# syamajala/cholesky

Hardware: AMD Instinct MI355X
Metric: fp64 factorization GF/s (numeric level loop, F_ref flops) on 3-D Laplacian (higher is better)
Workload: dtype f64; 1 GPU; tests/lapl_3375x3375 (reference fixture: 7-point Laplacian, nested-dissection ordering from the fixture files); n=3375, levels=5, separators=31, B_alg_bytes=2932064, parallelism=single GPU, precision=fp64

## Files before the change

cholesky_amd/_lib.py:

```python
import ctypes as C
import os

_HERE = os.path.dirname(os.path.abspath(__file__))
LIB_PATH = os.environ.get("CHOLAMD_LIB") or os.path.join(_HERE, "lib", "libcholamd.so")
HEADER_PATH = os.path.join(os.path.dirname(_HERE), "include", "cholamd.h")


class Filled(C.Structure):
    _fields_ = [("filled", C.c_int), ("sep_x", C.c_int), ("sep_y", C.c_int), ("interval", C.c_int), ("cluster", C.c_int),
                ("lo_x", C.c_int), ("lo_y", C.c_int), ("hi_x", C.c_int), ("hi_y", C.c_int)]


class Op(C.Structure):
    _fields_ = [("op", C.c_int), ("level", C.c_int), ("m", C.c_int), ("n", C.c_int), ("k", C.c_int),
                ("a_sx", C.c_int), ("a_sy", C.c_int), ("a_z", C.c_int), ("b_sx", C.c_int), ("b_sy", C.c_int), ("b_z", C.c_int),
                ("c_sx", C.c_int), ("c_sy", C.c_int), ("c_z", C.c_int)]


class Region(C.Structure):
    _fields_ = [("ptr", C.c_void_p), ("ld", C.c_int), ("lo_x", C.c_int), ("lo_y", C.c_int), ("hi_x", C.c_int), ("hi_y", C.c_int),
                ("tile_row", C.POINTER(C.c_int))]


class SepInfo(C.Structure):
# ... 76 lines not shown
    L.cholamd_device_set_option.argtypes = [vp, C.c_char_p, ci]
    L.cholamd_comm_unique_id.argtypes = [vp]
    L.cholamd_comm_create.argtypes = [vp, ci, ci, vp, C.POINTER(vp)]
    L.cholamd_comm_create_local.argtypes = [vp, ci, vp]
    L.cholamd_factor_multi.argtypes = [vp, vp, vp, ci, vp]
    L.cholamd_gather_factor.argtypes = [vp, vp, ci, vp]
    L.cholamd_comm_adopt.argtypes = [vp, ci, ci, C.POINTER(vp)]
    L.cholamd_comm_destroy.argtypes = [vp]
    L.cholamd_comm_destroy.restype = None
    L.cholamd_comm_allreduce.argtypes = [vp, vp, i64, vp]
    L.cholamd_device_tail_offset.argtypes = [vp]
    L.cholamd_device_tail_offset.restype = i64
    L.cholamd_exchange_tail.argtypes = [vp, vp, vp, vp]
    L.cholamd_factor_sharded.argtypes = [vp, vp, vp, vp]
    L.cholamd_factor_sharded_f32.argtypes = [vp, vp, vp, vp]
    L.cholamd_gather_to_root.argtypes = [vp, vp, ci, vp, vp]
    L.cholamd_exchange_volume.argtypes = [vp, vp]
    L.cholamd_plan_exchange_volume.argtypes = [vp, ci, ci, ci, vp]
    L.cholamd_plan_exchange_pieces.argtypes = [vp, ci, ci, ci, vp]
    L.cholamd_plan_solve_counts.argtypes = [vp, ci, ci, ci, vp]
    L.cholamd_plan_solve_skips.argtypes = [vp, ci, vp, vp]
    L.cholamd_solve_sharded.argtypes = [vp, vp, vp, vp, vp, vp]
    L.cholamd_solve_sharded_f32.argtypes = [vp, vp, vp, vp, vp, vp]
    L.cholamd_solve_refine_sharded.argtypes = [vp, vp, vp, vp, ci, C.c_double, vp, vp, vp, vp]
    L.cholamd_solve_multi.argtypes = [vp, vp, vp, vp, vp, ci, vp]
    L.cholamd_solve_refine_multi.argtypes = [vp, vp, vp, vp, ci, C.c_double, vp, vp, vp, ci, vp]
    L.cholamd_follow_rounds.argtypes = [ci, ci, ci, vp, vp]
    L.cholamd_plan_program_followers.argtypes = [vp, i64, vp]
    L.cholamd_plan_program_followers.restype = i64
    L.cholamd_plan_program_follow_own.argtypes = [vp, ci, ci, ci, ci, ci, i64, vp]
    L.cholamd_plan_program_follow_own.restype = i64
    L.cholamd_plan_program_check_follow.argtypes = [vp, ci, ci, ci, ci, ci, ci]
    L.cholamd_plan_program_hazards.argtypes = [vp, ci, ci, ci, ci, ci, vp]
    L.cholamd_factor_multi_f32.argtypes = [vp, vp, vp, ci, vp]
    L.cholamd_gather_factor_f32.argtypes = [vp, vp, ci, vp]
    L.cholamd_device_alloc.argtypes = [vp, i64, C.POINTER(vp)]
    L.cholamd_device_free.argtypes = [vp, vp]
    L.cholamd_device_upload.argtypes = [vp, vp, vp, i64, vp]
    L.cholamd_device_download.argtypes = [vp, vp, vp, i64, vp]
    L.cholamd_device_sync.argtypes = [vp, vp]
    L.cholamd_device_fill.argtypes = [vp, vp, vp]
    L.cholamd_factor.argtypes = [vp, vp, vp]
    L.cholamd_factor_levels.argtypes = [vp, vp, ci, ci, vp]
    L.cholamd_device_program_trace.argtypes = [vp, vp, vp, i64, vp, C.POINTER(ci)]
    L.cholamd_debug_live_buffers.argtypes = []
    L.cholamd_debug_live_buffers.restype = i64
    L.cholamd_factor_info.argtypes = [vp, C.POINTER(ci)]
    L.cholamd_solve.argtypes = [vp, vp, vp, vp, vp]
    L.cholamd_device_fill_f32.argtypes = [vp, vp, vp]
    L.cholamd_factor_f32.argtypes = [vp, vp, vp]
    L.cholamd_factor_levels_f32.argtypes = [vp, vp, ci, ci, vp]
    L.cholamd_solve_f32.argtypes = [vp, vp, vp, vp, vp]
    L.cholamd_solve_refine.argtypes = [vp, vp, vp, vp, ci, cd, C.POINTER(ci), C.POINTER(cd), vp]
    L.cholamd_residual.argtypes = [vp, vp, vp, vp, C.POINTER(cd), vp]
    L.cholamd_solve_nrhs.argtypes = [vp, vp, vp, i64, vp, i64, ci, vp]
    L.cholamd_solve_nrhs_f32.argtypes = [vp, vp, vp, i64, vp, i64, ci, vp]
    L.cholamd_solve_refine_nrhs.argtypes = [vp, vp, vp, i64, vp, i64, ci, ci, cd, C.POINTER(ci), vp, vp]
    L.cholamd_apply.argtypes = [vp, vp, vp, vp]
    L.cholamd_apply_nrhs.argtypes = [vp, vp, i64, vp, i64, ci, vp]
    L.cholamd_plan_apply_host.argtypes = [vp, vp, vp, vp]
    for name in ("cholamd_solve_pcg", "cholamd_solve_pcg_f32"):
        getattr(L, name).argtypes = [vp, vp, vp, vp, ci, cd, ci, vp, vp, vp, vp]
    for name in ("cholamd_solve_pcg_nrhs", "cholamd_solve_pcg_nrhs_f32"):
        getattr(L, name).argtypes = [vp, vp, vp, i64, vp, i64, ci, ci, cd, ci, vp, vp, vp, vp]
    L.cholamd_solve_half.argtypes = [vp, vp, vp, vp, ci, vp]
    L.cholamd_solve_half_f32.argtypes = [vp, vp, vp, vp, ci, vp]
# ... 125 lines not shown
```

cholesky_amd/csrc/chol_api.cpp:

```cpp
#include "chol_device.h"

int no_device_error()
{
  chol_set_error("no usable HIP device (libcholamd has no CPU fallback)");
  return CHOLAMD_ERR_NO_DEVICE;
}
bool ranges_overlap(const void *a, size_t na, const void *b, size_t nb)
{
  const char *pa = (const char *)a, *pb = (const char *)b;
  return pa < pb + nb && pb < pa + na;
}

extern "C" int cholamd_device_count(void)
{
  int n = 0;
  if (hipGetDeviceCount(&n) != hipSuccess) return 0;
  return n;
}

#define CHOL_POISON_GUARD ((size_t)64 << 10)
static bool poison_on()
{
  const char *e = std::getenv("CHOLAMD_POISON");
  return e && *e && atoi(e) != 0;
// ... 63 lines not shown

static int build_levels(cholamd_device *d)
{
  d->lv.clear(); d->lv32.clear(); d->prog = level_dev(); d->prog_ready = false;
  d->jobs.reset(); d->pwaits.reset(); d->exts.reset(); d->pctr.reset(); d->pctr_total.reset();
  d->sched_gen++;
  const int L = d->plan->levels;
  d->lv.resize(L);
  for (int lvl = 0; lvl < L; lvl++) {
    chol_level_work w;
    int rc = chol_build_level_work(d->plan, &d->opt, lvl, d->rank, d->world, &w);
    if (rc) return rc;
    rc = upload_level(d->lv[lvl], w);
    chol_level_work_free(&w);
    if (rc) return rc;
  }
  if (d->world == 1 && d->opt.program) {
    chol_level_work w;
    chol_program g;
    const bool built = chol_build_program(d->plan, &d->opt, &w, &g) == 0;
    const bool live = built && chol_program_check_built(d->plan, &d->opt, 4, &w, &g) == 0;
    if (built && !live) { chol_level_work_free(&w); chol_program_free(&g); }
    if (live) {
      int rc = upload_level(d->prog, w);
      std::vector<int> tot(g.ctr_total, g.ctr_total + g.n_ctr);
      int ncu = 256;
      hipDeviceProp_t prop;
      if (hipGetDeviceProperties(&prop, d->dev) == hipSuccess && prop.multiProcessorCount > 0) ncu = prop.multiProcessorCount;
      d->prog_grid = g.n_job < ncu ? g.n_job : ncu;
      tot.push_back(g.n_job + d->prog_grid);
      int mx = 1;
      for (int t : tot) mx = t > mx ? t : mx;
      d->prog_epoch_limit = (1 << 30) / mx;
      d->n_job = g.n_job; d->n_pctr = (int)tot.size(); d->prog_epoch = 0;
      d->jobs_host.assign(g.job, g.job + g.n_job);
      if (!rc) rc = d->jobs.upload(g.job, (size_t)g.n_job);
      const chol_wait no_wait = { 0, 0 };
      chol_ext no_ext;
      std::memset(&no_ext, 0, sizeof no_ext);
      if (!rc) rc = g.n_wait > 0 ? d->pwaits.upload(g.wait, (size_t)g.n_wait) : d->pwaits.upload(&no_wait, (size_t)1);
      if (!rc) rc = g.n_ext > 0 ? d->exts.upload(g.ext, (size_t)g.n_ext) : d->exts.upload(&no_ext, (size_t)1);
      if (!rc) rc = d->pctr_total.upload(tot.data(), tot.size());
      if (!rc) rc = d->pctr.alloc_zero(tot.size());
      chol_level_work_free(&w);
      chol_program_free(&g);
      if (rc) return rc;
      d->prog_ready = d->n_job > 0;
    }
  }
  return 0;
}

extern "C" int cholamd_device_create(const cholamd_plan *plan, int device_id, cholamd_device **out)
{
  *out = nullptr;
  if (!plan) { chol_set_error("null plan"); return CHOLAMD_ERR_ARG; }
  int ndev = 0;
  if (hipGetDeviceCount(&ndev) != hipSuccess || ndev <= 0) return no_device_error();
  if (device_id < 0 || device_id >= ndev) { chol_set_error("device %d out of range (%d devices)", device_id, ndev); return CHOLAMD_ERR_NO_DEVICE; }
  HIPCHK(hipSetDevice(device_id));
  cholamd_device *d = new cholamd_device();
  d->plan = plan; d->dev = device_id;
  chol_sched_opts_from_env(&d->opt);
  { const char *e = getenv("CHOLAMD_SOLVE_REFERENCE_SHAPE"); d->solve_reference_shape = e && *e && atoi(e) != 0; }
  { const char *e = getenv("CHOLAMD_SOLVE_DETERMINISTIC"); d->solve_deterministic = e && *e && atoi(e) != 0; }
  { const char *e = getenv("CHOLAMD_SOLVE_DETERMINISTIC_BLOCK"); d->solve_deterministic_block = e && *e && atoi(e) != 0; }
  { const char *e = getenv("CHOLAMD_SCHUR_DETERMINISTIC"); d->schur_deterministic = e && *e && atoi(e) != 0; }
// ... 30 lines not shown
  HIPCHK(hipSetDevice(d->dev));
  if (world < 1 || (world & (world - 1)) || rank < 0 || rank >= world || chol_split_level(world) > d->plan->levels - 1) {
    chol_set_error("bad partition: rank %d of %d for a %d-level tree", rank, world, d->plan->levels);
    return CHOLAMD_ERR_ARG;
  }
  d->rank = rank; d->world = world;
  free_solve_lists(d);
  return build_levels(d);
}

extern "C" int cholamd_device_bcast_phases(const cholamd_device *d)
{
  int n = 0;
  for (const level_dev &l : d->lv) for (const chol_phase &ph : l.phase) n += ph.kind == CHOL_PH_BCAST;
  return n;
}
extern "C" int cholamd_device_set_option(cholamd_device *d, const char *name, int value)
{
  HIPCHK(hipSetDevice(d->dev));
  const std::string n(name ? name : "");
  bool rebuild = true;
  if (n == "split_min") d->opt.split_min = value;
  else if (n == "split_nb") d->opt.split_nb = value;
  else if (n == "fuse") d->opt.fuse = value != 0;
  else if (n == "fuse_update_max") d->opt.fuse_update_max = value;
  else if (n == "mt_min_tiles") d->opt.mt_min_tiles = value;
  else if (n == "cells") d->opt.cells = value != 0;
  else if (n == "program") d->opt.program = value != 0;
  else if (n == "follow") d->opt.follow = value != 0;
  else if (n == "super_blocks") d->opt.super_blocks = value;
  else if (n == "follow_tail") d->opt.follow_tail = value;
  else if (n == "follow_tail_split") d->opt.follow_tail_split = value;
  else if (n == "follow_own") d->opt.follow_own = value < 0 ? 0 : value > 2 ? 2 : value;
  else if (n == "staged") d->opt.staged = value != 0;
  else if (n == "fine_upd") d->opt.fine_upd = value != 0;
  else if (n == "skyline") d->opt.skyline = value != 0;
  else if (n == "merge_targets") d->opt.merge_targets = value != 0;
  else if (n == "leaf_envelope") d->opt.leaf_envelope = value != 0;
  else if (n == "trsm_wt_min") d->opt.trsm_wt_min = value < 0 ? 0 : value;
  else if (n == "stage_chunk") d->opt.stage_chunk = value < 0 ? 0 : value;
  else if (n == "dist_top") d->opt.dist_top = value;
  else if (n == "solve_reference_shape") { d->solve_reference_shape = value != 0; rebuild = false; }
  else if (n == "solve_deterministic") { d->solve_deterministic = value != 0; rebuild = false; }
  else if (n == "solve_deterministic_block") { d->solve_deterministic_block = value != 0; rebuild = false; }
  else if (n == "schur_deterministic") { d->schur_deterministic = value != 0; rebuild = false; }
  else if (n == "multiply_nrhs_min") { d->multiply_nrhs_min = value; rebuild = false; }
  else { chol_set_error("unknown option '%s'", n.c_str()); return CHOLAMD_ERR_ARG; }
  return rebuild ? build_levels(d) : 0;
}

extern "C" int cholamd_device_alloc(cholamd_device *d, int64_t doubles, double **dptr)
{
  HIPCHK(hipSetDevice(d->dev));
  HIPCHK(fp_malloc((void **)dptr, (size_t)doubles * sizeof(double)));
  return 0;
}
extern "C" int cholamd_device_free(cholamd_device *d, double *dptr)
{
  HIPCHK(hipSetDevice(d->dev));
  HIPCHK(hipFree(dptr));
  return 0;
}
extern "C" int cholamd_device_upload(cholamd_device *d, double *d_dst, const double *h_src, int64_t doubles, void *stream)
{
  HIPCHK(hipSetDevice(d->dev));
  HIPCHK(hipMemcpyAsync(d_dst, h_src, (size_t)doubles * sizeof(double), hipMemcpyHostToDevice, (hipStream_t)stream));
// ... 172 lines not shown
  for (int k = 0; k < 4; k++) { ms_by_kind[k] = ms[k]; launches_by_kind[k] = n[k]; }
  return 0;
}

extern "C" int cholamd_device_event_overhead(cholamd_device *d, void *stream, float *ms_out)
{
  HIPCHK(hipSetDevice(d->dev));
  hipStream_t st = (hipStream_t)stream;
  const int reps = 64;
  std::vector<hipEvent_t> ev(2 * reps);
  for (auto &e : ev) e = get_event(d);
  for (int i = 0; i < reps; i++) { HIPCHK(hipEventRecord(ev[2 * i], st)); HIPCHK(hipEventRecord(ev[2 * i + 1], st)); }
  HIPCHK(hipStreamSynchronize(st));
  double acc = 0.0;
  for (int i = 0; i < reps; i++) { float ms = 0.f; HIPCHK(hipEventElapsedTime(&ms, ev[2 * i], ev[2 * i + 1])); acc += ms; }
  for (auto e : ev) d->pool.push_back(e);
  *ms_out = (float)(acc / reps);
  return 0;
}

extern "C" int cholamd_factor(cholamd_device *d, double *d_arena, void *stream)
{
  if (!d->prog_ready) return cholamd_factor_levels(d, d_arena, d->plan->levels - 1, 0, stream);
  HIPCHK(hipSetDevice(d->dev));
  hipStream_t st = (hipStream_t)stream;
  if (d->info_foreign) { HIPCHK(hipMemsetAsync(d->info, 0, 4 * sizeof(int), st)); d->info_foreign = false; }
  int *const info_cur = d->info + 2 * d->info_parity, *const info_next = d->info + 2 * (d->info_parity ^ 1);
  d->info_parity ^= 1; d->info_last = info_cur;
  if (d->prog_epoch >= d->prog_epoch_limit) { HIPCHK(hipMemsetAsync(d->pctr, 0, (size_t)d->n_pctr * sizeof(int), st)); d->prog_epoch = 0; }
  const level_dev &l = d->prog;
  {
    scoped_timer t(d, st, 3, true);
    HIPCHK((hipError_t)chol_launch_program(d_arena, d->ws, d->jobs, d->n_job, d->pwaits, l.potrf, l.trsm, l.task, l.src, d->exts, d->pctr, d->pctr_total, d->prog_epoch,
                                           d->pctr + d->n_pctr - 1, d->prog_epoch * (d->n_job + d->prog_grid), d->prog_grid, info_cur, info_next, d->trace, st));
  }
  d->prog_epoch++;
  return 0;
}
extern "C" int cholamd_device_program_trace(cholamd_device *d, double *d_arena, void *stream, int64_t cap, int64_t *out, int *njobs_out)
{
  HIPCHK(hipSetDevice(d->dev));
  if (!d->prog_ready) { chol_set_error("no program launch for this problem / these options"); return CHOLAMD_ERR_ARG; }
  *njobs_out = d->n_job;
  if (cap < (int64_t)5 * d->n_job) return 0;
  const size_t nst = (size_t)(4 + CHOL_TRACE_X) * d->n_job;
  std::vector<unsigned long long> h(nst);
  {
    dev_buf<unsigned long long> stamps;
    struct disarm { cholamd_device *d; ~disarm() { d->trace = nullptr; } } on_exit{ d };
    int rc = stamps.alloc_zero(nst);
    if (rc) return rc;
    d->trace = stamps;
    if ((rc = cholamd_factor(d, d_arena, stream))) return rc;
    HIPCHK(hipStreamSynchronize((hipStream_t)stream));
    HIPCHK(hipMemcpy(h.data(), stamps, h.size() * sizeof(unsigned long long), hipMemcpyDeviceToHost));
  }
  unsigned long long t0 = ~0ull;
  for (int j = 0; j < d->n_job; j++) if (h[4 * j] && h[4 * j] < t0) t0 = h[4 * j];
  for (int j = 0; j < d->n_job; j++) {
    out[5 * j] = d->jobs_host[j].kind + (d->jobs_host[j].kind == 0 && d->jobs_host[j].n_ext > 0 ? 10 : 0);
    for (int q = 0; q < 3; q++) out[5 * j + 1 + q] = (int64_t)(h[4 * j + q] - t0);
    out[5 * j + 4] = (int64_t)h[4 * j + 3];
  }
  if (const char *path = getenv("CHOLAMD_TRACE_FOLLOW")) {
    if (FILE *fp = fopen(path, "w")) {
      for (int j = 0; j < d->n_job; j++) {
        const unsigned long long *x = &h[(size_t)4 * d->n_job + (size_t)CHOL_TRACE_X * j];
        const int kind = d->jobs_host[j].kind;
        bool any = false;
        for (int i = 0; i < CHOL_TRACE_X; i++) any = any || x[i] != 0;
        if (!any) continue;
        if (kind == 2) { fprintf(fp, "job %d kind 2 last-stage-held %.1f\n", j, (double)(x[0] - t0) * 0.01); continue; }
        fprintf(fp, "job %d kind %d", j, kind);
        if (kind == 0 && x[1]) {
          fprintf(fp, " items %llu own-tiles-wait-over %.1f rounds:", x[1], x[0] ? (double)(x[0] - t0) * 0.01 : -1.0);
          for (unsigned long long i = 0; i < x[1] && i < 44; i++) if (x[2 + i]) fprintf(fp, " %llu:%.1f", i, (double)(x[2 + i] - t0) * 0.01);
        }
        if (kind == 0 && x[24]) { fprintf(fp, " | prologue (entry, LDS init, tables, slot tables read, columns 0-1 requested, tiles requested, columns 0-1 parked):"); const int ord[7] = { 0, 1, 2, 5, 6, 3, 4 }; for (int k = 0; k < 7; k++) fprintf(fp, " %.1f", x[24 + ord[k]] ? (double)(x[24 + ord[k]] - t0) * 0.01 : -1.0); }
        fprintf(fp, kind == 0 ? " | column started:" : " | POTRF column seen:");
        for (int k = 0; k < 24; k++) if (x[72 + k]) fprintf(fp, " %d:%.1f", k, (double)(x[72 + k] - t0) * 0.01);
        fprintf(fp, kind == 0 ? " | column published:" : " | column tile on the channel:");
        for (int k = 0; k < 24; k++) if (x[48 + k]) fprintf(fp, " %d:%.1f", k, (double)(x[48 + k] - t0) * 0.01);
        fprintf(fp, "\n");
      }
      fclose(fp);
    }
  }
  return 0;
}
extern "C" int cholamd_factor_info(cholamd_device *d, int *sep_out)
{
  HIPCHK(hipSetDevice(d->dev));
  int h[2] = { 0, 0 };
  HIPCHK(hipMemcpy(h, d->info_last ? d->info_last : d->info, sizeof h, hipMemcpyDeviceToHost));
  if (sep_out) *sep_out = h[1];
  if (h[0] == CHOLAMD_ERR_STALL)
    chol_set_error("factorisation stalled: a workgroup of a fused launch waited ~50 ms for a progress word of the same launch and gave up; the factor is not valid");
  else if (h[0] < 0) chol_set_error("factorisation failed with internal code %d", h[0]);
  return h[0];
}

__global__ void k_zero_ranges(double *y, const int *ranges, int nr)
{
  const int off = ranges[2 * blockIdx.y], len = ranges[2 * blockIdx.y + 1];
  for (int i = blockIdx.x * blockDim.x + threadIdx.x; i < len; i += gridDim.x * blockDim.x) y[off + i] = 0.0;
}
int build_solve(cholamd_device *d, int rank, int world)
{
  const int L = d->plan->levels;
  if (d->solve_ready && d->solve_rank == rank && d->solve_world == world) return 0;
  free_solve_lists(d);
// ... 1655 lines not shown
```

cholesky_amd/csrc/chol_device.h:

```cpp
#ifndef CHOL_DEVICE_H
#define CHOL_DEVICE_H
#include <hip/hip_runtime.h>
#include <rccl/rccl.h>

#include <cstdio>
#include <algorithm>
#include <cstdlib>
#include <cfloat>
#include <cmath>
#include <cctype>
#include <cstring>
#include <string>
#include <type_traits>
#include <vector>

#include <atomic>
#include "chol_devbuf.h"
#include "chol_kernels.h"
#include "chol_plan.h"
#include "cholamd.h"

#define HIPCHK(call)                                                                                  \
  do {                                                                                                \
    hipError_t e_ = (call);                                                                           \
// ... 55 lines not shown
  std::vector<level_dev> lv;
  std::vector<solve_dev> sv;
  bool solve_ready = false;
  int solve_rank = 0, solve_world = 1;
  dev_buf<int> zr_sub; int n_zr_sub = 0;
  dev_buf<double> ws;
  dev_buf<double> ws_solve;
  dev_buf<int> step_flags;
  int step_gen = 0;
  dev_buf<double> w256;
  dev_buf<double> step_xt;
  bool keep_inverses = false;
  dev_buf<int> info;
  int *info_last = nullptr;
  int info_parity = 0; bool info_foreign = false;
  dev_buf<int> progress;
  int epoch = 0, done_total = 0;
  dev_buf<int64_t> a_dst; dev_buf<double> a_val; dev_buf<int> perm; dev_buf<double> ytmp;
  dev_buf<int64_t> top_dst[2]; dev_buf<double> top_val[2]; dev_buf<int> top_e[2]; int64_t top_n[2] = { 0, 0 }; int top_gen[2] = { -1, -1 };
  dev_buf<int> a_src, csr_src; dev_buf<unsigned char> e_cls;
  dev_buf<int> e_row, e_col;
  dev_buf<int64_t> vs_dev, vs_init; pinned_words vs_host;
  int64_t vs_last[4] = { 0, 0, 0, 0 };
  bool vs_called = false, vs_last_valid = false;
  bool vs_in_force = false;
  bool f32_pending = false;
  bool timing = false;
  std::vector<timed_launch> tl;
  std::vector<hipEvent_t> pool;
  level_dev prog;
  dev_buf<chol_job> jobs; dev_buf<chol_wait> pwaits; dev_buf<chol_ext> exts;
  dev_buf<int> pctr, pctr_total;
  int n_job = 0, n_pctr = 0, prog_grid = 0, prog_epoch = 0, prog_epoch_limit = 0;
  bool prog_ready = false;
  unsigned long long *trace = nullptr;
  std::vector<chol_job> jobs_host;
  std::vector<level_dev> lv32;
  dev_buf<float> ws32;
  int f32_range = -1; int64_t f32_bad = -1;
  dev_buf<int64_t> csr_ptr; dev_buf<int> csr_col; dev_buf<double> csr_val;
  dev_buf<double> rvec, dxvec, partial;
  dev_buf<char> xstage; size_t xstage_bytes = 0; dev_buf<sum_desc> xdesc; int xdesc_gen = -1, xdesc_elem = 0, sched_gen = 0;
  chol_sched_opts opt;
  bool solve_reference_shape = false;
  bool solve_deterministic = false;
  bool solve_deterministic_block = false;
  sdet_dev sdet;
  dev_buf<double> ynrhs, bnrhs, rnrhs, dxnrhs, pnrhs;
  dev_buf<chol_trsv_desc> dg_desc; dev_buf<int> dg_prefix; int n_dg = 0;
  dev_buf<double> ld_part; dev_buf<int64_t> ld_ipart, ld_res;
  std::vector<selinv_dev> si; dev_buf<double> si_ws; bool si_ready = false;
  std::vector<schur_dev> sc;
  bool schur_deterministic = false;
  std::vector<sdet_dev> scd;
  int64_t schur_launches[4] = { 0, 0, 0, 0 };
  dev_buf<chol_mul_item> mul_item[2]; dev_buf<chol_mul_src> mul_src[2]; int n_mul_item[2] = { 0, 0 }; bool mul_ready = false;
  dev_buf<double> mvec, mr_part; dev_buf<int64_t> mr_ipart, mr_res;
  dev_buf<double> mznrhs, mwnrhs;
  int multiply_nrhs_min = 0;
  dev_buf<double> pcg_b, pcg_p, pcg_q, pcg_r, pcg_z, pcg_part;
  dev_buf<chol_pcg_rec> pcg_rec; pinned_words pcg_host;
};

struct local_group {
  int n = 0, refs = 0;
  std::vector<int> dev;
// ... 48 lines not shown
```

cholesky_amd/csrc/chol_kernels.h:

```cpp
#ifndef CHOL_KERNELS_H
#define CHOL_KERNELS_H
#include <hip/hip_runtime_api.h>
#include <stdint.h>
#include "chol_plan.h"
int chol_launch_scatter(double *arena, const int64_t *dst, const double *val, int64_t nnz, hipStream_t st);
#define CHOL_VALUES_STATUS 1
#define CHOL_VALUES_GATHER 2
int chol_launch_set_values(const double *vals, int64_t nz, const unsigned char *cls, double *a_val, const int *a_src, int64_t nnz_a,
                           double *csr_val, const int *csr_src, int64_t ncsr, int parts, int64_t *status, hipStream_t st);
int chol_launch_gather(double *out, const double *in, const int *idx, int64_t n, hipStream_t st);
int chol_launch_potrf(double *base, double *ws, const chol_potrf_desc *descs, int n, int *info, hipStream_t st);
int chol_launch_potrf_big(double *base, double *ws, const chol_potrf_desc *descs, int n, int *info, hipStream_t st);
int chol_launch_potrf_trsm(double *base, double *ws, const chol_potrf_desc *pdescs, int n_potrf, const chol_trsm_desc *tdescs, int n_trsm,
                           const chol_upd_task *tasks, const chol_upd_src *srcs, int n_task,
                           int *info, int *progress, int progress_base, int *done, int done_target, hipStream_t st);
int chol_launch_program(double *base, double *ws, const chol_job *jobs, int njobs, const chol_wait *waits, const chol_potrf_desc *pdescs, const chol_trsm_desc *tdescs,
                        const chol_upd_task *tasks, const chol_upd_src *srcs, const chol_ext *exts, int *ctr, const int *ctr_total, int epoch, int *head, int head_base,
                        int grid, int *info, int *info_next, unsigned long long *trace, hipStream_t st);
int chol_launch_trsm_w(double *base, const double *ws, const chol_trsm_desc *descs, int n, hipStream_t st);
int chol_launch_trsm_wt(double *base, const double *ws, const chol_trsm_desc *descs, int n, hipStream_t st);
int chol_launch_trsm_big(double *base, const double *ws, const chol_trsm_desc *descs, int n, hipStream_t st);
int chol_launch_dinv(const double *L, int n, int ldl, double *W, hipStream_t st);
int chol_launch_trsm(double *base, const double *ws, const chol_trsm_desc *descs, int n, hipStream_t st);
int chol_launch_update(double *base, const chol_upd_task *tasks, const chol_upd_src *srcs, int ntask, hipStream_t st);
int chol_launch_update_mt(double *base, const chol_upd_task *tasks, const chol_upd_src *srcs, int ntask, int64_t arena_elems, hipStream_t st);
int chol_launch_permute(const double *in, const int *perm, double *out, int n, int inverse, hipStream_t st);
template <class TL> int chol_launch_solve_dinv(const TL *base, const chol_trsv_desc *descs, int n, int max_n, double *W, hipStream_t st);
template <class TL> int chol_launch_solve_trsv(const TL *base, const chol_trsv_desc *descs, int n, int max_n, int max_under, const double *W, double *y, int backward, int *flags, int *gen, const double *W256, double *xt, hipStream_t st);
#define CHOL_STEPW_MAX_SEPS 128
template <class TL> int chol_launch_solve_inv256(const TL *base, const chol_trsv_desc *descs, int n, int max_n, const double *W16, double *W256, hipStream_t st);
template <class TL> int chol_launch_solve_offdiag(const TL *base, const chol_gemv_desc *blocks, const int *items, int n_items, double *y, int backward, hipStream_t st);
int chol_launch_trsv_fwd(const double *base, const chol_trsv_desc *descs, int n, double *y, hipStream_t st);
int chol_launch_gemv_fwd(const double *base, const chol_gemv_desc *descs, const int *grp_start, const int *grp_rows, int ngroups, double *y, hipStream_t st);
int chol_launch_bwd(const double *base, const chol_trsv_desc *descs, const chol_gemv_desc *gd, const int *gstart, int n, double *y, hipStream_t st);
int chol_launch_residual(const int64_t *ptr, const int *col, const double *val, const double *b, const double *x, double *r, int n, double *partial, hipStream_t st);
int chol_launch_axpy1(double *x, const double *dx, int n, hipStream_t st);
int chol_launch_scatter(float *arena, const int64_t *dst, const double *val, int64_t nnz, hipStream_t st);
int chol_launch_potrf(float *base, float *ws, const chol_potrf_desc *descs, int n, int *info, hipStream_t st);
int chol_launch_trsm(float *base, const float *ws, const chol_trsm_desc *descs, int n, hipStream_t st);
int chol_launch_trsm_wt(float *base, const float *ws, const chol_trsm_desc *descs, int n, hipStream_t st);
int chol_launch_update(float *base, const chol_upd_task *tasks, const chol_upd_src *srcs, int ntask, hipStream_t st);
int chol_launch_update_mt(float *base, const chol_upd_task *tasks, const chol_upd_src *srcs, int ntask, int64_t arena_elems, hipStream_t st);
#define CHOL_NRHS_W 32
int chol_nrhs_launch_permute(const double *B, int64_t ldb, const int *perm, double *Y, double *X, int64_t ldx, int n, int c0, int cols, int inverse, hipStream_t st);
template <class TL> int chol_nrhs_launch_trsv(const TL *base, const chol_trsv_desc *descs, int n, int max_n, int max_under, const double *W16, const double *W256, double *Y, int backward, hipStream_t st);
template <class TL> int chol_nrhs_launch_offdiag(const TL *base, const chol_gemv_desc *blocks, const int *items, int n_items, double *Y, int backward, hipStream_t st);
int chol_nrhs_launch_residual(const int64_t *ptr, const int *col, const double *val, const double *B, int64_t ldb, const double *X, int64_t ldx, double *R, int64_t ldr,
                              int n, int cols, double *partial, hipStream_t st);
int chol_nrhs_launch_axpy(double *X, int64_t ldx, const double *D, int64_t ldd, int n, int cols, hipStream_t st);
#define CHOL_LOGDET_MAX_BLOCKS 1024
template <class TL> int chol_launch_factor_diag(const TL *base, const chol_trsv_desc *descs, const int *prefix, int nd, int n, const int *perm, double *diag, hipStream_t st);
// ... 44 lines not shown
```

cholesky_amd/csrc/chol_kernels.hip:

```cpp
#include <hip/hip_runtime.h>
#include <float.h>
#include <stdint.h>

#include "chol_plan.h"
#include "chol_kernels.h"

#include "chol_wave.h"

__device__ __forceinline__ void report_stall(int *info)
{
#ifdef STALL_PLAIN
  atomicCAS(&info[0], 0, CHOLAMD_ERR_STALL);
#else
  int e;
  asm volatile("v_mov_b32 %0, %1" : "=v"(e) : "i"(CHOLAMD_ERR_STALL));
  atomicCAS(&info[0], 0, e);
#endif
}
__device__ __forceinline__ int wait_progress(const int *progress, int target, int seen, int *info)
{
  if (seen >= target) return seen;
  int v = 0;
  for (int it = 0; it < (1 << 23); ++it) {
    v = __builtin_amdgcn_readfirstlane(__hip_atomic_load(progress, __ATOMIC_RELAXED, __HIP_MEMORY_SCOPE_AGENT));
// ... 691 lines not shown
    if (rowok && col < n) e = (ti > tj || c <= r15) ? gload<PUB>(&src[(int64_t)(4 * q) * lda]) : 0.0;
    v[q] = e;
  }
  return v;
}
#define FOLLOW_SLOTS 4
#define FOLLOW_LOADS ((CHOL_FOLLOW_MAXT * TS * TS + RR_THREADS - 1) / RR_THREADS)
template <int SLEEP = 0>
__device__ __forceinline__ void wait_list(const chol_wait *__restrict__ wl, int n, const int *ctr, const int *__restrict__ ctr_total, int epoch, int lane, int *info)
{
  for (int b0 = 0; b0 < n; b0 += 64) {
    int c = 0, need = 0;
    const bool mine = b0 + lane < n;
    if (mine) { const chol_wait wt = wl[b0 + lane]; c = wt.ctr; need = wt.value + epoch * ctr_total[wt.ctr]; }
    for (int it = 0;; ++it) {
      const bool ok = !mine || __hip_atomic_load(&ctr[c], __ATOMIC_RELAXED, __HIP_MEMORY_SCOPE_AGENT) >= need;
      if (!__ballot(!ok)) break;
      if (it >= (1 << 21)) { if (lane == 0) report_stall(info); break; }
#ifndef WAIT_SLEEP
#define WAIT_SLEEP 32
#endif
      __builtin_amdgcn_s_sleep(SLEEP ? SLEEP : WAIT_SLEEP);
    }
  }
}
__device__ __forceinline__ bool wait_list_holds(const chol_wait *__restrict__ wl, int n, const int *ctr, const int *__restrict__ ctr_total, int epoch, int lane)
{
  bool ok = true;
  for (int b0 = 0; b0 < n; b0 += 64)
    if (b0 + lane < n) { const chol_wait wt = wl[b0 + lane]; ok = ok && __hip_atomic_load(&ctr[wt.ctr], __ATOMIC_RELAXED, __HIP_MEMORY_SCOPE_AGENT) >= wt.value + epoch * ctr_total[wt.ctr]; }
  return !__ballot(!ok);
}
struct follow_args { const chol_ext *ext; int n_ext; const int *ctr; const int *ctr_total; int epoch; const chol_wait *wl; int n_wl; unsigned long long *stamp, *xstamp;
                     int own_at;  };
__device__ __forceinline__ int ext_ready(const follow_args &f, int from, int lane)
{
  bool ok = true;
  if (from + lane < f.n_ext) {
    const int c = f.ext[from + lane].ctr;
    ok = __hip_atomic_load(&f.ctr[c], __ATOMIC_RELAXED, __HIP_MEMORY_SCOPE_AGENT) - f.epoch * f.ctr_total[c] >= f.ext[from + lane].need;
  }
  const unsigned long long notok = __ballot(!ok);
  const int lead = notok ? __builtin_ctzll(notok) : 64;
  return min(from + lead, f.n_ext);
}
template <bool UPD, bool PUB, bool TR = false>
__device__ __forceinline__ void follow_external(const double *__restrict__ base, const follow_args f, int T, int n, double *sE, d4 (&tile)[11], d4 (&stage)[3],
                                                const int (&ijp)[12], int w, int lane, int tid, int *info, const double *A, int lda, int r15, int g, int *sReady)
{
  const int lp = lane;
  int buf = 0;
  int ready = 0, ng = 0;
  double va[FOLLOW_LOADS], vb[FOLLOW_LOADS];
#ifndef FOLLOW_OWN_SLEEP
#define FOLLOW_OWN_SLEEP 4
#endif
  static_assert(CHOL_FOLLOW_PAIR_MAXT == RR_MAXT, "a pair of followed column tiles shares one LDS buffer of RR_MAXT tiles");
  const int own_at = f.own_at;
  const bool own_last = f.n_wl > 0 && own_at >= f.n_ext;
  bool own_ok = false;
  int own_c = 0, own_need = 0, own_v = 0;
  const bool own_look = !UPD && own_last && f.n_wl <= 64;
  if (own_look && lane < f.n_wl) { const chol_wait wt = f.wl[lane]; own_c = wt.ctr; own_need = wt.value + f.epoch * f.ctr_total[wt.ctr]; }
#define EXT_ROUND(I_) chol_follow_round(I_, f.n_ext, T)
#define EXT_LOAD(I_, V_)                                                                                             \
  {                                                                                                                  \
    const chol_ext xl_ = f.ext[I_];                                                                                  \
    const double *src_ = base + xl_.off;                                                                             \
    _Pragma("unroll") for (int it = 0; it < FOLLOW_LOADS; ++it) {                                                    \
      const int idx = tid + it * RR_THREADS;                                                                         \
      const int row = (idx >> 8) * TS + (idx & 15), col = (idx >> 4) & 15;                                           \
      V_[it] = (idx < T * TS * TS && row < n && col < xl_.ncol) ? gload<true>(&src_[row + (int64_t)col * xl_.ld]) : 0.0; \
    }                                                                                                                \
  }
#define EXT_LOAD_ROUND(I_)                                                                                           \
  {                                                                                                                  \
    EXT_LOAD(I_, va);                                                                                                \
    ng = EXT_ROUND(I_);                                                                                              \
    if (ng == 2) { EXT_LOAD((I_) + 1, vb); }                                                                         \
  }
#define EXT_UPDATE(acc_, ti_, tj_)                                                                                   \
  {                                                                                                                  \
    _Pragma("unroll") for (int st = 0; st < 4; ++st)                                                                 \
      acc_ = __builtin_amdgcn_mfma_f64_16x16x4f64(sB[(tj_) * (TS * TS) + st * 64 + lp], -sB[(ti_) * (TS * TS) + st * 64 + lp], acc_, 0, 0, 0); \
    if (G == 2) {                                                                                                    \
      _Pragma("unroll") for (int st = 0; st < 4; ++st)                                                               \
        acc_ = __builtin_amdgcn_mfma_f64_16x16x4f64(sB2[(tj_) * (TS * TS) + st * 64 + lp], -sB2[(ti_) * (TS * TS) + st * 64 + lp], acc_, 0, 0, 0); \
    }                                                                                                                \
  }
#define OWN_TILES()                                                                                                  \
  {                                                                                                                  \
  \
      if (!UPD) wait_list<FOLLOW_OWN_SLEEP>(f.wl, f.n_wl, f.ctr, f.ctr_total, f.epoch, lane, info);  \
      if (TR && !UPD && f.xstamp && lane == 0) f.xstamp[0] = __builtin_amdgcn_s_memrealtime(); \
      lds_barrier(); \
      if (UPD) { \
        int rx = r15, gx = g;  \
        asm volatile("" : "+v"(rx), "+v"(gx)); \
    _Pragma("unroll")                                                                                            \
        for (int it = 0; it < 3; ++it) { \
          const int u = min(w + it * RR_NW, 2 * T - 2); \
          stage[it] += load_tile<PUB>(A, lda, n, u < T ? u : u - T + 1, u < T ? 0 : 1, rx, gx); \
        } \
        __builtin_amdgcn_sched_barrier(0);  \
    _Pragma("unroll")                                                                                            \
        for (int s = 0; s < FOLLOW_SLOTS; ++s) \
          if (ijp[s] != 0xffff) tile[s] += load_tile<PUB>(A, lda, n, ijp[s] & 0xff, ijp[s] >> 8, rx, gx); \
        __builtin_amdgcn_sched_barrier(0); \
      } \
 \
  }
  for (int i = 0; i < f.n_ext;) {
    if (f.n_wl > 0 && i == own_at) OWN_TILES();
    if (ng == 0) {
      const int need = i + EXT_ROUND(i);
      if (ready < need) {
        if (!UPD) {
          ready = ext_ready(f, i, lane);
          for (int it = 0; ready < need; ++it) {
            if (it >= (1 << 24)) { if (lane == 0) report_stall(info); ready = f.n_ext; break; }
#ifndef EXT_SLEEP
#define EXT_SLEEP 4
#endif
            __builtin_amdgcn_s_sleep(EXT_SLEEP);
            ready = ext_ready(f, i, lane);
          }
          if (lane == 0) __hip_atomic_store(sReady, ready, __ATOMIC_RELAXED, __HIP_MEMORY_SCOPE_WORKGROUP);
        } else {
          for (int it = 0;; ++it) {
            ready = __builtin_amdgcn_readfirstlane(__hip_atomic_load(sReady, __ATOMIC_RELAXED, __HIP_MEMORY_SCOPE_WORKGROUP));
            if (ready >= need) break;
            if (it >= (1 << 25)) { if (lane == 0) report_stall(info); ready = f.n_ext; break; }
            __builtin_amdgcn_s_sleep(2);
          }
        }
      }
      EXT_LOAD_ROUND(i);
    }
    const int G = ng;
    if (TR && !UPD && f.xstamp && lane == 0 && i < 44) { f.xstamp[1] = f.n_ext; f.xstamp[2 + i] = __builtin_amdgcn_s_memrealtime(); }
    double *sB = sE + buf * (RR_MAXT * TS * TS), *sB2 = sB + T * TS * TS;
#pragma unroll
    for (int it = 0; it < FOLLOW_LOADS; ++it) {
      const int idx = tid + it * RR_THREADS;
      if (idx < T * TS * TS) { sB[idx] = va[it]; if (G == 2) sB2[idx] = vb[it]; }
    }
    const int j = i + G;
    ng = 0;
    int pv = 0, pneed = 0;
    bool polled = false;
    if (j < f.n_ext && j + EXT_ROUND(j) <= ready) { EXT_LOAD_ROUND(j); }
    else if (j < f.n_ext && !UPD) {
      polled = true;
      if (j + lane < f.n_ext) { const int c = f.ext[j + lane].ctr; pv = __hip_atomic_load(&f.ctr[c], __ATOMIC_RELAXED, __HIP_MEMORY_SCOPE_AGENT); pneed = f.epoch * f.ctr_total[c] + f.ext[j + lane].need; }
    }
    const bool look = own_look && !own_ok;
    if (look && lane < f.n_wl) own_v = __hip_atomic_load(&f.ctr[own_c], __ATOMIC_RELAXED, __HIP_MEMORY_SCOPE_AGENT);
    lds_barrier();
    if (look) own_ok = !__ballot(lane < f.n_wl && own_v < own_need);
    if (UPD) {
#pragma unroll
      for (int it = 0; it < 3; ++it) {
        const int u = w + it * RR_NW;
        if (u < 2 * T - 1) { const int tj = u < T ? 0 : 1, ti = u < T ? u : u - T + 1; EXT_UPDATE(stage[it], ti, tj); }
      }
#pragma unroll
      for (int s = 0; s < FOLLOW_SLOTS; ++s)
        if (ijp[s] != 0xffff) { const int ti = ijp[s] & 0xff, tj = ijp[s] >> 8; EXT_UPDATE(tile[s], ti, tj); }
    }
    buf ^= 1;
    if (polled) {
      const unsigned long long notok = __ballot(j + lane < f.n_ext && pv < pneed);
      const int r2 = min(j + (notok ? __builtin_ctzll(notok) : 64), f.n_ext);
      if (r2 > ready) { ready = r2; if (lane == 0) __hip_atomic_store(sReady, ready, __ATOMIC_RELAXED, __HIP_MEMORY_SCOPE_WORKGROUP); }
    } else if (UPD && j < f.n_ext && ready < j + EXT_ROUND(j)) {
      const int r2 = __builtin_amdgcn_readfirstlane(__hip_atomic_load(sReady, __ATOMIC_RELAXED, __HIP_MEMORY_SCOPE_WORKGROUP));
      ready = r2 > ready ? r2 : ready;
    }
    i = j;
  }
  if (own_last) {
    if (!UPD && !own_ok) wait_list<FOLLOW_OWN_SLEEP>(f.wl, f.n_wl, f.ctr, f.ctr_total, f.epoch, lane, info);
    if (TR && !UPD && f.xstamp && lane == 0) f.xstamp[0] = __builtin_amdgcn_s_memrealtime();
    lds_barrier();
    if (UPD) {
      int rx = r15, gx = g;
      asm volatile("" : "+v"(rx), "+v"(gx));
#pragma unroll
      for (int it = 0; it < 3; ++it) {
        const int u = min(w + it * RR_NW, 2 * T - 2);
        tile[FOLLOW_SLOTS + it] = load_tile<PUB>(A, lda, n, u < T ? u : u - T + 1, u < T ? 0 : 1, rx, gx);
      }
#pragma unroll
      for (int s = 0; s < FOLLOW_SLOTS; ++s) {
        const d4 zero4 = { 0.0, 0.0, 0.0, 0.0 };
        tile[FOLLOW_SLOTS + 3 + s] = zero4;
        if (ijp[s] != 0xffff) tile[FOLLOW_SLOTS + 3 + s] = load_tile<PUB>(A, lda, n, ijp[s] & 0xff, ijp[s] >> 8, rx, gx);
      }
    }
  }
#undef OWN_TILES
#undef EXT_LOAD_ROUND
#undef EXT_ROUND
#undef EXT_UPDATE
#undef EXT_LOAD
}

template <bool PUB, bool FOLLOW = false, bool TR = false>
__device__ __forceinline__ void potrf_rr_body(double *__restrict__ base, double *__restrict__ ws, const chol_potrf_desc d, int *__restrict__ info,
                                              int *__restrict__ progress, int progress_base, double *smem, const unsigned char *__restrict__ sky, const follow_args fa = follow_args(), const int tid = threadIdx.x)
{
  double (*const sRaw)[TS * TS] = (double (*)[TS * TS])(smem);
  double (*const sSol)[RR_MAXT][TS * TS] = (double (*)[RR_MAXT][TS * TS])(smem + RR_OFF_SOL);
  double (*const sDg)[TS * TS] = (double (*)[TS * TS])(smem + RR_OFF_DG);
  double (*const sLW)[4 * TS][TS + 1] = (double (*)[4 * TS][TS + 1])(smem + RR_OFF_LW);
  double (*const sConv)[TS + 1] = (double (*)[TS + 1])(smem + RR_OFF_CONV);
  double (*const sOv)[TS * TS] = (double (*)[TS * TS])(smem + RR_OFF_OV);
  unsigned short *const sIJ = (unsigned short *)(smem + RR_OFF_IJ);
  int *const sFlag = (int *)(smem + RR_OFF_FLAG);
  unsigned char *const sKm = (unsigned char *)(smem + RR_OFF_KM);
  int *const sMask = (int *)(smem + RR_OFF_MASK);
  unsigned char *const sSky = (unsigned char *)(smem + RR_OFF_SKY);
  int *const fL = &sFlag[0], *const fP = &sFlag[1], *const cSol = &sFlag[2], *const cUpd = &sFlag[3];
  int *const cRaw = &sFlag[4];
  int *const fA = &sFlag[6];
  int *const fD = &sFlag[7];
  int *const f00 = &sFlag[8];

  double *A = base + d.a_off;
  double *W = ws + d.dinv_off;
  const int n = d.n, lda = d.lda;
  const int T = (n + TS - 1) / TS;
  const int ntl = T * (T + 1) / 2;
  const int lane = tid & 63;
  const int wave = __builtin_amdgcn_readfirstlane(tid >> 6);
  const int r15 = lane & 15, g = lane >> 4;
  const int lp0 = g * TS + r15;

#define PSTAMP(i_) do { if (TR && fa.xstamp && fa.n_ext == 0 && tid == 64) fa.xstamp[24 + (i_)] = __builtin_amdgcn_s_memrealtime(); } while (0)
  PSTAMP(0);
  d4 stage[3];
  const bool own_pending = FOLLOW && fa.n_ext > 0 && fa.n_wl > 0 && fa.own_at >= fa.n_ext;
  const bool stage_early = !(FOLLOW && fa.n_ext > 0) && wave != 0;
  if (stage_early) {
#pragma unroll
    for (int it = 0; it < 3; ++it) {
      const int u = min(wave - 1 + it * RR_NW, 2 * T - 2);
      stage[it] = load_tile<PUB>(A, lda, n, u < T ? u : u - T + 1, u < T ? 0 : 1, r15, g);
    }
  }
  const unsigned char *const tab = d.tab > 0 ? sky - __builtin_offsetof(chol_potrf_desc, sky) + d.tab : nullptr;
  if (tab) {
    static_assert((RR_MAXT * RR_NW) % 1 == 0 && RR_THREADS >= RR_MAXT * RR_NW + RR_SLOTS * RR_NW / 2 + RR_SLOTS * RR_NW / 4, "one pass copies the tables");
    if (tid < RR_MAXT * RR_NW) sMask[tid] = ((const int *)(tab + CHOL_RR_TAB_MASK))[tid];
    else if (tid < RR_MAXT * RR_NW + RR_SLOTS * RR_NW / 2) ((int *)sIJ)[tid - RR_MAXT * RR_NW] = ((const int *)(tab + CHOL_RR_TAB_IJ))[tid - RR_MAXT * RR_NW];
    else if (tid < RR_MAXT * RR_NW + RR_SLOTS * RR_NW / 2 + RR_SLOTS * RR_NW / 4) ((int *)sKm)[tid - RR_MAXT * RR_NW - RR_SLOTS * RR_NW / 2] = ((const int *)(tab + CHOL_RR_TAB_KM))[tid - RR_MAXT * RR_NW - RR_SLOTS * RR_NW / 2];
  } else {
    for (int t = tid; t < RR_SLOTS * RR_NW; t += RR_THREADS) { sIJ[t] = (unsigned short)0xffff; sKm[t] = 0; }
    for (int t = tid; t < RR_MAXT * RR_NW; t += RR_THREADS) sMask[t] = 0;
  }
  if (tid < 24) sSky[tid] = sky[tid];
  if (tid < 10) sFlag[tid] = 0;
  if (tid < TS * TS) sConv[TS + (tid >> 4)][tid & 15] = (tid >> 4) == (tid & 15) ? 1.0 : 0.0;
  __syncthreads();
  PSTAMP(1);
  const int ntl2 = (T - 2) * (T - 1) / 2;
  if (!tab) {
  for (int t = tid + 2 * T - 1; t < ntl; t += RR_THREADS) {
    int ti, tj, ow, os;
    tile_of_index(t, T, ti, tj);
    rr_owner(ntl - 1 - t, ntl2, ow, os);
    sIJ[os * RR_NW + ow] = (unsigned short)(ti | (tj << 8));
    const int kmin = max(sky[min(ti, 23)], sky[min(tj, 23)]);
    sKm[os * RR_NW + ow] = kmin | (tj < sky[min(ti, 23)] ? CHOL_RR_KM_ZERO : 0);
    const int last = ti == tj ? tj - 2 : tj - 1;
    for (int k = min(kmin, last); k <= last; ++k) atomicOr(&sMask[k * RR_NW + ow], 1 << os);
  }
  for (int t = tid; t < T * T; t += RR_THREADS) {
    const int k = t / T, i = t % T;
    if (i >= k + 2 && sky[min(i, 23)] <= k) {
      const int hv = i % RR_NHEAVY;
      atomicOr(&sMask[k * RR_NW + hv + hv / 3], 1 << (i < k + 2 + RR_NHEAVY ? RR_M_SOLVE0 : RR_M_SOLVE1));
    }
  }
  __syncthreads();
  }
  PSTAMP(2);

  if (wave == 0) {
    __builtin_amdgcn_s_setprio(3);
    if (FOLLOW && fa.n_ext > 0) {
      d4 tdummy[RR_RSLOTS], sdummy[3];
      int idummy[RR_SLOTS];
      follow_external<false, PUB, TR>(base, fa, T, n, smem + RR_OFF_SOL, tdummy, sdummy, idummy, 0, lane, tid, info, A, lda, r15, g, &sFlag[5]);
      lds_barrier();
      if (TR && fa.stamp && lane == 0) *fa.stamp = __builtin_amdgcn_s_memrealtime();
    }
    __builtin_amdgcn_s_setprio(3);
    lds_wait_ge(f00, 1);
    d4 dk;
#pragma unroll
    for (int q = 0; q < 4; ++q) dk[q] = sDg[0][q * 64 + lp0];
    STAMP_DECL;
    POLL_DECL;
    for (int k = 0; k < T; ++k) {
      STAMPK(0);
      double a[TS], unused;
#pragma unroll
      for (int q = 0; q < 4; ++q) sConv[r15][g + 4 * q] = dk[q];
#pragma unroll
      for (int c = 0; c < TS; ++c) a[c] = sConv[lane & 31][c];
      const int cupd_early = __hip_atomic_load(cUpd, __ATOMIC_RELAXED, __HIP_MEMORY_SCOPE_WORKGROUP);
      STAMPK(1);
      if (TR && fa.xstamp && lane == 0 && k < 24) fa.xstamp[72 + k] = __builtin_amdgcn_s_memrealtime();
      const bool more = k + 1 < T;
      const int kn = more ? k + 1 : k;
      long long fl = 0;
      d4 raw, dn;
      const int bad = chol16_rows(a, unused, r15, [&]() {
        fl = __hip_atomic_load((long long *)fA, __ATOMIC_RELAXED, __HIP_MEMORY_SCOPE_WORKGROUP);
        asm volatile("" ::: "memory");
#pragma unroll
        for (int q = 0; q < 4; ++q) { raw[q] = sRaw[kn][q * 64 + lp0]; dn[q] = sDg[kn & 1][q * 64 + lp0]; }
      });
      STAMPK(2);
      if (bad && k * TS + bad <= n && lane == 0) {
        if (atomicCAS(&info[0], 0, d.col0 + k * TS + bad) == 0) info[1] = d.sep;
// ... 29 lines not shown
    STAMP_FLUSH;
    POLL_FLUSH;
    __builtin_amdgcn_s_setprio(0);
  } else {
    d4 tile[RR_RSLOTS];
    const int w = wave - 1;
    const int hw = rr_heavy_index(w);
    int ijp[RR_SLOTS];
#pragma unroll
    for (int s = 0; s < RR_SLOTS; ++s) ijp[s] = __builtin_amdgcn_readfirstlane((int)sIJ[s * RR_NW + w]);
    int kmn[RR_SLOTS];
#pragma unroll
    for (int s = 0; s < RR_SLOTS; ++s) kmn[s] = __builtin_amdgcn_readfirstlane((int)sKm[s * RR_NW + w]);
    unsigned zmask = 0;
#pragma unroll
    for (int s = 0; s < RR_SLOTS; ++s) { zmask |= (kmn[s] & CHOL_RR_KM_ZERO) ? 1u << s : 0u; kmn[s] &= CHOL_RR_KM_ZERO - 1; }
    PSTAMP(5);

    if (FOLLOW && fa.n_ext > 0) {
      const bool early = fa.n_wl == 0;
      const d4 zero4 = { 0.0, 0.0, 0.0, 0.0 };
#pragma unroll
      for (int it = 0; it < 3; ++it) {
        const int u = min(w + it * RR_NW, 2 * T - 2);
        stage[it] = zero4;
        if (early) stage[it] = load_tile<PUB>(A, lda, n, u < T ? u : u - T + 1, u < T ? 0 : 1, r15, g);
      }
#pragma unroll
      for (int s = 0; s < FOLLOW_SLOTS; ++s) {
        d4 v = zero4;
        if (early && ijp[s] != 0xffff) v = load_tile<PUB>(A, lda, n, ijp[s] & 0xff, ijp[s] >> 8, r15, g);
        tile[s] = v;
      }
      follow_external<true, PUB, TR>(base, fa, T, n, smem + RR_OFF_SOL, tile, stage, ijp, w, lane, tid, info, A, lda, r15, g, &sFlag[5]);
      lds_barrier();
      if (own_pending) {
#pragma unroll
        for (int it = 0; it < 3; ++it) stage[it] += tile[FOLLOW_SLOTS + it];
      }
    } else {
    PSTAMP(6);
#pragma unroll
    for (int s = 0; s < RR_RSLOTS; ++s) {
      d4 v = { 0.0, 0.0, 0.0, 0.0 };
      if (ijp[s] != 0xffff && !(zmask & (1u << s))) v = load_tile<PUB>(A, lda, n, ijp[s] & 0xff, ijp[s] >> 8, r15, g);
      tile[s] = v;
    }
    }
    PSTAMP(3);
#pragma unroll
    for (int it = 0; it < 3; ++it) {
      const int u = w + it * RR_NW;
      if (u < 2 * T - 1) {
        const int tj = u < T ? 0 : 1, ti = u < T ? u : u - T + 1;
        double *park = ti == tj ? &sDg[ti][0] : tj == 0 ? &sRaw[ti][0] : &sSol[1][ti][0];
#pragma unroll
        for (int q = 0; q < 4; ++q) park[q * 64 + lp0] = stage[it][q];
        if (u == 0) lds_set(f00, 1, lane);
        if (ti == 1) lds_set(tj == 0 ? fA : fD, 1, lane);
        if (tj == 0 && ti > 0) lds_inc(cRaw, lane);
      }
    }
    if (FOLLOW && fa.n_ext > 0) {
      static_assert(FOLLOW_SLOTS + 3 + FOLLOW_SLOTS <= RR_RSLOTS, "a follower's own tiles in flight fit the register tiles it does not use");
      if (own_pending) {
        __builtin_amdgcn_sched_barrier(0);
#pragma unroll
        for (int s = 0; s < FOLLOW_SLOTS; ++s) tile[s] += tile[FOLLOW_SLOTS + 3 + s];
      }
// ... 454 lines not shown
  const int wave = __builtin_amdgcn_readfirstlane(threadIdx.x >> 6);
  const int lane = threadIdx.x & 63;
  const int grp = wave >> 2;
  const int n_tg = (n_trsm + 2) / 3;
  if ((int)blockIdx.x < n_potrf) {
    potrf_rr_body<true>(base, ws, pdescs[blockIdx.x], info, progress + blockIdx.x, progress_base, smem, pdescs[blockIdx.x].sky);
  } else if ((int)blockIdx.x < n_potrf + n_tg) {
    double (*sX)[3][TS * TS] = (double (*)[3][TS * TS])smem;
    const int id = ((int)blockIdx.x - n_potrf) * 3 + grp;
    chol_trsm_desc d = tdescs[min(id, n_trsm - 1)];
    if (id >= n_trsm) d.m = 0;
    trsm_rr_body<true, FUSED_SLOTS>(base, ws, d, sX[grp], wave & 3, lane, progress + d.flag, progress_base, info);
    if (n_task > 0) {
      asm volatile("s_waitcnt vmcnt(0)" ::: "memory");
      lds_barrier();
      if (threadIdx.x == 0) __hip_atomic_fetch_add(done, 1, __ATOMIC_RELAXED, __HIP_MEMORY_SCOPE_AGENT);
    }
  } else {
    double (*sAcc)[3][3][4][64] = (double (*)[3][3][4][64])smem;
    const int u = (int)blockIdx.x - n_potrf - n_tg;
    int round = 0;
    for (int t0 = u * 3; t0 < n_task; t0 += n_upd_wg * 3, ++round) {
      const int tid = t0 + grp;
      const bool live = tid < n_task;
      update_task_body<true>(base, tasks[live ? tid : t0], srcs, sAcc[round & 1][grp], wave & 3, lane, live, round == 0 ? done : nullptr, done_target, info);
    }
  }
}

#define PROG_XFLAGS 32
#define PROG_OFF_XFLAG (3 * RR_MAXT * TS * TS)
static_assert(PROG_XFLAGS >= 4 * ((CHOL_RR_MAXN / TS + 3) / 4) && PROG_XFLAGS >= 4 * FUSED_SLOTS && PROG_OFF_XFLAG + (3 * PROG_XFLAGS + 1) / 2 <= RR_SMEM_DOUBLES, "the strips' slots and flags fit the image");
static_assert(CHOL_RR_MAXN <= RR_MAXT * TS && CHOL_FUSE_MAXN <= CHOL_RR_MAXN, "one slot per column tile of the widest strip");
template <bool TR>
__global__ __launch_bounds__(RR_THREADS) void k_program(double *__restrict__ base, double *__restrict__ ws, const chol_job *__restrict__ jobs, int njobs,
                                                        const chol_wait *__restrict__ waits, const chol_potrf_desc *__restrict__ pdescs,
                                                        const chol_trsm_desc *__restrict__ tdescs, const chol_upd_task *__restrict__ tasks,
                                                        const chol_upd_src *__restrict__ srcs, const chol_ext *__restrict__ exts,
                                                        int *__restrict__ ctr, const int *__restrict__ ctr_total, int epoch, int *__restrict__ head, int head_base,
                                                        int *__restrict__ info, int *__restrict__ info_next, unsigned long long *__restrict__ trace)
{
  if (info_next && blockIdx.x == 0 && threadIdx.x == 0) { info_next[0] = 0; info_next[1] = 0; }
  __shared__ double smem[RR_SMEM_DOUBLES];
  __shared__ int s_job;
  const int wave_id = __builtin_amdgcn_readfirstlane(threadIdx.x >> 6);
  for (;;) {
#ifdef TID_PLAIN
    int tid = threadIdx.x;
#else
    int tid = wave_id * 64 + (int)__builtin_amdgcn_mbcnt_hi(~0u, __builtin_amdgcn_mbcnt_lo(~0u, 0u));
#endif
    asm volatile("" : "+v"(tid));
    const int wave = wave_id;
    const int lane = tid & 63;
    const int grp = wave >> 2;
    __syncthreads();
    if (tid == 0) s_job = atomicAdd(head, 1) - head_base;
    __syncthreads();
    const int j = s_job;
    if (j >= njobs) break;
    const chol_job jb = jobs[j];
    if (TR && trace && tid == 0) { trace[4 * j] = __builtin_amdgcn_s_memrealtime(); trace[4 * j + 3] = blockIdx.x; }
    int *const xflags = (int *)(smem + PROG_OFF_XFLAG);
    if (jb.kind == CHOL_JOB_TRSM && tid < 3 * PROG_XFLAGS) xflags[tid] = 0;
    bool fenced = false;
    chol_upd_task tpre;
    if (jb.kind == CHOL_JOB_UPDATE) {
      const int tk = jb.first + min(jb.mode == 0 ? wave : grp, jb.n - 1);
      tpre = tasks[tk];
      int touch = 0;
      for (int sx = tpre.src_begin; sx < tpre.src_end; ++sx) touch += srcs[sx].k;
      asm volatile("" :: "s"(touch));
    }
    if (jb.n_pre > 0 && !(jb.kind == CHOL_JOB_POTRF && jb.n_ext > 0)) {
      if (wave == 0) wait_list(waits + jb.wait_first, jb.n_pre, ctr, ctr_total, epoch, lane, info);
      lds_barrier();
      fenced = true;
    }
    if (TR && trace && tid == 0) trace[4 * j + 1] = __builtin_amdgcn_s_memrealtime();
    if (jb.kind == CHOL_JOB_POTRF) {
      const chol_potrf_desc pd = pdescs[jb.first];
      follow_args fa;
      fa.ext = exts + jb.ext_first; fa.n_ext = jb.n_ext; fa.ctr = ctr; fa.ctr_total = ctr_total; fa.epoch = epoch; fa.wl = waits + jb.wait_first; fa.n_wl = jb.n_wait; fa.own_at = jb.mode; fa.stamp = TR && trace ? &trace[4 * j + 1] : nullptr; fa.xstamp = TR && trace ? &trace[4 * njobs + CHOL_TRACE_X * j] : nullptr;
      potrf_rr_body<true, true, TR>(base, ws, pd, info, ctr + pd.ctr, epoch * ctr_total[pd.ctr], smem, pdescs[jb.first].sky, fa, tid);
    } else if (jb.kind == CHOL_JOB_TRSM) {
      double (*sX)[RR_MAXT][TS * TS] = (double (*)[RR_MAXT][TS * TS])smem;
      chol_trsm_desc d = tdescs[jb.first + min(grp, jb.n - 1)];
      if (grp >= jb.n) d.m = 0;
      if (!fenced) lds_barrier();
      if (d.band > 0)
        trsm_rr_body<true, (CHOL_RR_MAXN / TS + 3) / 4, true, TR, true>(base, ws, d, sX[grp], wave & 3, lane, ctr + d.flag, epoch * ctr_total[d.flag], info, d.chan >= 0 ? ctr + d.chan : nullptr,
                                                                         TR && trace && grp == 0 ? &trace[4 * njobs + CHOL_TRACE_X * j] : nullptr, xflags + grp * PROG_XFLAGS);
      else
        trsm_rr_body<true, FUSED_SLOTS, false, TR, true>(base, ws, d, sX[grp], wave & 3, lane, ctr + d.flag, epoch * ctr_total[d.flag], info, d.chan >= 0 ? ctr + d.chan : nullptr,
                                                         TR && trace && grp == 0 ? &trace[4 * njobs + CHOL_TRACE_X * j] : nullptr, xflags + grp * PROG_XFLAGS);
    } else {
      stage_waits sw;
      sw.w = waits + jb.wait_first + jb.n_pre; sw.n = jb.n_wait - jb.n_pre; sw.ctr = ctr; sw.ctr_total = ctr_total; sw.epoch = epoch; sw.info = info;
      unsigned long long *const xs = TR && trace && wave == 0 ? &trace[4 * njobs + CHOL_TRACE_X * j] : nullptr;
      if (jb.mode == 0) {
        for (int t0 = jb.first; t0 < jb.first + jb.n; t0 += RR_NW + 1) {
          const int tk = t0 + wave;
          if (tk < jb.first + jb.n) update_task_wave<true, TR>(base, t0 == jb.first ? tpre : tasks[tk], srcs, lane, sw, xs);
        }
      } else {
        double (*sAcc)[3][3][4][64] = (double (*)[3][3][4][64])smem;
        int round = 0;
        for (int t0 = jb.first; t0 < jb.first + jb.n; t0 += 3, ++round) {
          const int tk = t0 + grp;
          const bool live = tk < jb.first + jb.n;
          update_task_body<true, TR>(base, t0 == jb.first ? tpre : tasks[live ? tk : t0], srcs, sAcc[round & 1][grp], wave & 3, lane, live, nullptr, 0, info, sw, xs);
        }
      }
    }
    if (jb.sig[0] >= 0) {
      asm volatile("s_waitcnt vmcnt(0)" ::: "memory");
      lds_barrier();
// ... 285 lines not shown
  return (int)hipGetLastError();
}
int chol_launch_potrf_big(double *base, double *ws, const chol_potrf_desc *descs, int n, int *info, hipStream_t st)
{
  if (n <= 0) return 0;
  hipLaunchKernelGGL(k_potrf_big, dim3(n), dim3(256), 0, st, base, ws, descs, info);
  return (int)hipGetLastError();
}
int chol_launch_dinv(const double *L, int n, int ldl, double *W, hipStream_t st)
{
  if (n <= 0) return 0;
  hipLaunchKernelGGL(k_dinv, dim3((n + TS - 1) / TS), dim3(64), 0, st, L, n, ldl, W);
  return (int)hipGetLastError();
}
int chol_launch_trsm(double *base, const double *ws, const chol_trsm_desc *descs, int n, hipStream_t st)
{
  if (n <= 0) return 0;
  hipLaunchKernelGGL(k_trsm_rr, dim3(n), dim3(256), 0, st, base, ws, descs);
  return (int)hipGetLastError();
}
int chol_launch_potrf_trsm(double *base, double *ws, const chol_potrf_desc *pdescs, int n_potrf, const chol_trsm_desc *tdescs, int n_trsm,
                           const chol_upd_task *tasks, const chol_upd_src *srcs, int n_task,
                           int *info, int *progress, int progress_base, int *done, int done_target, hipStream_t st)
{
  if (n_potrf <= 0) return 0;
  int n_upd_wg = (n_task + 2) / 3;
  if (n_upd_wg > 1024) n_upd_wg = 1024;
  hipLaunchKernelGGL(k_potrf_trsm, dim3(n_potrf + (n_trsm + 2) / 3 + n_upd_wg), dim3(RR_THREADS), 0, st, base, ws, pdescs, n_potrf, tdescs, n_trsm,
                     tasks, srcs, n_task, n_upd_wg, info, progress, progress_base, done, done_target);
  return (int)hipGetLastError();
}
int chol_launch_program(double *base, double *ws, const chol_job *jobs, int njobs, const chol_wait *waits, const chol_potrf_desc *pdescs, const chol_trsm_desc *tdescs,
                        const chol_upd_task *tasks, const chol_upd_src *srcs, const chol_ext *exts, int *ctr, const int *ctr_total, int epoch, int *head, int head_base,
                        int grid, int *info, int *info_next, unsigned long long *trace, hipStream_t st)
{
  if (njobs <= 0) return 0;
  if (trace) hipLaunchKernelGGL(k_program<true>, dim3(grid), dim3(RR_THREADS), 0, st, base, ws, jobs, njobs, waits, pdescs, tdescs, tasks, srcs, exts, ctr, ctr_total, epoch, head, head_base, info, info_next, trace);
  else hipLaunchKernelGGL(k_program<false>, dim3(grid), dim3(RR_THREADS), 0, st, base, ws, jobs, njobs, waits, pdescs, tdescs, tasks, srcs, exts, ctr, ctr_total, epoch, head, head_base, info, info_next, trace);
  return (int)hipGetLastError();
}
int chol_launch_trsm_w(double *base, const double *ws, const chol_trsm_desc *descs, int n, hipStream_t st)
{
  if (n <= 0) return 0;
  hipLaunchKernelGGL(k_trsm_w, dim3((n + 3) / 4), dim3(256), 0, st, base, ws, descs, n);
  return (int)hipGetLastError();
}
int chol_launch_trsm_wt(double *base, const double *ws, const chol_trsm_desc *descs, int n, hipStream_t st)
{
  if (n <= 0) return 0;
  hipLaunchKernelGGL(k_trsm_wt, dim3((n + TT_WAVES - 1) / TT_WAVES), dim3(64 * TT_WAVES), 0, st, base, ws, descs, n);
  return (int)hipGetLastError();
}
int chol_launch_trsm_big(double *base, const double *ws, const chol_trsm_desc *descs, int n, hipStream_t st)
{
  if (n <= 0) return 0;
  hipLaunchKernelGGL(k_trsm_big, dim3((n + 3) / 4), dim3(256), 0, st, base, ws, descs, n);
  return (int)hipGetLastError();
}
int chol_launch_update(double *base, const chol_upd_task *tasks, const chol_upd_src *srcs, int ntask, hipStream_t st)
{
  if (ntask <= 0) return 0;
  const int per_xcd = (ntask + 7) / 8;
  hipLaunchKernelGGL(k_update, dim3(per_xcd * 8), dim3(256), 0, st, base, tasks, srcs, ntask, per_xcd);
  return (int)hipGetLastError();
}
int chol_launch_update_mt(double *base, const chol_upd_task *tasks, const chol_upd_src *srcs, int ntask, int64_t arena_elems, hipStream_t st)
{
  if (ntask <= 0) return 0;
  const int per_xcd = (ntask + 7) / 8;
  hipLaunchKernelGGL(k_update_mt, dim3(per_xcd * 8), dim3(256), 0, st, base, tasks, srcs, ntask, per_xcd, arena_elems);
  return (int)hipGetLastError();
// ... 2 lines not shown
```

cholesky_amd/csrc/chol_plan.h:

```cpp
#ifndef CHOL_PLAN_H
#define CHOL_PLAN_H

#include <stdint.h>
#include "cholamd.h"

#ifdef __cplusplus
extern "C" {
#endif

#define CHOL_ENTRY_OUT 0
#define CHOL_ENTRY_IN 1
#define CHOL_ENTRY_DROPPED 2
#define CHOL_NB 16
#define CHOL_RR_MAXN 272
#ifndef CHOL_FOLLOW_ALL_MAXT
#define CHOL_FOLLOW_ALL_MAXT 4
#endif
#define CHOL_FOLLOW_TAIL 3
#define CHOL_FOLLOW_MAXT 10
#define CHOL32_TRSM_GROUP 16
#define CHOL32_MAXN 128

typedef struct {
  int n_int;
// ... 93 lines not shown
  int range;
  int stage, pad;
} chol_upd_src;

typedef struct {
  int64_t c_off;
  int ldc;
  short mv, nv;
  int lower;
  int src_begin, src_end;
  int ar, br;
  int blk;
} chol_upd_task;

typedef struct { int ctr, value; } chol_wait;
enum chol_job_kind { CHOL_JOB_POTRF = 0, CHOL_JOB_TRSM = 1, CHOL_JOB_UPDATE = 2 };
typedef struct {
  int kind;
  int first, n;
  int wait_first, n_wait;
  int sig[2], sig_add;
  int ext_first, n_ext;
  int mode, n_pre;
} chol_job;
typedef struct {
  int64_t off;
  int ld, ncol;
  int ctr, need;
} chol_ext;
#define CHOL_FOLLOW_PAIR_MAXT 17
#define CHOL_FOLLOW_SINGLE_TAIL 0
#define CHOL_FOLLOW_OWN_BEFORE 2
#define CHOL_FOLLOW_OWN 1
#if defined(__HIPCC__)
#define CHOL_HD __host__ __device__ __forceinline__
#else
#define CHOL_HD static inline
#endif
CHOL_HD int chol_follow_round(int i, int n_ext, int T)
{
  const int pair_lim = 2 * T <= CHOL_FOLLOW_PAIR_MAXT ? n_ext - CHOL_FOLLOW_SINGLE_TAIL : 0;
  return i + 1 < pair_lim ? 2 : 1;
}
CHOL_HD int chol_follow_own_at(int n_ext, int T)
{
  int own_at = 0;
  for (int i = 0; i < n_ext; i += chol_follow_round(i, n_ext, T))
    if (i <= n_ext - CHOL_FOLLOW_OWN_BEFORE) own_at = i;
  return own_at;
}

typedef struct {
  int n_job; chol_job *job;
  int n_wait; chol_wait *wait;
  int n_ext; chol_ext *ext;
  int n_ctr; int *ctr_total;
  int follow;
} chol_program;

enum chol_phase_kind {
  CHOL_PH_POTRF = 0, CHOL_PH_TRSM = 1,
  CHOL_PH_UPDATE = 2,
  CHOL_PH_UPDATE_MT = 3,
  CHOL_PH_TRSM_W = 4,
  CHOL_PH_FUSED = 5,
  CHOL_PH_BCAST = 6,
  CHOL_PH_TRSM_WT = 7
};
typedef struct {
  int kind;
  int first, n, first2, n2, first3, n3;
} chol_phase;
typedef struct { int64_t off, count; int owner, heap; } chol_bcast;
static inline unsigned chol_top_contributors(int heap, int world)
{
  int d = 0, l = 0;
  while ((1 << d) < world) d++;
  while ((heap >> (l + 1)) > 0) l++;
  const int lo = (heap << (d - l)) - (1 << d), hi = ((heap + 1) << (d - l)) - (1 << d);
  unsigned m = 0u;
  for (int g = lo; g < hi; g++) m |= 1u << g;
  return m;
}

#define CHOL_DIST_MIN 1024
#define CHOL_MT_MIN_TILES 8192
typedef struct {
  int split_min, split_nb;
  int fuse;
  int fuse_update_max;
  int mt_min_tiles;
  int trsm_group;
  int trsm_wt_min;
  int cells;
  int program;
  int follow;
  int dist_top;
  int skyline;
  int stage_chunk;
  int fine_upd;
  int staged;
  int follow_tail_split;
  int follow_tail;
  int merge_targets;
  int leaf_envelope;
  int super_blocks;
  int follow_own;
} chol_sched_opts;
#define CHOL_SUPER_BLOCKS 3
#define CHOL_STAGE_CHUNK 0
void chol_sched_opts_default(chol_sched_opts *o);
void chol_sched_opts_from_env(chol_sched_opts *o);

#define CHOL_SPLIT_MIN 144
#ifndef CHOL_PROG_SPLIT_MIN
#define CHOL_PROG_SPLIT_MIN 176
#endif
#define CHOL_SPLIT_NB 144

typedef struct {
  int level;
  int n_phase; chol_phase *phase;
  int n_potrf; chol_potrf_desc *potrf;
  int n_trsm; chol_trsm_desc *trsm;
  int n_task; chol_upd_task *task;
  int n_task_mt; chol_upd_task *task_mt;
  int n_src; chol_upd_src *src;
  int n_bcast; chol_bcast *bcast;
} chol_level_work;

typedef struct {
  int64_t a_off; int n, lda; int x_off; int sep;
  int64_t dinv_off;
  int band;
} chol_trsv_desc;
typedef struct {
  int64_t a_off; int m, n, lda; int x_off, y_off;
  int c_lo;
} chol_gemv_desc;

// ... 164 lines not shown
```

cholesky_amd/csrc/chol_schedule.c:

```c
#define _GNU_SOURCE
#include <stdlib.h>
#include <string.h>

#include "chol_plan.h"
#include "cholamd.h"

int chol_split_level(int world)
{
  int d = 0;
  while ((1 << d) < world) d++;
  return d;
}

int chol_owner_of(const plan_t *p, int label, int world)
{
  int d = chol_split_level(world), lvl = p->level_of[label];
  if (lvl < d) return -1;
  return (p->heap_of[label] >> (lvl - d)) - (1 << d);
}

typedef struct {
  int64_t key;
  int64_t seq;
  int64_t c_off, a_off, b_off;
// ... 34 lines not shown
}

static int same_sources(const upd_tuple *tu, const tgt_group *a, const tgt_group *b, int dr, int dc)
{
  if (a->e - a->i != b->e - b->i) return 0;
  for (int q = 0; q < a->e - a->i; q++) {
    const upd_tuple *x = &tu[a->i + q], *y = &tu[b->i + q];
    if (x->src_sep != y->src_sep || x->lda != y->lda || x->ldb != y->ldb || x->k != y->k || y->a_off != x->a_off + dr || y->b_off != x->b_off + dc) return 0;
  }
  return 1;
}

static void index_snapshot(const plan_t *p, int lbl, int64_t *first, int *count)
{
  for (int b = 0; b < p->nblk; b++) { first[b] = 0; count[b] = 0; }
  const cholamd_filled *v = p->snap[lbl];
  for (int64_t i = 0; i < p->snap_n[lbl]; i++) {
    int b = BIDX(p, v[i].sep_x, v[i].sep_y);
    if (count[b] == 0) first[b] = i;
    count[b]++;
  }
}

typedef struct { int64_t c_off; int ldc, m, n, syrk, src_begin, src_end, blk, ar0, br0; } upd_target;
typedef struct { chol_level_work *w; const chol_sched_opts *o; int force_fine; int cur_blk; const int *follow_lim;
  int dist_world, dist_rank; const struct cholamd_plan *dist_plan; int tgt_sep, tgt_col0; int cap_b;
  const int *sw_of;
  int cur_band; const int *bw_of;
  int cap_p, cap_t, cap_k, cap_km, cap_s, cap_ph; upd_target *pend; int n_pend, cap_pend; } builder;
static int env_int(const char *name, int dflt) { const char *e = getenv(name); return e && *e ? atoi(e) : dflt; }
void chol_sched_opts_default(chol_sched_opts *o)
{
  o->split_min = CHOL_SPLIT_MIN; o->split_nb = CHOL_SPLIT_NB; o->fuse = 1; o->fuse_update_max = CHOL_FUSE_UPDATE_MAX;
  o->mt_min_tiles = CHOL_MT_MIN_TILES; o->trsm_wt_min = CHOL_TRSM_WT_MIN; o->trsm_group = 0; o->cells = 1; o->program = 1; o->follow = 1; o->super_blocks = CHOL_SUPER_BLOCKS; o->dist_top = 2; o->follow_tail = CHOL_FOLLOW_TAIL; o->follow_tail_split = CHOL_FOLLOW_TAIL; o->staged = 1; o->fine_upd = 1; o->skyline = 1; o->stage_chunk = CHOL_STAGE_CHUNK; o->merge_targets = 1; o->leaf_envelope = 1; o->follow_own = CHOL_FOLLOW_OWN;
}
void chol_sched_opts_from_env(chol_sched_opts *o)
{
  chol_sched_opts_default(o);
  o->split_min = env_int("CHOLAMD_SPLIT_MIN", o->split_min);
  o->split_nb = env_int("CHOLAMD_SPLIT_NB", o->split_nb);
  o->fuse = !env_int("CHOLAMD_NO_FUSE", 0);
  o->fuse_update_max = env_int("CHOLAMD_FUSE_UPDATE_MAX", o->fuse_update_max);
  o->mt_min_tiles = env_int("CHOLAMD_MT_MIN_TILES", o->mt_min_tiles);
  o->trsm_wt_min = env_int("CHOLAMD_TRSM_WT_MIN", o->trsm_wt_min);
  o->cells = !env_int("CHOLAMD_NO_CELLS", 0);
  o->program = !env_int("CHOLAMD_NO_PROGRAM", 0);
  o->follow = !env_int("CHOLAMD_NO_FOLLOW", 0);
  o->dist_top = env_int("CHOLAMD_DIST_TOP", o->dist_top);
  o->super_blocks = env_int("CHOLAMD_SUPER_BLOCKS", o->super_blocks);
  o->follow_tail = env_int("CHOLAMD_FOLLOW_TAIL", o->follow_tail);
  o->follow_tail_split = env_int("CHOLAMD_FOLLOW_TAIL_SPLIT", o->follow_tail_split);
  o->follow_own = env_int("CHOLAMD_FOLLOW_OWN", o->follow_own);
  o->staged = !env_int("CHOLAMD_NO_STAGED", 0);
  o->fine_upd = !env_int("CHOLAMD_NO_FINE_UPD", 0);
  o->skyline = !env_int("CHOLAMD_NO_SKYLINE", 0);
  o->merge_targets = !env_int("CHOLAMD_NO_MERGE_TARGETS", 0);
  o->leaf_envelope = !env_int("CHOLAMD_NO_LEAF_ENVELOPE", 0);
  o->stage_chunk = env_int("CHOLAMD_STAGE_CHUNK", o->stage_chunk);
}
static int split_nb(const chol_sched_opts *o) { int v = o->split_nb; if (v > CHOL_RR_MAXN) v = CHOL_RR_MAXN; v = (v + 15) / 16 * 16; if (v < 16) v = 16; return v; }
static int pivot_blocks(const chol_sched_opts *o, int n) { return n > o->split_min || n > CHOL_RR_MAXN ? (n + split_nb(o) - 1) / split_nb(o) : 1; }
static int pivot_block_width(const chol_sched_opts *o, int n) { const int nb = pivot_blocks(o, n); return nb == 1 ? n : ((n + nb - 1) / nb + 15) / 16 * 16; }


static void push_phase_full(builder *B, chol_phase ph)
{
  chol_level_work *w = B->w;
  if (w->n_phase == B->cap_ph) { B->cap_ph = B->cap_ph ? 2 * B->cap_ph : 16; w->phase = realloc(w->phase, B->cap_ph * sizeof(chol_phase)); }
  w->phase[w->n_phase++] = ph;
}
static void push_phase_f(builder *B, int kind, int first, int n, int force)
{
  if (n <= 0 && !force) return;
  if (n < 0) n = 0;
  chol_phase ph = { kind, first, n, 0, 0, 0, 0 };
  push_phase_full(B, ph);
}
static void push_phase(builder *B, int kind, int first, int n) { push_phase_f(B, kind, first, n, 0); }
void chol_potrf_table(int n, const unsigned char *sky, unsigned char *out)
{
  int *mask = (int *)(out + CHOL_RR_TAB_MASK);
  unsigned short *ij = (unsigned short *)(out + CHOL_RR_TAB_IJ);
  unsigned char *km = out + CHOL_RR_TAB_KM;
  memset(out, 0, CHOL_RR_TAB_BYTES);
  for (int t = 0; t < CHOL_RR_SLOTS * CHOL_RR_NW; t++) ij[t] = 0xffff;
// ... 651 lines not shown
} pblock;
typedef struct { chol_program *pg; int cap_j, cap_w, cap_e, cap_c;
  int *c_updp, *cnt_updp;
} pbuild;
static int new_ctr(pbuild *P, int total)
{
  chol_program *g = P->pg;
  if (g->n_ctr == P->cap_c) { P->cap_c = P->cap_c ? 2 * P->cap_c : 256; g->ctr_total = realloc(g->ctr_total, P->cap_c * sizeof(int)); }
  g->ctr_total[g->n_ctr] = total;
  return g->n_ctr++;
}
static void add_wait(pbuild *P, int ctr, int value)
{
  chol_program *g = P->pg;
  if (value <= 0) return;
  if (g->n_wait == P->cap_w) { P->cap_w = P->cap_w ? 2 * P->cap_w : 1024; g->wait = realloc(g->wait, P->cap_w * sizeof(chol_wait)); }
  chol_wait wt = { ctr, value };
  g->wait[g->n_wait++] = wt;
}
static int add_ext(pbuild *P, chol_ext e)
{
  chol_program *g = P->pg;
  if (g->n_ext == P->cap_e) { P->cap_e = P->cap_e ? 2 * P->cap_e : 64; g->ext = realloc(g->ext, P->cap_e * sizeof(chol_ext)); }
  g->ext[g->n_ext] = e;
  return g->n_ext++;
}
typedef struct { chol_ext x; int key, seq; } ext_item;
static int cmp_ext_item(const void *a, const void *b)
{
  const ext_item *x = a, *y = b;
  if (x->key != y->key) return x->key < y->key ? -1 : 1;
  return x->seq < y->seq ? -1 : (x->seq > y->seq);
}
static void push_ext_items(ext_item **items, int *n, int *cap, int64_t off, int ld, int k, int chan, int nstrip, int key0, int e_from)
{
  for (int e = e_from; e * CHOL_NB < k; e++) {
    if (*n == *cap) { *cap = *cap ? 2 * *cap : 64; *items = realloc(*items, *cap * sizeof(ext_item)); }
    ext_item *it = &(*items)[(*n)];
    it->x.off = off + (int64_t)e * CHOL_NB * ld; it->x.ld = ld; it->x.ncol = k - e * CHOL_NB < CHOL_NB ? k - e * CHOL_NB : CHOL_NB;
    it->x.ctr = chan + e; it->x.need = nstrip;
    it->key = key0 + e; it->seq = *n;
    (*n)++;
  }
}
static chol_job *add_job(pbuild *P, int kind, int first, int n, int wait_first)
{
  chol_program *g = P->pg;
  if (g->n_job == P->cap_j) { P->cap_j = P->cap_j ? 2 * P->cap_j : 1024; g->job = realloc(g->job, P->cap_j * sizeof(chol_job)); }
  chol_job j = { kind, first, n, wait_first, g->n_wait - wait_first, { -1, -1 }, 0, g->n_ext, 0, 0, g->n_wait - wait_first };
  g->job[g->n_job] = j;
  return &g->job[g->n_job++];
}
void chol_program_free(chol_program *g)
{
  free(g->job); free(g->wait); free(g->ext); free(g->ctr_total);
  memset(g, 0, sizeof *g);
}
typedef struct {
  const plan_t *p; chol_sched_opts o; chol_level_work *w; chol_program *pg; builder B; pbuild P;
  int follow;
  unsigned char **sky;
  int *bw_of, *band_of;
  int *sw_of;
  int *nblk_of; pblock **pb;
  int *est_start;
  int *c_upd, *c_updd;
  int *cnt_upd, *cnt_updd;
  int *snap_upd;
  int *follow_lim;
  int level; const cholamd_filled *snap; int64_t *first; int *count;
  int *hs, nh, steps;
} prog_ctx;
// ... 125 lines not shown
    free(first[s]);
  }
  free(first);
  return sky;
}
void chol_free_skylines(unsigned char **sky, int ns) { if (!sky) return; for (int s = 1; s <= ns; s++) free(sky[s]); free(sky); }
int **chol_leaf_row_first(const plan_t *p)
{
  const int ns = p->nsep, L = p->levels;
  int **first = calloc(ns + 1, sizeof(int *));
  for (int h = 1 << (L - 1); h <= ns; h++) {
    const int s = p->tree[h], n = p->sep_size[s], ld = p->panel_ld[s];
    if (n <= 0) continue;
    first[s] = malloc((size_t)ld * sizeof(int));
    for (int r = 0; r < ld; r++) first[s][r] = r < n ? r : n;
  }
  for (int64_t e = 0; e < p->nnz_a; e++) {
    const int64_t off = p->a_dst[e];
    int lo = 1, hi = ns;
    while (lo < hi) { const int mid = (lo + hi + 1) / 2; if (p->panel_off[mid] <= off) lo = mid; else hi = mid - 1; }
    const int s = lo;
    if (!first[s]) continue;
    const int64_t rel = off - p->panel_off[s];
    const int ld = p->panel_ld[s], row = (int)(rel % ld), col = (int)(rel / ld);
    if (col < first[s][row]) first[s][row] = col;
  }
  return first;
}

typedef struct { int64_t off; int ld, k, ctr, need; } early_src;
#ifndef EARLY_CHUNK
#define EARLY_CHUNK 2
#endif
static int emit_early_cells(prog_ctx *c, int64_t c_off, int ldc, int lim, int blk, const early_src *es, int nes)
{
  chol_level_work *w = c->w;
  builder *B = &c->B;
  int nst = 0, maxch = 0;
  for (int q = 0; q < nes; q++) if (es[q].k > 0) { const int ch = ((es[q].k + CHOL_NB - 1) / CHOL_NB + EARLY_CHUNK - 1) / EARLY_CHUNK; nst += ch; if (ch > maxch) maxch = ch; }
  if (nst == 0) return 0;
  wait_src *ws = malloc(nst * sizeof(wait_src));
  nst = 0;
  for (int ch = 0; ch < maxch; ch++)
    for (int q = 0; q < nes; q++) {
      if (es[q].k <= 0) continue;
      const int et = (es[q].k + CHOL_NB - 1) / CHOL_NB;
      if (ch * EARLY_CHUNK >= et) continue;
      const int last = (ch + 1) * EARLY_CHUNK < et ? (ch + 1) * EARLY_CHUNK - 1 : et - 1;
      const wait_src x = { es[q].ctr - (et - 1) + last, es[q].need, q, ch };
      ws[nst++] = x;
    }
  const int staged = B->o->staged;
  const int k0 = w->n_task, Tl = (lim + CHOL_NB - 1) / CHOL_NB;
  for (int I = 0; I < Tl; I++)
    for (int J = 0; J <= I; J++) {
      const int sb = w->n_src;
      for (int z = 0; z < nst; z++) {
        const early_src *e = &es[ws[z].tag];
        const int col0 = ws[z].est * EARLY_CHUNK * CHOL_NB, kc = e->k - col0 < EARLY_CHUNK * CHOL_NB ? e->k - col0 : EARLY_CHUNK * CHOL_NB;
        chol_upd_src sd = { e->off + CHOL_NB * I + (int64_t)col0 * e->ld, e->off + CHOL_NB * J + (int64_t)col0 * e->ld, e->ld, e->ld, kc, 0, staged ? z + 1 : 0, 0 };
        push_src(B, sd);
      }
      if (w->n_task == B->cap_k) { B->cap_k = B->cap_k ? 2 * B->cap_k : 256; w->task = realloc(w->task, B->cap_k * sizeof(chol_upd_task)); }
      chol_upd_task *t = &w->task[w->n_task++];
      memset(t, 0, sizeof *t);
      t->c_off = c_off + CHOL_NB * I + (int64_t)(CHOL_NB * J) * ldc; t->ldc = ldc;
      t->mv = (short)(lim - CHOL_NB * I < CHOL_NB ? lim - CHOL_NB * I : CHOL_NB);
      t->nv = (short)(lim - CHOL_NB * J < CHOL_NB ? lim - CHOL_NB * J : CHOL_NB);
      t->lower = I == J;
      t->src_begin = sb; t->src_end = w->n_src;
      t->blk = blk;
    }
  const int col_sep = c->p->blk[blk].c;
  c->snap_upd[col_sep] = c->cnt_upd[col_sep];
  emit_update_jobs(c, k0, w->n_task, ws, nst, staged);
  free(ws);
  return w->n_task > k0;
}

static chol_sched_opts chol_program_opts(const chol_sched_opts *o)
{
  chol_sched_opts r = *o;
  if (r.split_min == CHOL_SPLIT_MIN && r.split_nb == CHOL_SPLIT_NB) r.split_min = CHOL_PROG_SPLIT_MIN;
  return r;
}
static void prog_ctx_free(prog_ctx *c)
{
  const int ns = c->p->nsep;
  free(c->P.c_updp); free(c->P.cnt_updp);
  if (c->pb) for (int s = 1; s <= ns; s++) free(c->pb[s]);
  chol_free_skylines(c->sky, ns); free(c->bw_of); free(c->band_of); free(c->sw_of);
  free(c->est_start); free(c->pb); free(c->nblk_of); free(c->first); free(c->count); free(c->hs);
  free(c->c_upd); free(c->c_updd); free(c->cnt_upd); free(c->cnt_updd); free(c->snap_upd); free(c->follow_lim);
// ... 61 lines not shown
      b->c0 = st * bw; b->nb = n - b->c0 < bw ? n - b->c0 : bw;
      b->potrf = -1; b->ch_below = b->ch_par = b->ch_rest = -1;
      b->c_prog = new_ctr(P, (b->nb + CHOL_NB - 1) / CHOL_NB);
      b->c_strips = new_ctr(P, 0);
    }
  }
  c->est_start = calloc(ns + 1, sizeof(int));
  for (int h = ns; h >= 1; h--) {
    int st0 = 0;
    for (int k = 2 * h; k <= 2 * h + 1 && k <= ns; k++) {
      const int kid = p->tree[k];
      const int end = c->est_start[kid] + (p->sep_size[kid] + CHOL_NB - 1) / CHOL_NB;
      if (end > st0) st0 = end;
    }
    c->est_start[p->tree[h]] = st0;
  }
  return 0;
}
static void prog_begin_level(prog_ctx *c, int level)
{
  const plan_t *p = c->p;
  const int lbl = p->levels - 1 - level;
  c->level = level;
  index_snapshot(p, lbl, c->first, c->count);
  c->snap = p->snap[lbl];
  c->nh = c->steps = 0;
  for (int h = 1 << level; h <= (1 << (level + 1)) - 1; h++) {
    const int s = p->tree[h];
    if (c->count[BIDX(p, s, s)] == 0 || p->sep_size[s] == 0) continue;
    c->hs[c->nh++] = h;
    if (c->nblk_of[s] > c->steps) c->steps = c->nblk_of[s];
  }
}
static void emit_potrf_job(prog_ctx *c, int s, int st, int ext_first, int early)
{
  const plan_t *p = c->p;
  chol_program *pg = c->pg;
  pblock *b = &c->pb[s][st];
  const int ld = p->panel_ld[s];
  const int64_t diag = p->panel_off[s] + b->c0 + (int64_t)b->c0 * ld;
  const int64_t dinv = p->dinv_off[s] + (int64_t)(b->c0 / CHOL_NB) * CHOL_NB * CHOL_NB;
  chol_potrf_desc pd = { diag, dinv, b->nb, ld, s, b->c0, b->c_prog, 0, { 0 } };
  if (c->sky[s])
    for (int i = 0; i * CHOL_NB < b->nb && i < 24; i++) {
      const int f = c->sky[s][b->c0 / CHOL_NB + i] - b->c0 / CHOL_NB;
      pd.sky[i] = (unsigned char)(f > 0 ? f : 0);
    }
  push_potrf(&c->B, pd);
  b->potrf = c->w->n_potrf - 1;
  const int wf = pg->n_wait;
  add_wait(&c->P, c->c_updd[s], c->cnt_updd[s]);
  chol_job *j = add_job(&c->P, CHOL_JOB_POTRF, b->potrf, 1, wf);
  j->ext_first = ext_first; j->n_ext = pg->n_ext - ext_first;
  if (j->n_ext > 0)
    j->mode = j->n_wait > 0 && (c->o.follow_own == 2 || (c->o.follow_own == 1 && early)) ? j->n_ext
              : chol_follow_own_at(j->n_ext, (b->nb + CHOL_NB - 1) / CHOL_NB);
  b->emitted = 1;
}
static void emit_plain_potrf_jobs(prog_ctx *c, int st)
{
  for (int q = 0; q < c->nh; q++) {
    const int s = c->p->tree[c->hs[q]];
    if (st < c->nblk_of[s] && !c->pb[s][st].emitted) emit_potrf_job(c, s, st, c->pg->n_ext, 0);
  }
}
static void emit_step_trsm_jobs(prog_ctx *c, int st)
{
  const plan_t *p = c->p;
  chol_level_work *w = c->w;
  builder *B = &c->B;
  pbuild *P = &c->P;
  for (int q = 0; q < c->nh; q++) {
    const int h = c->hs[q], s = p->tree[h], n = p->sep_size[s], ld = p->panel_ld[s];
    if (st >= c->nblk_of[s]) continue;
    pblock *b = &c->pb[s][st];
    const int c0 = b->c0, nb = b->nb, nt = (nb + CHOL_NB - 1) / CHOL_NB;
    const int64_t diag = p->panel_off[s] + c0 + (int64_t)c0 * ld;
    const int64_t dinv = p->dinv_off[s] + (int64_t)(c0 / CHOL_NB) * CHOL_NB * CHOL_NB;
    const int64_t colbase = (int64_t)c0 * ld;
    const int below = n - c0 - nb;
    const int t0 = w->n_trsm;
    B->cur_band = c->band_of[s];
    int nb1 = 0;
    if (below > 0) {
      nb1 = c->pb[s][st + 1].nb;
      const int fol = c->follow && (nb1 + CHOL_NB - 1) / CHOL_NB <= CHOL_FOLLOW_MAXT;
      if (fol) { b->ns_below = (nb1 + CHOL_TRSM_ROWS - 1) / CHOL_TRSM_ROWS; b->ch_below = new_ctr(P, b->ns_below); for (int e = 1; e < nt; e++) new_ctr(P, b->ns_below); }
      push_trsm_run(B, diag, dinv, p->panel_off[s] + (c0 + nb) + colbase, nb, ld, nb1, b->c_prog);
      for (int i = w->n_trsm - (nb1 + CHOL_TRSM_ROWS - 1) / CHOL_TRSM_ROWS; i < w->n_trsm; i++) w->trsm[i].chan = fol ? b->ch_below : -1;
    }
    int par_lim = 0;
    const int hp = h / 2;
    if (hp >= 1 && c->follow) {
      const int par = p->tree[hp];
      if (c->nblk_of[par] > 0 && (c->pb[par][0].nb + CHOL_NB - 1) / CHOL_NB <= CHOL_FOLLOW_MAXT && c->count[BIDX(p, par, s)] > 0) {
        par_lim = c->pb[par][0].nb;
// ... 13 lines not shown
      const int anc = p->tree[ha];
      if (BIDX(p, anc, s) < 0) continue;
      push_block_rows(c, anc, s, ha == hp ? par_lim : 0, p->sep_size[anc], diag, dinv, nb, ld, colbase, b->c_prog, -1);
    }
    if (c->sw_of[s] < c->bw_of[s] && w->n_trsm > t_rest) {
      b->ns_rest = w->n_trsm - t_rest; b->ch_rest = new_ctr(P, b->ns_rest);
      for (int e = 1; e < nt; e++) new_ctr(P, b->ns_rest);
      for (int i = t_rest; i < w->n_trsm; i++) w->trsm[i].chan = b->ch_rest;
    }
    B->cur_band = 0;
    b->n_groups = emit_trsm_jobs(c, s, b, t0);
    c->pg->ctr_total[b->c_strips] = b->n_groups;
  }
}
static void emit_next_block_followers(prog_ctx *c, int st)
{
  const plan_t *p = c->p;
  for (int q = 0; q < c->nh; q++) {
    const int s = p->tree[c->hs[q]];
    if (st + 1 >= c->nblk_of[s] || c->pb[s][st].ch_below < 0) continue;
    const pblock *b = &c->pb[s][st];
    const int ld = p->panel_ld[s];
    ext_item *items = NULL; int nit = 0, capit = 0;
    const int64_t e_off = p->panel_off[s] + (b->c0 + b->nb) + (int64_t)b->c0 * ld;
    const int nb1 = c->pb[s][st + 1].nb, nt = (b->nb + CHOL_NB - 1) / CHOL_NB;
    int bt = 0;
    if (c->o.follow_tail_split > 0 && (nb1 + CHOL_NB - 1) / CHOL_NB > CHOL_FOLLOW_ALL_MAXT && nt > c->o.follow_tail_split) bt = nt - c->o.follow_tail_split;
    if (bt > 0 && c->sky[s]) {
      int fmin = 1 << 20;
      for (int i = (b->c0 + b->nb) / CHOL_NB; i * CHOL_NB < b->c0 + b->nb + nb1; i++) if (c->sky[s][i] < fmin) fmin = c->sky[s][i];
      if (fmin - b->c0 / CHOL_NB >= bt) bt = 0;
    }
    int early = 0;
    if (bt > 0) {
      const early_src es = { e_off, ld, bt * CHOL_NB, b->ch_below + bt - 1, b->ns_below };
      early = emit_early_cells(c, p->panel_off[s] + (b->c0 + b->nb) + (int64_t)(b->c0 + b->nb) * ld, ld, nb1, BIDX(p, s, s), &es, 1);
    }
    const int ef = c->pg->n_ext;
    push_ext_items(&items, &nit, &capit, e_off, ld, b->nb, b->ch_below, b->ns_below, 0, bt);
    for (int i = 0; i < nit; i++) add_ext(&c->P, items[i].x);
    free(items);
    emit_potrf_job(c, s, st + 1, ef, early);
  }
}
static void emit_fast_parent_update(prog_ctx *c, int s, const pblock *b, int blk_par, int plim, int cols)
{
  const plan_t *p = c->p;
  chol_level_work *w = c->w;
  builder *B = &c->B;
  const int ld = p->panel_ld[s], c0 = b->c0, nb = b->nb, kf0 = w->n_task, ntl = (nb + CHOL_NB - 1) / CHOL_NB;
  const int64_t colbase = (int64_t)c0 * ld, x_piv = p->panel_off[s] + (c0 + nb) + colbase;
  B->cur_blk = blk_par;
  block_runs it = block_runs_of(p, blk_par, 0, plim, c->snap, c->first, c->count);
  for (int row, rows; block_runs_next(&it, &row, &rows);) {
    const int sb = w->n_src;
    for (int ch = 0; ch * EARLY_CHUNK < ntl; ch++) {
      const int col0 = ch * EARLY_CHUNK * CHOL_NB, kc = nb - col0 < EARLY_CHUNK * CHOL_NB ? nb - col0 : EARLY_CHUNK * CHOL_NB;
      chol_upd_src sa = { chol_block_row(it.Bk, row) + colbase + (int64_t)col0 * ld, x_piv + (int64_t)col0 * ld, ld, ld, kc, 0, c->o.staged ? 2 * ch + 2 : 0, 0 };
      push_src(B, sa);
    }
    push_tasks(B, chol_block_row(it.Bk, row) + (int64_t)(c0 + nb) * ld, ld, rows, cols, 0, sb, w->n_src);
  }
  flush_targets(B);
  wait_src ws[2 * 32]; int nws = 0;
  for (int ch = 0; ch * EARLY_CHUNK < ntl && nws < 62; ch++) {
    const int last = (ch + 1) * EARLY_CHUNK < ntl ? (ch + 1) * EARLY_CHUNK - 1 : ntl - 1;
    const wait_src x0 = { b->ch_par + last, b->ns_par, 0, 0 }, x1 = { b->ch_below + last, b->ns_below, 0, 0 };
    ws[nws++] = x0; ws[nws++] = x1;
  }
  emit_update_jobs(c, kf0, w->n_task, ws, nws, c->o.staged);
}
static void emit_trailing_update(prog_ctx *c, int st)
{
  const plan_t *p = c->p;
  chol_level_work *w = c->w;
// ... 47 lines not shown
      const int ba = BIDX(p, p->tree[ha], s);
      if (ba < 0) continue;
      block_runs it = block_runs_of(p, ba, (fine && ha == hpp) ? par_lim : 0, 1 << 30, c->snap, c->first, c->count);
      for (int row, rows; block_runs_next(&it, &row, &rows);) {
        chol_upd_src sa = { chol_block_row(it.Bk, row) + colbase, x_piv, ld, ld, nb, 0, 0, 0 };
        const int si = push_src(B, sa);
        push_tasks(B, chol_block_row(it.Bk, row) + (int64_t)(c0 + nb) * ld, ld, rows, below, 0, si, si + 1);
      }
    }
    flush_targets(B);
    const wait_src strips = { b->c_strips, b->n_groups, 0, 0 };
    emit_update_jobs(c, k0, w->n_task, &strips, 1, 0);
  }
}
static void emit_parent_followers(prog_ctx *c)
{
  const plan_t *p = c->p;
  memset(c->follow_lim, 0, p->nblk * sizeof(int));
  if (!c->follow) return;
  for (int hp = (1 << c->level) / 2; hp <= ((1 << (c->level + 1)) - 1) / 2; hp++) {
    const int par = p->tree[hp];
    if (c->nblk_of[par] == 0 || c->pb[par][0].emitted || c->count[BIDX(p, par, par)] == 0) continue;
    int kids[2] = { p->tree[2 * hp], p->tree[2 * hp + 1] };
    if (p->sep_size[kids[0]] > p->sep_size[kids[1]]) { const int t = kids[0]; kids[0] = kids[1]; kids[1] = t; }
    const int ef = c->pg->n_ext;
    int all = 1;
    for (int k = 0; k < 2; k++)
      for (int st = 0; st < c->nblk_of[kids[k]]; st++)
        if (c->count[BIDX(p, par, kids[k])] > 0 && c->pb[kids[k]][st].ch_par < 0) all = 0;
    if (!all) continue;
    ext_item *items = NULL; int nit = 0, capit = 0;
    const int lim = c->pb[par][0].nb, wide = c->o.follow_tail > 0 && (lim + CHOL_NB - 1) / CHOL_NB > CHOL_FOLLOW_ALL_MAXT;
    early_src es[2 * 32]; int nes = 0;
    for (int k = 0; k < 2; k++) {
      int total = 0;
      for (int st = 0; st < c->nblk_of[kids[k]]; st++) total += (c->pb[kids[k]][st].nb + CHOL_NB - 1) / CHOL_NB;
      const int bt = wide && total > c->o.follow_tail ? total - c->o.follow_tail : 0;
      int before = 0;
      for (int st = 0; st < c->nblk_of[kids[k]]; st++) {
        const pblock *b = &c->pb[kids[k]][st];
        const int nt = (b->nb + CHOL_NB - 1) / CHOL_NB;
        const int et = bt - before < 0 ? 0 : bt - before > nt ? nt : bt - before;
        if (b->ch_par >= 0) {
          if (et > 0 && nes < 64) { const early_src e1 = { b->par_off, p->panel_ld[kids[k]], et * CHOL_NB < b->nb ? et * CHOL_NB : b->nb, b->ch_par + et - 1, b->ns_par }; es[nes++] = e1; }
          push_ext_items(&items, &nit, &capit, b->par_off, p->panel_ld[kids[k]], b->nb, b->ch_par, b->ns_par, c->est_start[kids[k]] + before, et);
        }
        before += nt;
      }
    }
    int early = 0;
    if (nes > 0) {
      const chol_block *Bp = &p->blk[BIDX(p, par, par)];
      early = emit_early_cells(c, Bp->off, Bp->ld, lim, BIDX(p, par, par), es, nes);
    }
    qsort(items, nit, sizeof(ext_item), cmp_ext_item);
    for (int i = 0; i < nit; i++) add_ext(&c->P, items[i].x);
    free(items);
    if (c->pg->n_ext == ef) continue;
    c->follow_lim[BIDX(p, par, par)] = c->pb[par][0].nb;
    emit_potrf_job(c, par, 0, ef, early);
  }
}
typedef struct { int i, e, prio; } blk_range;
static blk_range *urgent_block_ranges(const prog_ctx *c, int k0, int *n_out)
{
  const plan_t *p = c->p;
  const chol_level_work *w = c->w;
  const int L = p->levels;
  int nrg = 0, caprg = 64;
  blk_range *rg = malloc(caprg * sizeof(blk_range));
  for (int i = k0; i < w->n_task;) {
    int e = i + 1;
    while (e < w->n_task && w->task[e].blk == w->task[i].blk) e++;
    const chol_block *Bc = &p->blk[w->task[i].blk];
    if (nrg == caprg) { caprg *= 2; rg = realloc(rg, caprg * sizeof(blk_range)); }
    rg[nrg].i = i; rg[nrg].e = e;
    rg[nrg].prio = (L - p->level_of[Bc->c]) * 4 * L + (Bc->r == Bc->c ? 0 : 1 + (p->level_of[Bc->c] - p->level_of[Bc->r]));
    nrg++;
    i = e;
  }
  for (int a = 1; a < nrg; a++) {
    blk_range t = rg[a];
    int b = a - 1;
    while (b >= 0 && rg[b].prio > t.prio) { rg[b + 1] = rg[b]; b--; }
    rg[b + 1] = t;
  }
  *n_out = nrg;
  return rg;
}
static wait_src *target_wait_list(const prog_ctx *c, int col_sep, int *n_out)
{
  const plan_t *p = c->p;
  const int hpar = p->heap_of[col_sep], dl = c->level - p->level_of[col_sep];
// ... 68 lines not shown
int chol_build_program(const plan_t *p, const chol_sched_opts *opts, chol_level_work *w, chol_program *pg)
{
  memset(w, 0, sizeof *w);
  memset(pg, 0, sizeof *pg);
  w->level = -1;
  chol_sched_opts dflt;
  if (!opts) { chol_sched_opts_default(&dflt); opts = &dflt; }
  prog_ctx c;
  int rc = prog_ctx_init(&c, p, opts, w, pg);
  for (int level = p->levels - 1; level >= 0 && !rc; level--) {
    prog_begin_level(&c, level);
    for (int st = 0; st < c.steps; st++) {
      emit_plain_potrf_jobs(&c, st);
      emit_step_trsm_jobs(&c, st);
      emit_next_block_followers(&c, st);
      emit_trailing_update(&c, st);
    }
    if (level == 0) break;
    emit_parent_followers(&c);
    rc = emit_level_extend_add(&c);
    if (w->n_task > PROG_MAX_TASKS && !rc) { chol_set_error("program launch: more than %d update tasks", PROG_MAX_TASKS); rc = CHOLAMD_ERR_ARG; }
  }
  if (!rc && w->n_task_mt > 0) { chol_set_error("program launch: macro-tile update phases"); rc = CHOLAMD_ERR_ARG; }
  if (!rc && w->n_task > PROG_MAX_TASKS) { chol_set_error("program launch: %d update tasks", w->n_task); rc = CHOLAMD_ERR_ARG; }
  if (!rc) for (int s = 1; s <= p->nsep; s++) { pg->ctr_total[c.c_upd[s]] = c.cnt_upd[s]; pg->ctr_total[c.c_updd[s]] = c.cnt_updd[s]; if (c.P.c_updp) pg->ctr_total[c.P.c_updp[s]] = c.P.cnt_updp[s]; }
  prog_ctx_free(&c);
  if (rc) { chol_level_work_free(w); chol_program_free(pg); }
  return rc;
}


typedef struct { int64_t a, b, c, d; } quad;
static int cmp_quad(const void *x, const void *y) { return memcmp(x, y, sizeof(quad)); }
int chol_program_check(const plan_t *p, const chol_sched_opts *opts, int workers)
{
  chol_level_work w;
  chol_program g;
  int rc = chol_build_program(p, opts, &w, &g);
  if (rc) return rc;
  rc = chol_program_check_built(p, opts, workers, &w, &g);
  chol_level_work_free(&w);
  chol_program_free(&g);
  return rc;
}
int chol_program_check_built(const plan_t *p, const chol_sched_opts *opts, int workers, const chol_level_work *wp, const chol_program *gp)
{
  const chol_level_work w = *wp;
  const chol_program g = *gp;
  int rc = 0;
  int *val = calloc(g.n_ctr > 0 ? g.n_ctr : 1, sizeof(int));
  char *state = calloc(g.n_job > 0 ? g.n_job : 1, 1);
  int next = 0, running = 0, done = 0;
  while (done < g.n_job && !rc) {
    while (running < workers && next < g.n_job) { state[next++] = 1; running++; }
    int progressed = 0;
    for (int j = 0; j < next; j++) {
      if (state[j] != 1) continue;
      const chol_job *jb = &g.job[j];
      int ok = 1;
      for (int q = 0; q < jb->n_wait && ok; q++) {
        const chol_wait *wt = &g.wait[jb->wait_first + q];
        if (wt->ctr < 0 || wt->ctr >= g.n_ctr || wt->value > g.ctr_total[wt->ctr]) { chol_set_error("program job %d waits for %d on counter %d (total %d)", j, wt->value, wt->ctr, wt->ctr >= 0 && wt->ctr < g.n_ctr ? g.ctr_total[wt->ctr] : -1); rc = CHOLAMD_ERR_ARG; ok = 0; break; }
        if (val[wt->ctr] < wt->value) ok = 0;
      }
      if (rc) break;
      if (jb->kind == CHOL_JOB_POTRF && jb->n_ext > 0) {
        int at = 0;
        while (at < jb->mode && at < jb->n_ext) at += chol_follow_round(at, jb->n_ext, (w.potrf[jb->first].n + CHOL_NB - 1) / CHOL_NB);
        if (at != jb->mode) { chol_set_error("program job %d adds its own tiles at item %d of %d: not the start of a round", j, jb->mode, jb->n_ext); rc = CHOLAMD_ERR_ARG; break; }
      }
      if (ok && jb->kind == CHOL_JOB_POTRF)
        for (int x = 0; x < jb->n_ext && ok; x++) {
          const chol_ext *e = &g.ext[jb->ext_first + x];
          if (val[e->ctr] < e->need) ok = 0;
        }
      if (ok && jb->kind == CHOL_JOB_TRSM && val[w.trsm[jb->first].flag] < g.ctr_total[w.trsm[jb->first].flag]) ok = 0;
      if (!ok) continue;
      if (jb->kind == CHOL_JOB_POTRF) val[w.potrf[jb->first].ctr] = g.ctr_total[w.potrf[jb->first].ctr];
      if (jb->kind == CHOL_JOB_TRSM)
        for (int i = jb->first; i < jb->first + jb->n; i++)
          if (w.trsm[i].chan >= 0 && w.trsm[i].m > 0)
            for (int t = 0; t < (w.trsm[i].n + CHOL_NB - 1) / CHOL_NB; t++) val[w.trsm[i].chan + t]++;
      for (int q = 0; q < 2; q++) if (jb->sig[q] >= 0) val[jb->sig[q]] += jb->sig_add;
      state[j] = 2; running--; done++; progressed = 1;
    }
    if (!rc && !progressed && (running == workers || next == g.n_job)) {
      int j = 0;
      while (j < next && state[j] != 1) j++;
      chol_set_error("program dead-locks with %d resident workgroups: job %d (kind %d) can never run; %d of %d jobs done", workers, j, j < g.n_job ? g.job[j].kind : -1, done, g.n_job);
      rc = CHOLAMD_ERR_ARG;
    }
  }
  for (int c = 0; c < g.n_ctr && !rc; c++)
    if (val[c] != g.ctr_total[c]) { chol_set_error("program counter %d ends at %d, total %d", c, val[c], g.ctr_total[c]); rc = CHOLAMD_ERR_ARG; }
  free(val); free(state);
  if (!rc) {
    quad *a = NULL, *b = NULL;
    int64_t na = 0, nb = 0, ca = 0, cb = 0;
#define PUSHQ(V_, N_, C_, A_, B_, C2_, D_) do { if (N_ == C_) { C_ = C_ ? 2 * C_ : 4096; V_ = realloc(V_, C_ * sizeof(quad)); } quad q_ = { A_, B_, C2_, D_ }; V_[N_++] = q_; } while (0)
    for (int l = 0; l < p->levels && !rc; l++) {
      chol_level_work lw;
      chol_sched_opts lo = *opts; lo.leaf_envelope = 0;
      rc = chol_build_level_work(p, &lo, l, 0, 1, &lw);
      if (rc) break;
      for (int i = 0; i < lw.n_potrf; i++) for (int ct = 0; ct * CHOL_NB < lw.potrf[i].n; ct++) for (int r = ct * CHOL_NB; r < lw.potrf[i].n; r++) PUSHQ(a, na, ca, -1, lw.potrf[i].a_off + r + (int64_t)ct * CHOL_NB * lw.potrf[i].lda, 0, 0);
      for (int i = 0; i < lw.n_trsm; i++) for (int r = 0; r < lw.trsm[i].m; r++) for (int ct = 0; ct * CHOL_NB < lw.trsm[i].n; ct++) PUSHQ(a, na, ca, -1, lw.trsm[i].b_off + r + (int64_t)ct * CHOL_NB * lw.trsm[i].ldb, 0, 0);
      chol_level_work_free(&lw);
    }
    for (int i = 0; i < w.n_potrf; i++) for (int ct = 0; ct * CHOL_NB < w.potrf[i].n; ct++) for (int r = ct * CHOL_NB; r < w.potrf[i].n; r++) PUSHQ(b, nb, cb, -1, w.potrf[i].a_off + r + (int64_t)ct * CHOL_NB * w.potrf[i].lda, 0, 0);
    for (int i = 0; i < w.n_trsm; i++) for (int r = 0; r < w.trsm[i].m; r++) for (int ct = 0; ct * CHOL_NB < w.trsm[i].n; ct++) PUSHQ(b, nb, cb, -1, w.trsm[i].b_off + r + (int64_t)ct * CHOL_NB * w.trsm[i].ldb, 0, 0);
#undef PUSHQ
    if (!rc) {
      qsort(a, na, sizeof(quad), cmp_quad);
      qsort(b, nb, sizeof(quad), cmp_quad);
      if (na != nb || (na > 0 && memcmp(a, b, na * sizeof(quad)))) { chol_set_error("program pivot blocks / TRSM rows differ from the level lists (%lld vs %lld items)", (long long)nb, (long long)na); rc = CHOLAMD_ERR_ARG; }
    }
    free(a); free(b);
  }
  return rc;
}
int cholamd_plan_program_check(const cholamd_plan *p, int follow, int workers)
{
  chol_sched_opts o;
  chol_sched_opts_default(&o);
  o.follow = follow;
  return chol_program_check(p, &o, workers);
}
int cholamd_plan_program_check_opts(const cholamd_plan *p, int follow_tail, int split_min, int split_nb, int workers)
{
  chol_sched_opts o;
  chol_sched_opts_from_env(&o);
  if (follow_tail >= 0) o.follow_tail = follow_tail;
  if (split_min >= 0) o.split_min = split_min;
  if (split_nb >= 0) o.split_nb = split_nb;
  return chol_program_check(p, &o, workers);
}
int cholamd_plan_program_check_follow(const cholamd_plan *p, int follow_tail, int follow_tail_split, int follow_own, int split_min, int split_nb, int workers)
{
  chol_sched_opts o;
  chol_sched_opts_from_env(&o);
  if (follow_tail >= 0) o.follow_tail = follow_tail;
  if (follow_tail_split >= 0) o.follow_tail_split = follow_tail_split;
  if (follow_own >= 0) o.follow_own = follow_own;
  if (split_min >= 0) o.split_min = split_min;
  if (split_nb >= 0) o.split_nb = split_nb;
  return chol_program_check(p, &o, workers);
}
int64_t cholamd_plan_program_jobs(const cholamd_plan *p, int follow, int64_t cap, int *out)
{
  chol_sched_opts o;
  chol_sched_opts_default(&o);
  o.follow = follow;
  chol_level_work w; chol_program g;
  if (chol_build_program(p, &o, &w, &g)) return -1;
  const int64_t need = (int64_t)8 * g.n_job + (int64_t)3 * g.n_wait + 1;
  if (cap >= need) {
    int64_t k = 0;
    for (int j = 0; j < g.n_job; j++) {
      const chol_job *jb = &g.job[j];
      int a = 0, b = 0;
      if (jb->kind == CHOL_JOB_POTRF) { a = w.potrf[jb->first].sep; b = w.potrf[jb->first].col0; }
      else if (jb->kind == CHOL_JOB_TRSM) { for (int i = 0; i < w.n_potrf; i++) if (w.potrf[i].ctr == w.trsm[jb->first].flag) { a = w.potrf[i].sep; b = w.potrf[i].col0; } }
      else { a = p->blk[w.task[jb->first].blk].c; b = p->blk[w.task[jb->first].blk].r; }
      out[k++] = jb->kind; out[k++] = a; out[k++] = b; out[k++] = jb->first; out[k++] = jb->n; out[k++] = jb->sig[0]; out[k++] = jb->kind == CHOL_JOB_TRSM ? w.trsm[jb->first].chan : jb->sig[1]; out[k++] = jb->n_wait;
    }
    for (int j = 0; j < g.n_job; j++)
      for (int q = 0; q < g.job[j].n_wait; q++) { out[k++] = j; out[k++] = g.wait[g.job[j].wait_first + q].ctr; out[k++] = g.wait[g.job[j].wait_first + q].value; }
    out[k++] = g.n_job;
  }
  chol_level_work_free(&w); chol_program_free(&g);
  return need;
}
int cholamd_follow_rounds(int n_ext, int tile_columns, int cap, int *rounds_out, int *own_at_out)
{
  int n = 0;
  for (int i = 0; i < n_ext; i += chol_follow_round(i, n_ext, tile_columns), n++)
    if (n < cap && rounds_out) rounds_out[n] = chol_follow_round(i, n_ext, tile_columns);
  if (own_at_out) *own_at_out = chol_follow_own_at(n_ext, tile_columns);
  return n;
}
int64_t cholamd_plan_program_followers(const cholamd_plan *p, int64_t cap, int *out)
{
  chol_sched_opts o;
  chol_sched_opts_default(&o);
  chol_level_work w; chol_program g;
  if (chol_build_program(p, &o, &w, &g)) return -1;
  int64_t n = 0;
  for (int j = 0; j < g.n_job; j++) {
    const chol_job *jb = &g.job[j];
    if (jb->kind != CHOL_JOB_POTRF || jb->n_ext <= 0) continue;
    if (4 * n + 3 < cap) { out[4 * n] = j; out[4 * n + 1] = jb->n_ext; out[4 * n + 2] = (w.potrf[jb->first].n + CHOL_NB - 1) / CHOL_NB; out[4 * n + 3] = jb->n_wait; }
    n++;
  }
  chol_level_work_free(&w); chol_program_free(&g);
  return n;
}
int64_t cholamd_plan_program_follow_own(const cholamd_plan *p, int follow_tail, int follow_tail_split, int follow_own, int split_min, int split_nb, int64_t cap, int *out)
{
  chol_sched_opts o;
  chol_sched_opts_default(&o);
  if (follow_tail >= 0) o.follow_tail = follow_tail;
  if (follow_tail_split >= 0) o.follow_tail_split = follow_tail_split;
  if (follow_own >= 0) o.follow_own = follow_own;
  if (split_min >= 0) o.split_min = split_min;
  if (split_nb >= 0) o.split_nb = split_nb;
  chol_level_work w; chol_program g;
  if (chol_build_program(p, &o, &w, &g)) return -1;
  int64_t n = 0;
  for (int j = 0; j < g.n_job; j++) {
    const chol_job *jb = &g.job[j];
    if (jb->kind != CHOL_JOB_POTRF || jb->n_ext <= 0) continue;
    if (5 * n + 4 < cap) { out[5 * n] = j; out[5 * n + 1] = jb->n_ext; out[5 * n + 2] = (w.potrf[jb->first].n + CHOL_NB - 1) / CHOL_NB; out[5 * n + 3] = jb->mode; out[5 * n + 4] = jb->n_wait; }
    n++;
  }
  chol_level_work_free(&w); chol_program_free(&g);
  return n;
}
typedef struct { int job, add; } hz_sig;
int cholamd_plan_program_hazards(const cholamd_plan *p, int follow_tail, int follow_tail_split, int follow_own, int split_min, int split_nb, int out[4])
{
  chol_sched_opts o;
  chol_sched_opts_default(&o);
  if (follow_tail >= 0) o.follow_tail = follow_tail;
  if (follow_tail_split >= 0) o.follow_tail_split = follow_tail_split;
  if (follow_own >= 0) o.follow_own = follow_own;
  if (split_min >= 0) o.split_min = split_min;
  if (split_nb >= 0) o.split_nb = split_nb;
  chol_level_work w; chol_program g;
  int rc = chol_build_program(p, &o, &w, &g);
  if (rc) return rc;
  const int nj = g.n_job, nw = (nj + 63) / 64;
  int *ns = calloc(g.n_ctr + 1, sizeof(int)), *first = calloc(g.n_ctr + 2, sizeof(int));
  hz_sig *sg = NULL;
  for (int pass = 0; pass < 2; pass++) {
    if (pass) { for (int c = 0; c < g.n_ctr; c++) { first[c + 1] = first[c] + ns[c]; ns[c] = 0; } sg = malloc((first[g.n_ctr] + 1) * sizeof(hz_sig)); }
#define HZ_SIG(C_, J_, ADD_) do { if (pass) { hz_sig s_ = { J_, ADD_ }; sg[first[C_] + ns[C_]] = s_; } ns[C_]++; } while (0)
    for (int j = 0; j < nj; j++) {
      const chol_job *jb = &g.job[j];
      if (jb->kind == CHOL_JOB_POTRF) HZ_SIG(w.potrf[jb->first].ctr, j, g.ctr_total[w.potrf[jb->first].ctr]);
      if (jb->kind == CHOL_JOB_TRSM)
        for (int t = 0; t < (w.trsm[jb->first].n + CHOL_NB - 1) / CHOL_NB; t++) {
          int add = 0;
          for (int i = jb->first; i < jb->first + jb->n; i++) add += w.trsm[i].chan >= 0 && w.trsm[i].m > 0;
          if (add > 0) HZ_SIG(w.trsm[jb->first].chan + t, j, add);
        }
      for (int q = 0; q < 2; q++) if (jb->sig[q] >= 0 && jb->sig_add > 0) HZ_SIG(jb->sig[q], j, jb->sig_add);
    }
#undef HZ_SIG
  }
  int nwt = 0;
  for (int j = 0; j < nj; j++) nwt += g.job[j].n_wait + (g.job[j].kind == CHOL_JOB_POTRF ? g.job[j].n_ext : g.job[j].kind == CHOL_JOB_TRSM ? 1 : 0);
  typedef struct { int job, ctr, value, gating; } hz_wait;
  hz_wait *wt = malloc((nwt + 1) * sizeof(hz_wait));
  int *nwc = calloc(g.n_ctr + 1, sizeof(int)), *wfirst = calloc(g.n_ctr + 2, sizeof(int)), *wof = malloc((nwt + 1) * sizeof(int));
  nwt = 0;
  for (int j = 0; j < nj; j++) {
    const chol_job *jb = &g.job[j];
    for (int q = 0; q < jb->n_wait; q++) { hz_wait x = { j, g.wait[jb->wait_first + q].ctr, g.wait[jb->wait_first + q].value, jb->kind != CHOL_JOB_UPDATE || q < jb->n_pre }; wt[nwt++] = x; }
    if (jb->kind == CHOL_JOB_POTRF) for (int q = 0; q < jb->n_ext; q++) { hz_wait x = { j, g.ext[jb->ext_first + q].ctr, g.ext[jb->ext_first + q].need, 1 }; wt[nwt++] = x; }
    if (jb->kind == CHOL_JOB_TRSM) { hz_wait x = { j, w.trsm[jb->first].flag, 1, 1 }; wt[nwt++] = x; }
  }
  for (int i = 0; i < nwt; i++) nwc[wt[i].ctr]++;
// ... 2 lines not shown
  uint64_t *pre = calloc((size_t)nj * nw + 1, sizeof(uint64_t)), *start = calloc((size_t)nj * nw + 1, sizeof(uint64_t));
  int *reqv = malloc((first[g.n_ctr] + 1) * sizeof(int));
#define HZ_HAS(S_, J_, A_) ((S_[(size_t)(J_) * nw + (A_) / 64] >> ((A_) % 64)) & 1)
  for (int changed = 1, sweep = 0; changed && sweep < 64; sweep++) {
    changed = 0;
    for (int c = 0; c < g.n_ctr; c++) {
      for (int y = first[c]; y < first[c + 1]; y++) {
        int m = 0;
        for (int z = wfirst[c]; z < wfirst[c + 1]; z++) {
          const hz_wait *x = &wt[wof[z]];
          if (x->value > m && (x->job == sg[y].job || HZ_HAS(pre, sg[y].job, x->job))) m = x->value;
        }
        reqv[y] = m;
      }
      for (int z = wfirst[c]; z < wfirst[c + 1]; z++) {
        const hz_wait *x = &wt[wof[z]];
        uint64_t *pj = pre + (size_t)x->job * nw, *sj = start + (size_t)x->job * nw;
        for (int a = first[c]; a < first[c + 1]; a++) {
          const int A = sg[a].job;
          if (HZ_HAS(pre, x->job, A) && (!x->gating || HZ_HAS(start, x->job, A))) continue;
          int f = 0;
          for (int y = first[c]; y < first[c + 1] && f < x->value; y++) if (sg[y].job != A && reqv[y] < x->value && !HZ_HAS(pre, sg[y].job, A)) f += sg[y].add;
          if (f >= x->value) continue;
          const uint64_t *pa = pre + (size_t)A * nw;
          for (int k = 0; k < nw; k++) {
            const uint64_t add = pa[k] | (k == A / 64 ? (uint64_t)1 << (A % 64) : 0);
            if (add & ~pj[k]) { pj[k] |= add; changed = 1; }
            if (x->gating && (add & ~sj[k])) { sj[k] |= add; changed = 1; }
          }
        }
      }
    }
  }
  free(wt); free(nwc); free(wfirst); free(wof); free(reqv);
  int *last = malloc((size_t)(p->arena > 0 ? p->arena : 1) * sizeof(int));
  for (int64_t e = 0; e < p->arena; e++) last[e] = -1;
  uint64_t *seen = calloc((size_t)nj * nw + 1, sizeof(uint64_t));
  out[0] = out[1] = 0; out[2] = out[3] = -1;
  for (int j = 0; j < nj; j++) {
    const chol_job *jb = &g.job[j];
    if (jb->kind != CHOL_JOB_UPDATE) continue;
    for (int t = jb->first; t < jb->first + jb->n; t++) {
      const chol_upd_task *tk = &w.task[t];
      for (int col = 0; col < tk->nv; col++)
        for (int r = 0; r < tk->mv; r++) {
          const int64_t e = tk->c_off + r + (int64_t)col * tk->ldc;
          if (e < 0 || e >= p->arena) { chol_set_error("program task %d writes outside the arena", t); rc = CHOLAMD_ERR_ARG; continue; }
          const int a = last[e];
          last[e] = j;
          if (a < 0 || a == j || HZ_HAS(seen, j, a)) continue;
          seen[(size_t)j * nw + a / 64] |= (uint64_t)1 << (a % 64);
          out[0]++;
          if (!HZ_HAS(start, j, a)) { if (out[1]++ == 0) { out[2] = a; out[3] = j; } }
        }
    }
  }
#undef HZ_HAS
  free(last); free(seen); free(pre); free(start); free(sg); free(ns); free(first);
  chol_level_work_free(&w); chol_program_free(&g);
  return rc;
}
int cholamd_plan_program_counts(const cholamd_plan *p, int follow, int out[6])
{
  chol_sched_opts o;
  chol_sched_opts_default(&o);
  o.follow = follow;
  chol_level_work w; chol_program g;
  int rc = chol_build_program(p, &o, &w, &g);
  if (rc) return rc;
  int nf = 0;
  for (int j = 0; j < g.n_job; j++) nf += g.job[j].kind == CHOL_JOB_POTRF && g.job[j].n_ext > 0;
  out[0] = g.n_job; out[1] = nf; out[2] = w.n_task; out[3] = w.n_trsm; out[4] = g.n_ctr; out[5] = g.n_ext;
  chol_level_work_free(&w); chol_program_free(&g);
  return 0;
}

static int level_work_volume(const cholamd_plan *p, const chol_sched_opts *o, int level, int rank, int world, int64_t out[6], int64_t counts[3])
{
  chol_level_work w;
  int rc = chol_build_level_work(p, o, level, rank, world, &w);
  if (rc) return rc;
  memset(out, 0, 6 * sizeof(int64_t));
  if (counts) { counts[0] = w.n_task; counts[1] = w.n_task_mt; counts[2] = 0; for (int i = 0; i < w.n_trsm; i++) counts[2] += w.trsm[i].m > 0; }
  for (int i = 0; i < w.n_potrf; i++) out[0] += w.potrf[i].n;
  for (int i = 0; i < w.n_trsm; i++) out[1] += (int64_t)w.trsm[i].m * w.trsm[i].n;
  for (int pass = 0; pass < 2; pass++) {
    const chol_upd_task *T = pass ? w.task_mt : w.task;
    const int nt = pass ? w.n_task_mt : w.n_task;
    for (int i = 0; i < nt; i++) {
      const chol_upd_task *t = &T[i];
      int64_t full = 0;
      for (int c = 0; c < t->nv; c++) full += t->lower ? (t->mv - c > 0 ? t->mv - c : 0) : t->mv;
      for (int q = t->src_begin; q < t->src_end; q++) {
        const chol_upd_src *sd = &w.src[q];
// ... 149 lines not shown
```

cholesky_amd/plan.py:

```python
import ctypes as C
import os

import numpy as np

from ._lib import Filled, Op, check, load

OP_NAMES = ("POTRF", "TRSM", "SYRK", "GEMM")


class Plan:
    def __init__(self, matrix_file=None, separator_file=None, clusters_file=None, _handle=None):
        self.L = load()
        if _handle is not None:
            self.h = _handle
        else:
            h = C.c_void_p()
            check(self.L.cholamd_plan_create(os.fsencode(matrix_file), os.fsencode(separator_file), os.fsencode(clusters_file), C.byref(h)),
                  "cholamd_plan_create")
            self.h = h
        g = self.L
        self.n = g.cholamd_plan_n(self.h)
        self.nz = g.cholamd_plan_nz(self.h)
        self.levels = g.cholamd_plan_levels(self.h)
        self.nsep = g.cholamd_plan_num_separators(self.h)
# ... 202 lines not shown
            check(m, "cholamd_plan_selinv_front")
        pos = np.zeros(max(m, 1), dtype=np.int32)
        off = np.zeros((max(m, 1), max(m, 1)), dtype=np.int64)
        m2 = self.L.cholamd_plan_selinv_front(self.h, int(sep), int(block), m, cols.ctypes.data, pos.ctypes.data, off.ctypes.data)
        if m2 < 0:
            check(m2, "cholamd_plan_selinv_front")
        return int(cols[0]), int(cols[1]), pos[:m], off[:m, :m]

    def exchange_pieces(self, world, dist_top=2):
        out = np.zeros((4096, 4), dtype=np.int64)
        n = self.L.cholamd_plan_exchange_pieces(self.h, world, dist_top, len(out), out.ctypes.data)
        if n < 0:
            check(n, "cholamd_plan_exchange_pieces")
        return out[:min(n, len(out))]

    def level_work_volume(self, level, rank=0, world=1, dist_top=2):
        out = np.zeros(6, dtype=np.int64)
        check(self.L.cholamd_plan_level_work_volume(self.h, level, rank, world, dist_top, out.ctypes.data), "cholamd_plan_level_work_volume")
        return tuple(int(v) for v in out)

    def level_work_volume_opts(self, level, merge_targets=1, mt_min_tiles=-1):
        out = np.zeros(9, dtype=np.int64)
        check(self.L.cholamd_plan_level_work_volume_opts(self.h, level, int(merge_targets), int(mt_min_tiles), out.ctypes.data), "cholamd_plan_level_work_volume_opts")
        return tuple(int(v) for v in out)

    def level_mt_fill(self, level):
        out = np.zeros(4, dtype=np.int64)
        check(self.L.cholamd_plan_level_mt_fill(self.h, level, out.ctypes.data), "cholamd_plan_level_mt_fill")
        return tuple(int(v) for v in out)

    def program_check(self, follow=True, workers=64):
        check(self.L.cholamd_plan_program_check(self.h, int(follow), int(workers)), "cholamd_plan_program_check")

    def program_check_opts(self, follow_tail=-1, split_min=-1, split_nb=-1, workers=64, follow_tail_split=-1, follow_own=-1):
        check(self.L.cholamd_plan_program_check_follow(self.h, follow_tail, follow_tail_split, follow_own, split_min, split_nb, int(workers)),
              "cholamd_plan_program_check_follow")

    def program_follow_own(self, follow_own=-1, follow_tail=-1, follow_tail_split=-1, split_min=-1, split_nb=-1):
        n = self.L.cholamd_plan_program_follow_own(self.h, follow_tail, follow_tail_split, follow_own, split_min, split_nb, 0, None)
        if n < 0:
            check(int(n), "cholamd_plan_program_follow_own")
        buf = np.zeros(5 * n + 5, dtype=np.int32)
        self.L.cholamd_plan_program_follow_own(self.h, follow_tail, follow_tail_split, follow_own, split_min, split_nb, buf.size, buf.ctypes.data)
        return [dict(zip(("job", "n_ext", "T", "own_at", "n_wait"), (int(v) for v in buf[5 * i:5 * i + 5]))) for i in range(n)]

    def program_hazards(self, follow_own=-1, follow_tail=-1, follow_tail_split=-1, split_min=-1, split_nb=-1):
        out = np.zeros(4, dtype=np.int32)
        check(self.L.cholamd_plan_program_hazards(self.h, follow_tail, follow_tail_split, follow_own, split_min, split_nb, out.ctypes.data), "cholamd_plan_program_hazards")
        return int(out[0]), int(out[1]), (int(out[2]), int(out[3]))

    def program_counts(self, follow=True):
        out = np.zeros(6, dtype=np.int32)
        check(self.L.cholamd_plan_program_counts(self.h, int(follow), out.ctypes.data), "cholamd_plan_program_counts")
        return dict(zip(("jobs", "followers", "tasks", "strips", "counters", "followed_panels"), (int(v) for v in out)))

    def program_jobs(self, follow=True):
        need = self.L.cholamd_plan_program_jobs(self.h, int(follow), 0, None)
        buf = np.zeros(need, dtype=np.int32)
        self.L.cholamd_plan_program_jobs(self.h, int(follow), need, buf.ctypes.data)
        nj = int(buf[-1])
        return buf[:8 * nj].reshape(nj, 8), buf[8 * nj:-1].reshape(-1, 3)

    SCHUR_RECORD = 7

    def schur_size(self, k):
        m = self.L.cholamd_plan_schur_size(self.h, int(k))
        if m < 0:
            check(m, "cholamd_plan_schur_size")
        return m

    def schur_dofs(self, k):
        m = self.schur_size(k)
        out = np.zeros(max(m, 1), dtype=np.int32)
        check(min(self.L.cholamd_plan_schur_dofs(self.h, int(k), out.ctypes.data), 0), "cholamd_plan_schur_dofs")
        return out[:m]

    def schur_list(self, k):
# ... 261 lines not shown
```

include/cholamd.h:

```cpp
#ifndef CHOLAMD_H
#define CHOLAMD_H

#include <stdint.h>
#include <stdio.h>

#ifdef __cplusplus
extern "C" {
#endif

#define CHOLAMD_OK 0
#define CHOLAMD_ERR_IO (-1)
#define CHOLAMD_ERR_FORMAT (-2)
#define CHOLAMD_ERR_INVARIANT (-3)
#define CHOLAMD_ERR_ARG (-4)
#define CHOLAMD_ERR_NO_DEVICE (-5)
#define CHOLAMD_ERR_HIP (-6)
#define CHOLAMD_ERR_NOMEM (-7)
#define CHOLAMD_ERR_COMM (-9)
#define CHOLAMD_ERR_STALL (-8)

const char *cholamd_last_error(void);
const char *cholamd_version(void);

typedef char MM_typecode[4];
// ... 60 lines not shown
const char *cholamd_plan_banner(const cholamd_plan *p);
void cholamd_plan_perm(const cholamd_plan *p, int *out);
void cholamd_plan_sep_sizes(const cholamd_plan *p, int *out);
void cholamd_plan_sep_offsets(const cholamd_plan *p, int *out);
void cholamd_plan_tree(const cholamd_plan *p, int *out);
void cholamd_plan_blocks(const cholamd_plan *p, int *out);
int64_t cholamd_plan_snapshot_count(const cholamd_plan *p, int interval_lbl);
void cholamd_plan_snapshot(const cholamd_plan *p, int interval_lbl, cholamd_filled *out);
int64_t cholamd_plan_num_ops(const cholamd_plan *p);
void cholamd_plan_ops(const cholamd_plan *p, cholamd_op *out);
void cholamd_plan_counts(const cholamd_plan *p, int level , int64_t calls[4], double flops[4]);
double cholamd_plan_flops(const cholamd_plan *p);
int64_t cholamd_plan_nnz_a(const cholamd_plan *p);
int64_t cholamd_plan_nnz_l(const cholamd_plan *p);
int64_t cholamd_plan_nnz_tiles(const cholamd_plan *p);
double cholamd_plan_fmin(const cholamd_plan *p);
int64_t cholamd_plan_alg_bytes(const cholamd_plan *p);

int cholamd_plan_fill_host(const cholamd_plan *p, double *arena);
int cholamd_plan_entries(const cholamd_plan *p, int *row, int *col);
int cholamd_plan_value_map(const cholamd_plan *p, int64_t *src_out);
int cholamd_plan_fill_host_values(const cholamd_plan *p, const double *vals, int64_t count, double *arena);
int cholamd_plan_diag_list(const cholamd_plan *p, int64_t *a_off, int *cols, int *lda, int *x_off, int *sep, int *prefix);
int cholamd_plan_fill_host_part(const cholamd_plan *p, double *arena, int rank, int world, int64_t *tail_offset_out);
int cholamd_plan_level_work_counts(const cholamd_plan *p, int level, int rank, int world, int out[4]);
int cholamd_plan_level_work_volume_opts(const cholamd_plan *p, int level, int merge_targets, int mt_min_tiles, int64_t out[9]);
int cholamd_plan_level_mt_fill(const cholamd_plan *p, int level, int64_t out[4]);
int cholamd_plan_level_work_volume(const cholamd_plan *p, int level, int rank, int world, int dist_top, int64_t out[6]);
int cholamd_plan_exchange_volume(const cholamd_plan *p, int rank, int world, int dist_top, int64_t out[4]);
int cholamd_plan_exchange_pieces(const cholamd_plan *p, int world, int dist_top, int max, int64_t (*out)[4]);
int cholamd_plan_program_check(const cholamd_plan *p, int follow, int workers);
int cholamd_plan_program_check_opts(const cholamd_plan *p, int follow_tail, int split_min, int split_nb, int workers);
int cholamd_plan_program_check_follow(const cholamd_plan *p, int follow_tail, int follow_tail_split, int follow_own, int split_min, int split_nb, int workers);
int cholamd_plan_program_counts(const cholamd_plan *p, int follow, int out[6]);
int cholamd_follow_rounds(int n_ext, int tile_columns, int cap, int *rounds_out, int *own_at_out);
int64_t cholamd_plan_program_followers(const cholamd_plan *p, int64_t cap, int *out);
int64_t cholamd_plan_program_follow_own(const cholamd_plan *p, int follow_tail, int follow_tail_split, int follow_own, int split_min, int split_nb, int64_t cap, int *out);
int cholamd_plan_program_hazards(const cholamd_plan *p, int follow_tail, int follow_tail_split, int follow_own, int split_min, int split_nb, int out[4]);
int64_t cholamd_plan_program_jobs(const cholamd_plan *p, int follow, int64_t cap, int *out);
int cholamd_plan_arena_to_dense(const cholamd_plan *p, const double *arena, double *dense);
int cholamd_plan_write_matrix(const cholamd_plan *p, const double *arena, const char *file, int full_precision);
int cholamd_write_solution(const char *file, const double *x, int n, int full_precision);
int cholamd_plan_write_debug_log(const cholamd_plan *p, FILE *f);
int cholamd_plan_write_debug_header(const cholamd_plan *p, FILE *f);
int cholamd_plan_write_blocks_txt(const cholamd_plan *p, const double *arena, const char *file, const char *header);
int cholamd_plan_ntiles_at_level(const cholamd_plan *p, int sep, int level);

typedef struct cholamd_problem cholamd_problem;
int cholamd_generate_laplacian(int nx, int ny, int nz, int levels, int tile, cholamd_problem **out);
void cholamd_problem_destroy(cholamd_problem *g);
int cholamd_problem_n(const cholamd_problem *g);
int cholamd_problem_nz(const cholamd_problem *g);
int cholamd_problem_write(const cholamd_problem *g, const char *prefix);
int cholamd_plan_create_from_problem(const cholamd_problem *g, cholamd_plan **out);
void cholamd_problem_rhs(const cholamd_problem *g, double *b);

typedef struct cholamd_device cholamd_device;

int cholamd_device_count(void);
int cholamd_device_create(const cholamd_plan *plan, int device_id, cholamd_device **out);
void cholamd_device_destroy(cholamd_device *d);
int cholamd_device_alloc(cholamd_device *d, int64_t doubles, double **dptr);
int cholamd_device_free(cholamd_device *d, double *dptr);
int cholamd_device_upload(cholamd_device *d, double *d_dst, const double *h_src, int64_t doubles, void *stream);
int cholamd_device_download(cholamd_device *d, double *h_dst, const double *d_src, int64_t doubles, void *stream);
int cholamd_device_sync(cholamd_device *d, void *stream);
int cholamd_device_fill(cholamd_device *d, double *d_arena, void *stream);
#define CHOLAMD_VALUES_NOCHECK 1
int cholamd_device_set_values(cholamd_device *d, const double *d_vals, int64_t count, int flags, void *stream);
int cholamd_device_values_status(cholamd_device *d, void *stream, int64_t out[4]);
int cholamd_factor(cholamd_device *d, double *d_arena, void *stream);
// ... 214 lines not shown
```

Baseline: 891.5 GF/s.

## Let POTRF followers start external rounds before leading column tiles finish

Adds a follow_cols mode where the POTRF follower splits its wait list. It waits on the first columns' dependency separately, at its own round, so external update rounds touching only narrow column ranges can proceed earlier. Narrow external sources load fewer columns, and the owned tiles are loaded and folded into the staging registers once those columns are ready. The scheduler, hazard checker and the Python and C APIs are extended to compute and verify this. It adds kernel complexity and register pressure, plus a correctness risk if hazards are missed.

New measurement: 865.0 GF/s. 0.97x the previous value.

```diff
diff --git a/cholesky_amd/_lib.py b/cholesky_amd/_lib.py
--- a/cholesky_amd/_lib.py
+++ b/cholesky_amd/_lib.py
@@ -132,6 +132,10 @@
     L.cholamd_plan_program_follow_own.restype = i64
     L.cholamd_plan_program_check_follow.argtypes = [vp, ci, ci, ci, ci, ci, ci]
     L.cholamd_plan_program_hazards.argtypes = [vp, ci, ci, ci, ci, ci, vp]
+    L.cholamd_plan_program_check_cols.argtypes = [vp, ci, ci, ci, ci, ci, ci, ci]
+    L.cholamd_plan_program_hazards_cols.argtypes = [vp, ci, ci, ci, ci, ci, ci, vp]
+    L.cholamd_plan_program_follow_cols.argtypes = [vp, ci, ci, ci, ci, ci, ci, i64, vp]
+    L.cholamd_plan_program_follow_cols.restype = i64
     L.cholamd_factor_multi_f32.argtypes = [vp, vp, vp, ci, vp]
     L.cholamd_gather_factor_f32.argtypes = [vp, vp, ci, vp]
     L.cholamd_device_alloc.argtypes = [vp, i64, C.POINTER(vp)]
diff --git a/cholesky_amd/csrc/chol_api.cpp b/cholesky_amd/csrc/chol_api.cpp
--- a/cholesky_amd/csrc/chol_api.cpp
+++ b/cholesky_amd/csrc/chol_api.cpp
@@ -119,7 +119,7 @@
       int mx = 1;
       for (int t : tot) mx = t > mx ? t : mx;
       d->prog_epoch_limit = (1 << 30) / mx;
-      d->n_job = g.n_job; d->n_pctr = (int)tot.size(); d->prog_epoch = 0;
+      d->n_job = g.n_job; d->n_pctr = (int)tot.size(); d->prog_epoch = 0; d->prog_cols = g.cols;
       d->jobs_host.assign(g.job, g.job + g.n_job);
       if (!rc) rc = d->jobs.upload(g.job, (size_t)g.n_job);
       const chol_wait no_wait = { 0, 0 };
@@ -216,6 +216,7 @@
   else if (n == "follow_tail") d->opt.follow_tail = value;
   else if (n == "follow_tail_split") d->opt.follow_tail_split = value;
   else if (n == "follow_own") d->opt.follow_own = value < 0 ? 0 : value > 2 ? 2 : value;
+  else if (n == "follow_cols") d->opt.follow_cols = value < 0 ? 0 : value > 2 ? 2 : value;
   else if (n == "staged") d->opt.staged = value != 0;
   else if (n == "fine_upd") d->opt.fine_upd = value != 0;
   else if (n == "skyline") d->opt.skyline = value != 0;
@@ -454,7 +455,7 @@
   {
     scoped_timer t(d, st, 3, true);
     HIPCHK((hipError_t)chol_launch_program(d_arena, d->ws, d->jobs, d->n_job, d->pwaits, l.potrf, l.trsm, l.task, l.src, d->exts, d->pctr, d->pctr_total, d->prog_epoch,
-                                           d->pctr + d->n_pctr - 1, d->prog_epoch * (d->n_job + d->prog_grid), d->prog_grid, info_cur, info_next, d->trace, st));
+                                           d->pctr + d->n_pctr - 1, d->prog_epoch * (d->n_job + d->prog_grid), d->prog_grid, info_cur, info_next, d->trace, d->prog_cols, st));
   }
   d->prog_epoch++;
   return 0;
@@ -499,6 +500,7 @@
           for (unsigned long long i = 0; i < x[1] && i < 44; i++) if (x[2 + i]) fprintf(fp, " %llu:%.1f", i, (double)(x[2 + i] - t0) * 0.01);
         }
         if (kind == 0 && x[24]) { fprintf(fp, " | prologue (entry, LDS init, tables, slot tables read, columns 0-1 requested, tiles requested, columns 0-1 parked):"); const int ord[7] = { 0, 1, 2, 5, 6, 3, 4 }; for (int k = 0; k < 7; k++) fprintf(fp, " %.1f", x[24 + ord[k]] ? (double)(x[24 + ord[k]] - t0) * 0.01 : -1.0); }
+        if (kind == 0 && x[1]) fprintf(fp, " | columns 0-1 requested: %.1f | last round's barrier: %.1f", x[46] ? (double)(x[46] - t0) * 0.01 : -1.0, x[47] ? (double)(x[47] - t0) * 0.01 : -1.0);
         fprintf(fp, kind == 0 ? " | column started:" : " | POTRF column seen:");
         for (int k = 0; k < 24; k++) if (x[72 + k]) fprintf(fp, " %d:%.1f", k, (double)(x[72 + k] - t0) * 0.01);
         fprintf(fp, kind == 0 ? " | column published:" : " | column tile on the channel:");
diff --git a/cholesky_amd/csrc/chol_device.h b/cholesky_amd/csrc/chol_device.h
--- a/cholesky_amd/csrc/chol_device.h
+++ b/cholesky_amd/csrc/chol_device.h
@@ -111,6 +111,7 @@
   dev_buf<chol_job> jobs; dev_buf<chol_wait> pwaits; dev_buf<chol_ext> exts;
   dev_buf<int> pctr, pctr_total;
   int n_job = 0, n_pctr = 0, prog_grid = 0, prog_epoch = 0, prog_epoch_limit = 0;
+  int prog_cols = 0;
   bool prog_ready = false;
   unsigned long long *trace = nullptr;
   std::vector<chol_job> jobs_host;
diff --git a/cholesky_amd/csrc/chol_kernels.h b/cholesky_amd/csrc/chol_kernels.h
--- a/cholesky_amd/csrc/chol_kernels.h
+++ b/cholesky_amd/csrc/chol_kernels.h
@@ -16,7 +16,7 @@
                            int *info, int *progress, int progress_base, int *done, int done_target, hipStream_t st);
 int chol_launch_program(double *base, double *ws, const chol_job *jobs, int njobs, const chol_wait *waits, const chol_potrf_desc *pdescs, const chol_trsm_desc *tdescs,
                         const chol_upd_task *tasks, const chol_upd_src *srcs, const chol_ext *exts, int *ctr, const int *ctr_total, int epoch, int *head, int head_base,
-                        int grid, int *info, int *info_next, unsigned long long *trace, hipStream_t st);
+                        int grid, int *info, int *info_next, unsigned long long *trace, int cols, hipStream_t st);
 int chol_launch_trsm_w(double *base, const double *ws, const chol_trsm_desc *descs, int n, hipStream_t st);
 int chol_launch_trsm_wt(double *base, const double *ws, const chol_trsm_desc *descs, int n, hipStream_t st);
 int chol_launch_trsm_big(double *base, const double *ws, const chol_trsm_desc *descs, int n, hipStream_t st);
diff --git a/cholesky_amd/csrc/chol_kernels.hip b/cholesky_amd/csrc/chol_kernels.hip
--- a/cholesky_amd/csrc/chol_kernels.hip
+++ b/cholesky_amd/csrc/chol_kernels.hip
@@ -747,7 +747,8 @@
   return !__ballot(!ok);
 }
 struct follow_args { const chol_ext *ext; int n_ext; const int *ctr; const int *ctr_total; int epoch; const chol_wait *wl; int n_wl; unsigned long long *stamp, *xstamp;
-                     int own_at;  };
+                     int own_at;
+                      };
 __device__ __forceinline__ int ext_ready(const follow_args &f, int from, int lane)
 {
   bool ok = true;
@@ -759,20 +760,29 @@
   const int lead = notok ? __builtin_ctzll(notok) : 64;
   return min(from + lead, f.n_ext);
 }
-template <bool UPD, bool PUB, bool TR = false>
+template <bool UPD, bool PUB, bool TR = false, bool COLS = false>
 __device__ __forceinline__ void follow_external(const double *__restrict__ base, const follow_args f, int T, int n, double *sE, d4 (&tile)[11], d4 (&stage)[3],
                                                 const int (&ijp)[12], int w, int lane, int tid, int *info, const double *A, int lda, int r15, int g, int *sReady)
 {
   const int lp = lane;
   int buf = 0;
   int ready = 0, ng = 0;
+  int nar = 0;
   double va[FOLLOW_LOADS], vb[FOLLOW_LOADS];
 #ifndef FOLLOW_OWN_SLEEP
 #define FOLLOW_OWN_SLEEP 4
 #endif
+#ifndef EXT_SLEEP
+#define EXT_SLEEP 4
+#endif
   static_assert(CHOL_FOLLOW_PAIR_MAXT == RR_MAXT, "a pair of followed column tiles shares one LDS buffer of RR_MAXT tiles");
-  const int own_at = f.own_at;
-  const bool own_last = f.n_wl > 0 && own_at >= f.n_ext;
+  const int own_at = COLS ? f.own_at & 0xffff : f.own_at;
+  const int a_at = COLS ? (f.own_at >> 16) - 1 : -1;
+  const bool cols = COLS && a_at >= 0;
+  const chol_wait *const wlb = f.wl + (cols ? 1 : 0);
+  const int n_wlb = f.n_wl - (cols ? 1 : 0);
+  bool a_ok = false;
+  const bool own_last = n_wlb > 0 && own_at >= f.n_ext;
   bool own_ok = false;
   int own_c = 0, own_need = 0, own_v = 0;
   const bool own_look = !UPD && own_last && f.n_wl <= 64;
@@ -785,7 +795,7 @@
     _Pragma("unroll") for (int it = 0; it < FOLLOW_LOADS; ++it) {                                                    \
       const int idx = tid + it * RR_THREADS;                                                                         \
       const int row = (idx >> 8) * TS + (idx & 15), col = (idx >> 4) & 15;                                           \
-      V_[it] = (idx < T * TS * TS && row < n && col < xl_.ncol) ? gload<true>(&src_[row + (int64_t)col * xl_.ld]) : 0.0; \
+      V_[it] = (idx < T * TS * TS && row < n && col < (COLS ? CHOL_EXT_NCOL(xl_.ncol) : xl_.ncol)) ? gload<true>(&src_[row + (int64_t)col * xl_.ld]) : 0.0; \
     }                                                                                                                \
   }
 #define EXT_LOAD_ROUND(I_)                                                                                           \
@@ -793,12 +803,13 @@
     EXT_LOAD(I_, va);                                                                                                \
     ng = EXT_ROUND(I_);                                                                                              \
     if (ng == 2) { EXT_LOAD((I_) + 1, vb); }                                                                         \
-  }
-#define EXT_UPDATE(acc_, ti_, tj_)                                                                                   \
+    if (COLS) nar = (f.ext[I_].ncol & CHOL_EXT_NARROW ? 1 : 0) | (ng == 2 && (f.ext[(I_) + 1].ncol & CHOL_EXT_NARROW) ? 2 : 0);  \
+  }
+#define EXT_UPDATE(acc_, ti_, tj_, s0_, two_)                                                                        \
   {                                                                                                                  \
     _Pragma("unroll") for (int st = 0; st < 4; ++st)                                                                 \
-      acc_ = __builtin_amdgcn_mfma_f64_16x16x4f64(sB[(tj_) * (TS * TS) + st * 64 + lp], -sB[(ti_) * (TS * TS) + st * 64 + lp], acc_, 0, 0, 0); \
-    if (G == 2) {                                                                                                    \
+      acc_ = __builtin_amdgcn_mfma_f64_16x16x4f64(s0_[(tj_) * (TS * TS) + st * 64 + lp], -s0_[(ti_) * (TS * TS) + st * 64 + lp], acc_, 0, 0, 0); \
+    if (two_) {                                                                                                      \
       _Pragma("unroll") for (int st = 0; st < 4; ++st)                                                               \
         acc_ = __builtin_amdgcn_mfma_f64_16x16x4f64(sB2[(tj_) * (TS * TS) + st * 64 + lp], -sB2[(ti_) * (TS * TS) + st * 64 + lp], acc_, 0, 0, 0); \
     }                                                                                                                \
@@ -806,7 +817,7 @@
 #define OWN_TILES()                                                                                                  \
   {                                                                                                                  \
   \
-      if (!UPD) wait_list<FOLLOW_OWN_SLEEP>(f.wl, f.n_wl, f.ctr, f.ctr_total, f.epoch, lane, info);  \
+      if (!UPD) wait_list<FOLLOW_OWN_SLEEP>(wlb, n_wlb, f.ctr, f.ctr_total, f.epoch, lane, info);  \
       if (TR && !UPD && f.xstamp && lane == 0) f.xstamp[0] = __builtin_amdgcn_s_memrealtime(); \
       lds_barrier(); \
       if (UPD) { \
@@ -826,35 +837,64 @@
  \
   }
   for (int i = 0; i < f.n_ext;) {
-    if (f.n_wl > 0 && i == own_at) OWN_TILES();
-    if (ng == 0) {
-      const int need = i + EXT_ROUND(i);
-      if (ready < need) {
-        if (!UPD) {
-          ready = ext_ready(f, i, lane);
-          for (int it = 0; ready < need; ++it) {
-            if (it >= (1 << 24)) { if (lane == 0) report_stall(info); ready = f.n_ext; break; }
-#ifndef EXT_SLEEP
-#define EXT_SLEEP 4
-#endif
-            __builtin_amdgcn_s_sleep(EXT_SLEEP);
-            ready = ext_ready(f, i, lane);
-          }
-          if (lane == 0) __hip_atomic_store(sReady, ready, __ATOMIC_RELAXED, __HIP_MEMORY_SCOPE_WORKGROUP);
-        } else {
-          for (int it = 0;; ++it) {
-            ready = __builtin_amdgcn_readfirstlane(__hip_atomic_load(sReady, __ATOMIC_RELAXED, __HIP_MEMORY_SCOPE_WORKGROUP));
-            if (ready >= need) break;
-            if (it >= (1 << 25)) { if (lane == 0) report_stall(info); ready = f.n_ext; break; }
-            __builtin_amdgcn_s_sleep(2);
-          }
+    if (n_wlb > 0 && i == own_at) OWN_TILES();
+#define EXT_ACQUIRE(I_)                                                                                              \
+  {                                                                                                                  \
+    const int need = (I_) + EXT_ROUND(I_);                                                                           \
+    if (ready < need) {                                                                                              \
+       \
+       \
+       \
+      if (!UPD) {                                                                                                    \
+        ready = ext_ready(f, I_, lane);                                                                              \
+        for (int it = 0; ready < need; ++it) {  \
+          if (it >= (1 << 24)) { if (lane == 0) report_stall(info); ready = f.n_ext; break; }  \
+          __builtin_amdgcn_s_sleep(EXT_SLEEP);                                                                       \
+          ready = ext_ready(f, I_, lane);                                                                            \
+        }                                                                                                            \
+        if (lane == 0) __hip_atomic_store(sReady, ready, __ATOMIC_RELAXED, __HIP_MEMORY_SCOPE_WORKGROUP);            \
+      } else {                                                                                                       \
+        for (int it = 0;; ++it) {                                                                                    \
+          ready = __builtin_amdgcn_readfirstlane(__hip_atomic_load(sReady, __ATOMIC_RELAXED, __HIP_MEMORY_SCOPE_WORKGROUP)); \
+          if (ready >= need) break;                                                                                  \
+          if (it >= (1 << 25)) { if (lane == 0) report_stall(info); ready = f.n_ext; break; }                        \
+          __builtin_amdgcn_s_sleep(2);                                                                               \
+        }                                                                                                            \
+      }                                                                                                              \
+    }                                                                                                                \
+    EXT_LOAD_ROUND(I_);                                                                                              \
+  }
+    if (cols && i == a_at) {
+      if (!UPD) {
+        if (!a_ok) wait_list<FOLLOW_OWN_SLEEP>(f.wl, 1, f.ctr, f.ctr_total, f.epoch, lane, info);
+        a_ok = true;
+        if (TR && f.xstamp && lane == 0) f.xstamp[46] = __builtin_amdgcn_s_memrealtime();
+        if (lane == 0) __hip_atomic_store(sReady + 4, 1, __ATOMIC_RELAXED, __HIP_MEMORY_SCOPE_WORKGROUP);
+      } else {
+        for (int it = 0;; ++it) {
+          if (__builtin_amdgcn_readfirstlane(__hip_atomic_load(sReady + 4, __ATOMIC_RELAXED, __HIP_MEMORY_SCOPE_WORKGROUP)) != 0) break;
+          if (it >= (1 << 25)) { if (lane == 0) report_stall(info); break; }
+          __builtin_amdgcn_s_sleep(2);
         }
-      }
-      EXT_LOAD_ROUND(i);
-    }
+        int rx = r15, gx = g;
+        asm volatile("" : "+v"(rx), "+v"(gx));
+        d4 own[3];
+#pragma unroll
+        for (int it = 0; it < 3; ++it) {
+          const int u = min(w + it * RR_NW, 2 * T - 2);
+          own[it] = load_tile<PUB>(A, lda, n, u < T ? u : u - T + 1, u < T ? 0 : 1, rx, gx);
+        }
+        if (ng == 0) EXT_ACQUIRE(i);
+#pragma unroll
+        for (int it = 0; it < 3; ++it) stage[it] += own[it];
+      }
+    }
+    if (ng == 0) EXT_ACQUIRE(i);
     const int G = ng;
+    const bool full0 = !COLS || !(nar & 1), full1 = G == 2 && (!COLS || !(nar & 2));
     if (TR && !UPD && f.xstamp && lane == 0 && i < 44) { f.xstamp[1] = f.n_ext; f.xstamp[2 + i] = __builtin_amdgcn_s_memrealtime(); }
     double *sB = sE + buf * (RR_MAXT * TS * TS), *sB2 = sB + T * TS * TS;
+    const double *sF = !COLS || full0 ? sB : sB2;
 #pragma unroll
     for (int it = 0; it < FOLLOW_LOADS; ++it) {
       const int idx = tid + it * RR_THREADS;
@@ -872,16 +912,23 @@
     const bool look = own_look && !own_ok;
     if (look && lane < f.n_wl) own_v = __hip_atomic_load(&f.ctr[own_c], __ATOMIC_RELAXED, __HIP_MEMORY_SCOPE_AGENT);
     lds_barrier();
-    if (look) own_ok = !__ballot(lane < f.n_wl && own_v < own_need);
+    if (TR && !UPD && f.xstamp && lane == 0) f.xstamp[47] = __builtin_amdgcn_s_memrealtime();
+    if (look) {
+      const unsigned long long nok = __ballot(lane < f.n_wl && own_v < own_need);
+      own_ok = !(cols ? nok >> 1 : nok);
+      if (cols && !(nok & 1)) a_ok = true;
+    }
     if (UPD) {
 #pragma unroll
       for (int it = 0; it < 3; ++it) {
         const int u = w + it * RR_NW;
-        if (u < 2 * T - 1) { const int tj = u < T ? 0 : 1, ti = u < T ? u : u - T + 1; EXT_UPDATE(stage[it], ti, tj); }
-      }
-#pragma unroll
-      for (int s = 0; s < FOLLOW_SLOTS; ++s)
-        if (ijp[s] != 0xffff) { const int ti = ijp[s] & 0xff, tj = ijp[s] >> 8; EXT_UPDATE(tile[s], ti, tj); }
+        if (u < 2 * T - 1) { const int tj = u < T ? 0 : 1, ti = u < T ? u : u - T + 1; EXT_UPDATE(stage[it], ti, tj, sB, G == 2); }
+      }
+      if (!COLS || full0 || full1) {
+#pragma unroll
+        for (int s = 0; s < FOLLOW_SLOTS; ++s)
+          if (ijp[s] != 0xffff) { const int ti = ijp[s] & 0xff, tj = ijp[s] >> 8; EXT_UPDATE(tile[s], ti, tj, sF, COLS ? full0 && full1 : G == 2); }
+      }
     }
     buf ^= 1;
     if (polled) {
@@ -895,16 +942,18 @@
     i = j;
   }
   if (own_last) {
-    if (!UPD && !own_ok) wait_list<FOLLOW_OWN_SLEEP>(f.wl, f.n_wl, f.ctr, f.ctr_total, f.epoch, lane, info);
+    if (!UPD && !own_ok) wait_list<FOLLOW_OWN_SLEEP>(wlb, n_wlb, f.ctr, f.ctr_total, f.epoch, lane, info);
     if (TR && !UPD && f.xstamp && lane == 0) f.xstamp[0] = __builtin_amdgcn_s_memrealtime();
     lds_barrier();
     if (UPD) {
       int rx = r15, gx = g;
       asm volatile("" : "+v"(rx), "+v"(gx));
-#pragma unroll
-      for (int it = 0; it < 3; ++it) {
-        const int u = min(w + it * RR_NW, 2 * T - 2);
-        tile[FOLLOW_SLOTS + it] = load_tile<PUB>(A, lda, n, u < T ? u : u - T + 1, u < T ? 0 : 1, rx, gx);
+      if (!cols) {
+#pragma unroll
+        for (int it = 0; it < 3; ++it) {
+          const int u = min(w + it * RR_NW, 2 * T - 2);
+          tile[FOLLOW_SLOTS + it] = load_tile<PUB>(A, lda, n, u < T ? u : u - T + 1, u < T ? 0 : 1, rx, gx);
+        }
       }
 #pragma unroll
       for (int s = 0; s < FOLLOW_SLOTS; ++s) {
@@ -915,13 +964,14 @@
     }
   }
 #undef OWN_TILES
+#undef EXT_ACQUIRE
 #undef EXT_LOAD_ROUND
 #undef EXT_ROUND
 #undef EXT_UPDATE
 #undef EXT_LOAD
 }
 
-template <bool PUB, bool FOLLOW = false, bool TR = false>
+template <bool PUB, bool FOLLOW = false, bool TR = false, bool COLS = false>
 __device__ __forceinline__ void potrf_rr_body(double *__restrict__ base, double *__restrict__ ws, const chol_potrf_desc d, int *__restrict__ info,
                                               int *__restrict__ progress, int progress_base, double *smem, const unsigned char *__restrict__ sky, const follow_args fa = follow_args(), const int tid = threadIdx.x)
 {
@@ -955,7 +1005,8 @@
 #define PSTAMP(i_) do { if (TR && fa.xstamp && fa.n_ext == 0 && tid == 64) fa.xstamp[24 + (i_)] = __builtin_amdgcn_s_memrealtime(); } while (0)
   PSTAMP(0);
   d4 stage[3];
-  const bool own_pending = FOLLOW && fa.n_ext > 0 && fa.n_wl > 0 && fa.own_at >= fa.n_ext;
+  const bool fcols = COLS && (fa.own_at >> 16) > 0;
+  const bool own_pending = FOLLOW && fa.n_ext > 0 && fa.n_wl - (fcols ? 1 : 0) > 0 && (COLS ? fa.own_at & 0xffff : fa.own_at) >= fa.n_ext;
   const bool stage_early = !(FOLLOW && fa.n_ext > 0) && wave != 0;
   if (stage_early) {
 #pragma unroll
@@ -1007,7 +1058,7 @@
     if (FOLLOW && fa.n_ext > 0) {
       d4 tdummy[RR_RSLOTS], sdummy[3];
       int idummy[RR_SLOTS];
-      follow_external<false, PUB, TR>(base, fa, T, n, smem + RR_OFF_SOL, tdummy, sdummy, idummy, 0, lane, tid, info, A, lda, r15, g, &sFlag[5]);
+      follow_external<false, PUB, TR, COLS>(base, fa, T, n, smem + RR_OFF_SOL, tdummy, sdummy, idummy, 0, lane, tid, info, A, lda, r15, g, &sFlag[5]);
       lds_barrier();
       if (TR && fa.stamp && lane == 0) *fa.stamp = __builtin_amdgcn_s_memrealtime();
     }
@@ -1103,9 +1154,9 @@
         if (early && ijp[s] != 0xffff) v = load_tile<PUB>(A, lda, n, ijp[s] & 0xff, ijp[s] >> 8, r15, g);
         tile[s] = v;
       }
-      follow_external<true, PUB, TR>(base, fa, T, n, smem + RR_OFF_SOL, tile, stage, ijp, w, lane, tid, info, A, lda, r15, g, &sFlag[5]);
+      follow_external<true, PUB, TR, COLS>(base, fa, T, n, smem + RR_OFF_SOL, tile, stage, ijp, w, lane, tid, info, A, lda, r15, g, &sFlag[5]);
       lds_barrier();
-      if (own_pending) {
+      if (own_pending && !fcols) {
 #pragma unroll
         for (int it = 0; it < 3; ++it) stage[it] += tile[FOLLOW_SLOTS + it];
       }
@@ -1626,7 +1677,7 @@
 #define PROG_OFF_XFLAG (3 * RR_MAXT * TS * TS)
 static_assert(PROG_XFLAGS >= 4 * ((CHOL_RR_MAXN / TS + 3) / 4) && PROG_XFLAGS >= 4 * FUSED_SLOTS && PROG_OFF_XFLAG + (3 * PROG_XFLAGS + 1) / 2 <= RR_SMEM_DOUBLES, "the strips' slots and flags fit the image");
 static_assert(CHOL_RR_MAXN <= RR_MAXT * TS && CHOL_FUSE_MAXN <= CHOL_RR_MAXN, "one slot per column tile of the widest strip");
-template <bool TR>
+template <bool TR, bool COLS>
 __global__ __launch_bounds__(RR_THREADS) void k_program(double *__restrict__ base, double *__restrict__ ws, const chol_job *__restrict__ jobs, int njobs,
                                                         const chol_wait *__restrict__ waits, const chol_potrf_desc *__restrict__ pdescs,
                                                         const chol_trsm_desc *__restrict__ tdescs, const chol_upd_task *__restrict__ tasks,
@@ -1642,7 +1693,9 @@
 #ifdef TID_PLAIN
     int tid = threadIdx.x;
 #else
-    int tid = wave_id * 64 + (int)__builtin_amdgcn_mbcnt_hi(~0u, __builtin_amdgcn_mbcnt_lo(~0u, 0u));
+    unsigned lane0 = 0u;
+    asm volatile("" : "+v"(lane0));
+    int tid = wave_id * 64 + (int)__builtin_amdgcn_mbcnt_hi(~0u, __builtin_amdgcn_mbcnt_lo(~0u, lane0));
 #endif
     asm volatile("" : "+v"(tid));
     const int wave = wave_id;
@@ -1675,8 +1728,8 @@
     if (jb.kind == CHOL_JOB_POTRF) {
       const chol_potrf_desc pd = pdescs[jb.first];
       follow_args fa;
-      fa.ext = exts + jb.ext_first; fa.n_ext = jb.n_ext; fa.ctr = ctr; fa.ctr_total = ctr_total; fa.epoch = epoch; fa.wl = waits + jb.wait_first; fa.n_wl = jb.n_wait; fa.own_at = jb.mode; fa.stamp = TR && trace ? &trace[4 * j + 1] : nullptr; fa.xstamp = TR && trace ? &trace[4 * njobs + CHOL_TRACE_X * j] : nullptr;
-      potrf_rr_body<true, true, TR>(base, ws, pd, info, ctr + pd.ctr, epoch * ctr_total[pd.ctr], smem, pdescs[jb.first].sky, fa, tid);
+      fa.ext = exts + jb.ext_first; fa.n_ext = jb.n_ext; fa.ctr = ctr; fa.ctr_total = ctr_total; fa.epoch = epoch; fa.wl = waits + jb.wait_first; fa.n_wl = jb.n_wait; fa.own_at = COLS && jb.n_ext > 0 && jb.n_pre < 0 ? jb.mode | (-jb.n_pre) << 16 : jb.mode; fa.stamp = TR && trace ? &trace[4 * j + 1] : nullptr; fa.xstamp = TR && trace ? &trace[4 * njobs + CHOL_TRACE_X * j] : nullptr;
+      potrf_rr_body<true, true, TR, COLS>(base, ws, pd, info, ctr + pd.ctr, epoch * ctr_total[pd.ctr], smem, pdescs[jb.first].sky, fa, tid);
     } else if (jb.kind == CHOL_JOB_TRSM) {
       double (*sX)[RR_MAXT][TS * TS] = (double (*)[RR_MAXT][TS * TS])smem;
       chol_trsm_desc d = tdescs[jb.first + min(grp, jb.n - 1)];
@@ -2028,11 +2081,16 @@
 }
 int chol_launch_program(double *base, double *ws, const chol_job *jobs, int njobs, const chol_wait *waits, const chol_potrf_desc *pdescs, const chol_trsm_desc *tdescs,
                         const chol_upd_task *tasks, const chol_upd_src *srcs, const chol_ext *exts, int *ctr, const int *ctr_total, int epoch, int *head, int head_base,
-                        int grid, int *info, int *info_next, unsigned long long *trace, hipStream_t st)
+                        int grid, int *info, int *info_next, unsigned long long *trace, int cols, hipStream_t st)
 {
   if (njobs <= 0) return 0;
-  if (trace) hipLaunchKernelGGL(k_program<true>, dim3(grid), dim3(RR_THREADS), 0, st, base, ws, jobs, njobs, waits, pdescs, tdescs, tasks, srcs, exts, ctr, ctr_total, epoch, head, head_base, info, info_next, trace);
-  else hipLaunchKernelGGL(k_program<false>, dim3(grid), dim3(RR_THREADS), 0, st, base, ws, jobs, njobs, waits, pdescs, tdescs, tasks, srcs, exts, ctr, ctr_total, epoch, head, head_base, info, info_next, trace);
+  if (cols) {
+    if (trace) hipLaunchKernelGGL((k_program<true, true>), dim3(grid), dim3(RR_THREADS), 0, st, base, ws, jobs, njobs, waits, pdescs, tdescs, tasks, srcs, exts, ctr, ctr_total, epoch, head, head_base, info, info_next, trace);
+    else hipLaunchKernelGGL((k_program<false, true>), dim3(grid), dim3(RR_THREADS), 0, st, base, ws, jobs, njobs, waits, pdescs, tdescs, tasks, srcs, exts, ctr, ctr_total, epoch, head, head_base, info, info_next, trace);
+    return (int)hipGetLastError();
+  }
+  if (trace) hipLaunchKernelGGL((k_program<true, false>), dim3(grid), dim3(RR_THREADS), 0, st, base, ws, jobs, njobs, waits, pdescs, tdescs, tasks, srcs, exts, ctr, ctr_total, epoch, head, head_base, info, info_next, trace);
+  else hipLaunchKernelGGL((k_program<false, false>), dim3(grid), dim3(RR_THREADS), 0, st, base, ws, jobs, njobs, waits, pdescs, tdescs, tasks, srcs, exts, ctr, ctr_total, epoch, head, head_base, info, info_next, trace);
   return (int)hipGetLastError();
 }
 int chol_launch_trsm_w(double *base, const double *ws, const chol_trsm_desc *descs, int n, hipStream_t st)
diff --git a/cholesky_amd/csrc/chol_plan.h b/cholesky_amd/csrc/chol_plan.h
--- a/cholesky_amd/csrc/chol_plan.h
+++ b/cholesky_amd/csrc/chol_plan.h
@@ -149,6 +149,10 @@
 #define CHOL_FOLLOW_SINGLE_TAIL 0
 #define CHOL_FOLLOW_OWN_BEFORE 2
 #define CHOL_FOLLOW_OWN 1
+#define CHOL_FOLLOW_COLS 0
+#define CHOL_FOLLOW_COLS_N 2
+#define CHOL_EXT_NARROW 0x100
+#define CHOL_EXT_NCOL(x_) ((x_) & 0xff)
 #if defined(__HIPCC__)
 #define CHOL_HD __host__ __device__ __forceinline__
 #else
@@ -173,6 +177,7 @@
   int n_ext; chol_ext *ext;
   int n_ctr; int *ctr_total;
   int follow;
+  int cols;
 } chol_program;
 
 enum chol_phase_kind {
@@ -223,6 +228,7 @@
   int leaf_envelope;
   int super_blocks;
   int follow_own;
+  int follow_cols;
 } chol_sched_opts;
 #define CHOL_SUPER_BLOCKS 3
 #define CHOL_STAGE_CHUNK 0
diff --git a/cholesky_amd/csrc/chol_schedule.c b/cholesky_amd/csrc/chol_schedule.c
--- a/cholesky_amd/csrc/chol_schedule.c
+++ b/cholesky_amd/csrc/chol_schedule.c
@@ -90,7 +90,7 @@
 void chol_sched_opts_default(chol_sched_opts *o)
 {
   o->split_min = CHOL_SPLIT_MIN; o->split_nb = CHOL_SPLIT_NB; o->fuse = 1; o->fuse_update_max = CHOL_FUSE_UPDATE_MAX;
-  o->mt_min_tiles = CHOL_MT_MIN_TILES; o->trsm_wt_min = CHOL_TRSM_WT_MIN; o->trsm_group = 0; o->cells = 1; o->program = 1; o->follow = 1; o->super_blocks = CHOL_SUPER_BLOCKS; o->dist_top = 2; o->follow_tail = CHOL_FOLLOW_TAIL; o->follow_tail_split = CHOL_FOLLOW_TAIL; o->staged = 1; o->fine_upd = 1; o->skyline = 1; o->stage_chunk = CHOL_STAGE_CHUNK; o->merge_targets = 1; o->leaf_envelope = 1; o->follow_own = CHOL_FOLLOW_OWN;
+  o->mt_min_tiles = CHOL_MT_MIN_TILES; o->trsm_wt_min = CHOL_TRSM_WT_MIN; o->trsm_group = 0; o->cells = 1; o->program = 1; o->follow = 1; o->super_blocks = CHOL_SUPER_BLOCKS; o->dist_top = 2; o->follow_tail = CHOL_FOLLOW_TAIL; o->follow_tail_split = CHOL_FOLLOW_TAIL; o->staged = 1; o->fine_upd = 1; o->skyline = 1; o->stage_chunk = CHOL_STAGE_CHUNK; o->merge_targets = 1; o->leaf_envelope = 1; o->follow_own = CHOL_FOLLOW_OWN; o->follow_cols = CHOL_FOLLOW_COLS;
 }
 void chol_sched_opts_from_env(chol_sched_opts *o)
 {
@@ -109,6 +109,8 @@
   o->follow_tail = env_int("CHOLAMD_FOLLOW_TAIL", o->follow_tail);
   o->follow_tail_split = env_int("CHOLAMD_FOLLOW_TAIL_SPLIT", o->follow_tail_split);
   o->follow_own = env_int("CHOLAMD_FOLLOW_OWN", o->follow_own);
+  o->follow_cols = env_int("CHOLAMD_FOLLOW_COLS", o->follow_cols);
+  o->follow_cols = o->follow_cols < 0 ? 0 : o->follow_cols > 2 ? 2 : o->follow_cols;
   o->staged = !env_int("CHOLAMD_NO_STAGED", 0);
   o->fine_upd = !env_int("CHOLAMD_NO_FINE_UPD", 0);
   o->skyline = !env_int("CHOLAMD_NO_SKYLINE", 0);
@@ -826,12 +828,13 @@
   if (x->key != y->key) return x->key < y->key ? -1 : 1;
   return x->seq < y->seq ? -1 : (x->seq > y->seq);
 }
-static void push_ext_items(ext_item **items, int *n, int *cap, int64_t off, int ld, int k, int chan, int nstrip, int key0, int e_from)
+static void push_ext_items(ext_item **items, int *n, int *cap, int64_t off, int ld, int k, int chan, int nstrip, int key0, int e_from, int narrow_to)
 {
   for (int e = e_from; e * CHOL_NB < k; e++) {
     if (*n == *cap) { *cap = *cap ? 2 * *cap : 64; *items = realloc(*items, *cap * sizeof(ext_item)); }
     ext_item *it = &(*items)[(*n)];
     it->x.off = off + (int64_t)e * CHOL_NB * ld; it->x.ld = ld; it->x.ncol = k - e * CHOL_NB < CHOL_NB ? k - e * CHOL_NB : CHOL_NB;
+    if (e < narrow_to) it->x.ncol |= CHOL_EXT_NARROW;
     it->x.ctr = chan + e; it->x.need = nstrip;
     it->key = key0 + e; it->seq = *n;
     (*n)++;
@@ -1023,7 +1026,7 @@
 #ifndef EARLY_CHUNK
 #define EARLY_CHUNK 2
 #endif
-static int emit_early_cells(prog_ctx *c, int64_t c_off, int ldc, int lim, int blk, const early_src *es, int nes)
+static int emit_early_cells(prog_ctx *c, int64_t c_off, int ldc, int lim, int blk, const early_src *es, int nes, int j_from)
 {
   chol_level_work *w = c->w;
   builder *B = &c->B;
@@ -1044,12 +1047,12 @@
   const int staged = B->o->staged;
   const int k0 = w->n_task, Tl = (lim + CHOL_NB - 1) / CHOL_NB;
   for (int I = 0; I < Tl; I++)
-    for (int J = 0; J <= I; J++) {
+    for (int J = j_from; J <= I; J++) {
       const int sb = w->n_src;
       for (int z = 0; z < nst; z++) {
         const early_src *e = &es[ws[z].tag];
         const int col0 = ws[z].est * EARLY_CHUNK * CHOL_NB, kc = e->k - col0 < EARLY_CHUNK * CHOL_NB ? e->k - col0 : EARLY_CHUNK * CHOL_NB;
-        chol_upd_src sd = { e->off + CHOL_NB * I + (int64_t)col0 * e->ld, e->off + CHOL_NB * J + (int64_t)col0 * e->ld, e->ld, e->ld, kc, 0, staged ? z + 1 : 0, 0 };
+        chol_upd_src sd = { e->off + CHOL_NB * I + (int64_t)col0 * e->ld, e->off + CHOL_NB * J + (int64_t)col0 * e->ld, e->ld, e->ld, kc, 0, staged ? z + 1 : 0, 1 };
         push_src(B, sd);
       }
       if (w->n_task == B->cap_k) { B->cap_k = B->cap_k ? 2 * B->cap_k : 256; w->task = realloc(w->task, B->cap_k * sizeof(chol_upd_task)); }
@@ -1177,7 +1180,12 @@
     if (c->nblk_of[s] > c->steps) c->steps = c->nblk_of[s];
   }
 }
-static void emit_potrf_job(prog_ctx *c, int s, int st, int ext_first, int early)
+static int follow_cols_mode(const prog_ctx *c, int T, int early)
+{
+  return early && c->o.follow_own > 0 && T > CHOL_FOLLOW_ALL_MAXT && T > CHOL_FOLLOW_COLS_N
+         && (c->o.follow_cols >= 2 || (c->o.follow_cols == 1 && 2 * T <= CHOL_FOLLOW_PAIR_MAXT));
+}
+static void emit_potrf_job(prog_ctx *c, int s, int st, int ext_first, int early, int part_a)
 {
   const plan_t *p = c->p;
   chol_program *pg = c->pg;
@@ -1194,19 +1202,21 @@
   push_potrf(&c->B, pd);
   b->potrf = c->w->n_potrf - 1;
   const int wf = pg->n_wait;
+  if (part_a >= 0) { add_wait(&c->P, c->c_updd[s], 1 << 30); pg->wait[pg->n_wait - 1].value = part_a; }
   add_wait(&c->P, c->c_updd[s], c->cnt_updd[s]);
   chol_job *j = add_job(&c->P, CHOL_JOB_POTRF, b->potrf, 1, wf);
   j->ext_first = ext_first; j->n_ext = pg->n_ext - ext_first;
   if (j->n_ext > 0)
     j->mode = j->n_wait > 0 && (c->o.follow_own == 2 || (c->o.follow_own == 1 && early)) ? j->n_ext
               : chol_follow_own_at(j->n_ext, (b->nb + CHOL_NB - 1) / CHOL_NB);
+  if (part_a >= 0) { j->n_pre = -1 - chol_follow_own_at(j->n_ext, (b->nb + CHOL_NB - 1) / CHOL_NB); pg->cols++; }
   b->emitted = 1;
 }
 static void emit_plain_potrf_jobs(prog_ctx *c, int st)
 {
   for (int q = 0; q < c->nh; q++) {
     const int s = c->p->tree[c->hs[q]];
-    if (st < c->nblk_of[s] && !c->pb[s][st].emitted) emit_potrf_job(c, s, st, c->pg->n_ext, 0);
+    if (st < c->nblk_of[s] && !c->pb[s][st].emitted) emit_potrf_job(c, s, st, c->pg->n_ext, 0, -1);
   }
 }
 static void emit_step_trsm_jobs(prog_ctx *c, int st)
@@ -1286,15 +1296,17 @@
       if (fmin - b->c0 / CHOL_NB >= bt) bt = 0;
     }
     int early = 0;
+    const int cols = follow_cols_mode(c, (nb1 + CHOL_NB - 1) / CHOL_NB, bt > 0);
+    const int part_a = cols ? c->cnt_updd[s] : -1;
     if (bt > 0) {
       const early_src es = { e_off, ld, bt * CHOL_NB, b->ch_below + bt - 1, b->ns_below };
-      early = emit_early_cells(c, p->panel_off[s] + (b->c0 + b->nb) + (int64_t)(b->c0 + b->nb) * ld, ld, nb1, BIDX(p, s, s), &es, 1);
+      early = emit_early_cells(c, p->panel_off[s] + (b->c0 + b->nb) + (int64_t)(b->c0 + b->nb) * ld, ld, nb1, BIDX(p, s, s), &es, 1, cols ? CHOL_FOLLOW_COLS_N : 0);
     }
     const int ef = c->pg->n_ext;
-    push_ext_items(&items, &nit, &capit, e_off, ld, b->nb, b->ch_below, b->ns_below, 0, bt);
+    push_ext_items(&items, &nit, &capit, e_off, ld, b->nb, b->ch_below, b->ns_below, 0, cols ? 0 : bt, cols ? bt : 0);
     for (int i = 0; i < nit; i++) add_ext(&c->P, items[i].x);
     free(items);
-    emit_potrf_job(c, s, st + 1, ef, early);
+    emit_potrf_job(c, s, st + 1, ef, early, part_a);
   }
 }
 static void emit_fast_parent_update(prog_ctx *c, int s, const pblock *b, int blk_par, int plim, int cols)
@@ -1408,6 +1420,14 @@
     ext_item *items = NULL; int nit = 0, capit = 0;
     const int lim = c->pb[par][0].nb, wide = c->o.follow_tail > 0 && (lim + CHOL_NB - 1) / CHOL_NB > CHOL_FOLLOW_ALL_MAXT;
     early_src es[2 * 32]; int nes = 0;
+    int any_early = 0;
+    for (int k = 0; k < 2 && wide; k++) {
+      int total = 0, with_chan = 0;
+      for (int st = 0; st < c->nblk_of[kids[k]]; st++) { total += (c->pb[kids[k]][st].nb + CHOL_NB - 1) / CHOL_NB; with_chan |= c->pb[kids[k]][st].ch_par >= 0; }
+      if (with_chan && total > c->o.follow_tail) any_early = 1;
+    }
+    const int cols = follow_cols_mode(c, (lim + CHOL_NB - 1) / CHOL_NB, any_early);
+    const int part_a = cols ? c->cnt_updd[par] : -1;
     for (int k = 0; k < 2; k++) {
       int total = 0;
       for (int st = 0; st < c->nblk_of[kids[k]]; st++) total += (c->pb[kids[k]][st].nb + CHOL_NB - 1) / CHOL_NB;
@@ -1419,7 +1439,7 @@
         const int et = bt - before < 0 ? 0 : bt - before > nt ? nt : bt - before;
         if (b->ch_par >= 0) {
           if (et > 0 && nes < 64) { const early_src e1 = { b->par_off, p->panel_ld[kids[k]], et * CHOL_NB < b->nb ? et * CHOL_NB : b->nb, b->ch_par + et - 1, b->ns_par }; es[nes++] = e1; }
-          push_ext_items(&items, &nit, &capit, b->par_off, p->panel_ld[kids[k]], b->nb, b->ch_par, b->ns_par, c->est_start[kids[k]] + before, et);
+          push_ext_items(&items, &nit, &capit, b->par_off, p->panel_ld[kids[k]], b->nb, b->ch_par, b->ns_par, c->est_start[kids[k]] + before, cols ? 0 : et, cols ? et : 0);
         }
         before += nt;
       }
@@ -1427,14 +1447,14 @@
     int early = 0;
     if (nes > 0) {
       const chol_block *Bp = &p->blk[BIDX(p, par, par)];
-      early = emit_early_cells(c, Bp->off, Bp->ld, lim, BIDX(p, par, par), es, nes);
+      early = emit_early_cells(c, Bp->off, Bp->ld, lim, BIDX(p, par, par), es, nes, cols ? CHOL_FOLLOW_COLS_N : 0);
     }
     qsort(items, nit, sizeof(ext_item), cmp_ext_item);
     for (int i = 0; i < nit; i++) add_ext(&c->P, items[i].x);
     free(items);
     if (c->pg->n_ext == ef) continue;
     c->follow_lim[BIDX(p, par, par)] = c->pb[par][0].nb;
-    emit_potrf_job(c, par, 0, ef, early);
+    emit_potrf_job(c, par, 0, ef, early, early ? part_a : -1);
   }
 }
 typedef struct { int i, e, prio; } blk_range;
@@ -1569,6 +1589,81 @@
 
 typedef struct { int64_t a, b, c, d; } quad;
 static int cmp_quad(const void *x, const void *y) { return memcmp(x, y, sizeof(quad)); }
+typedef struct { int I, J; int64_t tile; } early_cell;
+static int *early_task_list(const chol_level_work *w, int *n_out)
+{
+  int n = 0;
+  int *l = malloc((w->n_task > 0 ? w->n_task : 1) * sizeof(int));
+  for (int t = 0; t < w->n_task; t++)
+    if (w->task[t].src_end > w->task[t].src_begin && w->src[w->task[t].src_begin].pad == 1) l[n++] = t;
+  *n_out = n;
+  return l;
+}
+static int64_t follower_early_cells(const chol_level_work *w, const int *et, int net, const chol_potrf_desc *pd, early_cell *out, int64_t cap)
+{
+  int64_t n = 0;
+  for (int z = 0; z < net; z++) {
+    const chol_upd_task *tk = &w->task[et[z]];
+    const int64_t rel = tk->c_off - pd->a_off;
+    if (rel < 0 || tk->ldc != pd->lda || rel / pd->lda >= pd->n || rel % pd->lda >= pd->n) continue;
+    const int ri = (int)(rel % pd->lda), rj = (int)(rel / pd->lda);
+    if (ri % CHOL_NB || rj % CHOL_NB || rj > ri) return -1;
+    for (int q = tk->src_begin; q < tk->src_end; q++) {
+      const chol_upd_src *sd = &w->src[q];
+      if (sd->pad != 1 || sd->lda != sd->ldb || sd->a_off - ri != sd->b_off - rj) return -1;
+      for (int m = 0; m * CHOL_NB < sd->k; m++) {
+        if (n < cap) { const early_cell x = { ri / CHOL_NB, rj / CHOL_NB, sd->a_off - ri + (int64_t)m * CHOL_NB * sd->lda }; out[n] = x; }
+        n++;
+      }
+    }
+  }
+  return n;
+}
+static int check_follow_coverage(const chol_level_work *w, const chol_program *g)
+{
+  int rc = 0, net;
+  int *et = early_task_list(w, &net);
+  for (int j = 0; j < g->n_job && !rc; j++) {
+    const chol_job *jb = &g->job[j];
+    if (jb->kind != CHOL_JOB_POTRF || jb->n_ext <= 0) continue;
+    const chol_potrf_desc *pd = &w->potrf[jb->first];
+    const int T = (pd->n + CHOL_NB - 1) / CHOL_NB, nc = T * T;
+    const int64_t ne = follower_early_cells(w, et, net, pd, NULL, 0);
+    if (ne < 0) { chol_set_error("program job %d: an early task into its diagonal block is not a cell of the tile grid", j); rc = CHOLAMD_ERR_ARG; break; }
+    early_cell *ec = malloc((ne > 0 ? ne : 1) * sizeof(early_cell));
+    follower_early_cells(w, et, net, pd, ec, ne);
+    int64_t *tile = malloc((jb->n_ext + ne + 1) * sizeof(int64_t));
+    int nt = 0;
+    for (int x = 0; x < jb->n_ext; x++) tile[nt++] = g->ext[jb->ext_first + x].off;
+    for (int64_t z = 0; z < ne; z++) {
+      int u = 0;
+      while (u < nt && tile[u] != ec[z].tile) u++;
+      if (u == nt) tile[nt++] = ec[z].tile;
+    }
+    unsigned char *cnt = calloc((size_t)nt * nc + 1, 1);
+    for (int x = 0; x < jb->n_ext; x++) {
+      const int narrow = (g->ext[jb->ext_first + x].ncol & CHOL_EXT_NARROW) != 0;
+      int u = 0;
+      while (tile[u] != g->ext[jb->ext_first + x].off) u++;
+      for (int I = 0; I < T; I++) for (int J = 0; J <= I && J < (narrow ? CHOL_FOLLOW_COLS_N : T); J++) if (cnt[(size_t)u * nc + I * T + J] < 255) cnt[(size_t)u * nc + I * T + J]++;
+    }
+    for (int64_t z = 0; z < ne; z++) {
+      int u = 0;
+      while (tile[u] != ec[z].tile) u++;
+      if (cnt[(size_t)u * nc + ec[z].I * T + ec[z].J] < 255) cnt[(size_t)u * nc + ec[z].I * T + ec[z].J]++;
+    }
+    for (int u = 0; u < nt && !rc; u++)
+      for (int I = 0; I < T && !rc; I++)
+        for (int J = 0; J <= I; J++)
+          if (cnt[(size_t)u * nc + I * T + J] != 1) {
+            chol_set_error("program job %d: cell (%d, %d) of its diagonal block gets source column tile %d (of %d) %d times", j, I, J, u, nt, cnt[(size_t)u * nc + I * T + J]);
+            rc = CHOLAMD_ERR_ARG; break;
+          }
+    free(cnt); free(tile); free(ec);
+  }
+  free(et);
+  return rc;
+}
 int chol_program_check(const plan_t *p, const chol_sched_opts *opts, int workers)
 {
   chol_level_work w;
@@ -1605,6 +1700,18 @@
         int at = 0;
         while (at < jb->mode && at < jb->n_ext) at += chol_follow_round(at, jb->n_ext, (w.potrf[jb->first].n + CHOL_NB - 1) / CHOL_NB);
         if (at != jb->mode) { chol_set_error("program job %d adds its own tiles at item %d of %d: not the start of a round", j, jb->mode, jb->n_ext); rc = CHOLAMD_ERR_ARG; break; }
+        const int T = (w.potrf[jb->first].n + CHOL_NB - 1) / CHOL_NB;
+        int narrow = 0;
+        for (int x = 0; x < jb->n_ext; x++) narrow += (g.ext[jb->ext_first + x].ncol & CHOL_EXT_NARROW) != 0;
+        if (jb->n_pre < 0) {
+          const int a_at = -1 - jb->n_pre;
+          const chol_wait *wa = &g.wait[jb->wait_first];
+          at = 0;
+          while (at < a_at && at < jb->n_ext) at += chol_follow_round(at, jb->n_ext, T);
+          if (at != a_at || a_at >= jb->n_ext || jb->mode != jb->n_ext || jb->n_wait != 2 || wa[0].ctr != wa[1].ctr || wa[0].value > wa[1].value || wa[0].value < 0 || T <= CHOL_FOLLOW_COLS_N || narrow == 0) {
+            chol_set_error("program job %d: follow_cols mode with part A at item %d of %d, own tiles at %d, %d waits, %d narrow items", j, a_at, jb->n_ext, jb->mode, jb->n_wait, narrow); rc = CHOLAMD_ERR_ARG; break;
+          }
+        } else if (narrow) { chol_set_error("program job %d has %d narrow items outside the follow_cols mode", j, narrow); rc = CHOLAMD_ERR_ARG; break; }
       }
       if (ok && jb->kind == CHOL_JOB_POTRF)
         for (int x = 0; x < jb->n_ext && ok; x++) {
@@ -1631,6 +1738,7 @@
   for (int c = 0; c < g.n_ctr && !rc; c++)
     if (val[c] != g.ctr_total[c]) { chol_set_error("program counter %d ends at %d, total %d", c, val[c], g.ctr_total[c]); rc = CHOLAMD_ERR_ARG; }
   free(val); free(state);
+  if (!rc) rc = check_follow_coverage(&w, &g);
   if (!rc) {
     quad *a = NULL, *b = NULL;
     int64_t na = 0, nb = 0, ca = 0, cb = 0;
@@ -1681,6 +1789,22 @@
   if (follow_own >= 0) o.follow_own = follow_own;
   if (split_min >= 0) o.split_min = split_min;
   if (split_nb >= 0) o.split_nb = split_nb;
+  return chol_program_check(p, &o, workers);
+}
+static void follow_opts(chol_sched_opts *o, int env, int follow_tail, int follow_tail_split, int follow_own, int follow_cols, int split_min, int split_nb)
+{
+  if (env) chol_sched_opts_from_env(o); else chol_sched_opts_default(o);
+  if (follow_tail >= 0) o->follow_tail = follow_tail;
+  if (follow_tail_split >= 0) o->follow_tail_split = follow_tail_split;
+  if (follow_own >= 0) o->follow_own = follow_own;
+  if (follow_cols >= 0) o->follow_cols = follow_cols;
+  if (split_min >= 0) o->split_min = split_min;
+  if (split_nb >= 0) o->split_nb = split_nb;
+}
+int cholamd_plan_program_check_cols(const cholamd_plan *p, int follow_tail, int follow_tail_split, int follow_own, int follow_cols, int split_min, int split_nb, int workers)
+{
+  chol_sched_opts o;
+  follow_opts(&o, 1, follow_tail, follow_tail_split, follow_own, follow_cols, split_min, split_nb);
   return chol_program_check(p, &o, workers);
 }
 int64_t cholamd_plan_program_jobs(const cholamd_plan *p, int follow, int64_t cap, int *out)
@@ -1735,12 +1859,7 @@
 int64_t cholamd_plan_program_follow_own(const cholamd_plan *p, int follow_tail, int follow_tail_split, int follow_own, int split_min, int split_nb, int64_t cap, int *out)
 {
   chol_sched_opts o;
-  chol_sched_opts_default(&o);
-  if (follow_tail >= 0) o.follow_tail = follow_tail;
-  if (follow_tail_split >= 0) o.follow_tail_split = follow_tail_split;
-  if (follow_own >= 0) o.follow_own = follow_own;
-  if (split_min >= 0) o.split_min = split_min;
-  if (split_nb >= 0) o.split_nb = split_nb;
+  follow_opts(&o, 0, follow_tail, follow_tail_split, follow_own, 0, split_min, split_nb);
   chol_level_work w; chol_program g;
   if (chol_build_program(p, &o, &w, &g)) return -1;
   int64_t n = 0;
@@ -1753,18 +1872,46 @@
   chol_level_work_free(&w); chol_program_free(&g);
   return n;
 }
+int64_t cholamd_plan_program_follow_cols(const cholamd_plan *p, int follow_tail, int follow_tail_split, int follow_own, int follow_cols, int split_min, int split_nb, int64_t cap, int64_t *out)
+{
+  chol_sched_opts o;
+  follow_opts(&o, 0, follow_tail, follow_tail_split, follow_own, follow_cols, split_min, split_nb);
+  chol_level_work w; chol_program g;
+  if (chol_build_program(p, &o, &w, &g)) return -1;
+  int net;
+  int *et = early_task_list(&w, &net);
+  int64_t k = 1, nrec = 0;
+#define PUT(V_) do { if (k < cap) out[k] = (V_); k++; } while (0)
+  for (int j = 0; j < g.n_job; j++) {
+    const chol_job *jb = &g.job[j];
+    if (jb->kind != CHOL_JOB_POTRF || jb->n_ext <= 0) continue;
+    const chol_potrf_desc *pd = &w.potrf[jb->first];
+    const chol_wait *wl = &g.wait[jb->wait_first];
+    const int cols = jb->n_pre < 0;
+    int64_t ne = follower_early_cells(&w, et, net, pd, NULL, 0);
+    if (ne < 0) ne = 0;
+    early_cell *ec = malloc((ne > 0 ? ne : 1) * sizeof(early_cell));
+    follower_early_cells(&w, et, net, pd, ec, ne);
+    PUT(j); PUT(jb->n_ext); PUT((pd->n + CHOL_NB - 1) / CHOL_NB); PUT(jb->mode); PUT(cols ? -1 - jb->n_pre : -1);
+    PUT(cols ? wl[0].ctr : -1); PUT(cols ? wl[0].value : 0);
+    PUT(jb->n_wait > 0 ? wl[jb->n_wait - 1].ctr : -1); PUT(jb->n_wait > 0 ? wl[jb->n_wait - 1].value : 0);
+    PUT(jb->n_wait); PUT(ne); PUT(CHOL_FOLLOW_COLS_N);
+    for (int x = 0; x < jb->n_ext; x++) { const chol_ext *e = &g.ext[jb->ext_first + x]; PUT(e->off); PUT((e->ncol & CHOL_EXT_NARROW) != 0); PUT(e->ctr); }
+    for (int64_t z = 0; z < ne; z++) { PUT(ec[z].I); PUT(ec[z].J); PUT(ec[z].tile); }
+    free(ec);
+    nrec++;
+  }
+#undef PUT
+  if (cap > 0) out[0] = nrec;
+  free(et);
+  chol_level_work_free(&w); chol_program_free(&g);
+  return k;
+}
 typedef struct { int job, add; } hz_sig;
-int cholamd_plan_program_hazards(const cholamd_plan *p, int follow_tail, int follow_tail_split, int follow_own, int split_min, int split_nb, int out[4])
-{
-  chol_sched_opts o;
-  chol_sched_opts_default(&o);
-  if (follow_tail >= 0) o.follow_tail = follow_tail;
-  if (follow_tail_split >= 0) o.follow_tail_split = follow_tail_split;
-  if (follow_own >= 0) o.follow_own = follow_own;
-  if (split_min >= 0) o.split_min = split_min;
-  if (split_nb >= 0) o.split_nb = split_nb;
+static int program_hazards(const cholamd_plan *p, const chol_sched_opts *opts, int out[6])
+{
   chol_level_work w; chol_program g;
-  int rc = chol_build_program(p, &o, &w, &g);
+  int rc = chol_build_program(p, opts, &w, &g);
   if (rc) return rc;
   const int nj = g.n_job, nw = (nj + 63) / 64;
   int *ns = calloc(g.n_ctr + 1, sizeof(int)), *first = calloc(g.n_ctr + 2, sizeof(int));
@@ -1833,6 +1980,49 @@
       }
     }
   }
+  out[4] = out[5] = 0;
+  uint64_t *gs = calloc(nw + 1, sizeof(uint64_t));
+  for (int j = 0; j < nj; j++) {
+    const chol_job *jb = &g.job[j];
+    if (jb->kind != CHOL_JOB_POTRF || jb->n_ext <= 0 || jb->n_pre >= 0) continue;
+    const int c = g.wait[jb->wait_first].ctr, v = g.wait[jb->wait_first].value;
+    memset(gs, 0, (nw + 1) * sizeof(uint64_t));
+    for (int y = first[c]; y < first[c + 1]; y++) {
+      int m = 0;
+      for (int z = wfirst[c]; z < wfirst[c + 1]; z++) {
+        const hz_wait *x = &wt[wof[z]];
+        if (x->value > m && (x->job == sg[y].job || HZ_HAS(pre, sg[y].job, x->job))) m = x->value;
+      }
+      reqv[y] = m;
+    }
+    for (int a = first[c]; a < first[c + 1] && v > 0; a++) {
+      const int A = sg[a].job;
+      int f = 0;
+      for (int y = first[c]; y < first[c + 1] && f < v; y++) if (sg[y].job != A && reqv[y] < v && !HZ_HAS(pre, sg[y].job, A)) f += sg[y].add;
+      if (f >= v) continue;
+      const uint64_t *pa = pre + (size_t)A * nw;
+      for (int k = 0; k < nw; k++) gs[k] |= pa[k] | (k == A / 64 ? (uint64_t)1 << (A % 64) : 0);
+    }
+    const chol_potrf_desc *pd = &w.potrf[jb->first];
+    const int64_t pbase = pd->a_off - pd->col0 - (int64_t)pd->col0 * pd->lda, pend = (int64_t)pd->lda * p->sep_size[pd->sep];
+    const int cw = pd->n < CHOL_FOLLOW_COLS_N * CHOL_NB ? pd->n : CHOL_FOLLOW_COLS_N * CHOL_NB;
+    for (int u = 0; u < nj; u++) {
+      const chol_job *ub = &g.job[u];
+      if (ub->kind != CHOL_JOB_UPDATE) continue;
+      int hit = 0;
+      for (int t = ub->first; t < ub->first + ub->n && !hit; t++) {
+        const chol_upd_task *tk = &w.task[t];
+        const int64_t rel = tk->c_off - pbase;
+        if (rel < 0 || rel >= pend) continue;
+        const int r0 = (int)(rel % pd->lda), c0 = (int)(rel / pd->lda);
+        hit = r0 < pd->col0 + pd->n && r0 + tk->mv > pd->col0 && c0 < pd->col0 + cw && c0 + tk->nv > pd->col0;
+      }
+      if (!hit) continue;
+      out[4]++;
+      if (!((gs[u / 64] >> (u % 64)) & 1)) out[5]++;
+    }
+  }
+  free(gs);
   free(wt); free(nwc); free(wfirst); free(wof); free(reqv);
   int *last = malloc((size_t)(p->arena > 0 ? p->arena : 1) * sizeof(int));
   for (int64_t e = 0; e < p->arena; e++) last[e] = -1;
@@ -1861,6 +2051,21 @@
   chol_level_work_free(&w); chol_program_free(&g);
   return rc;
 }
+int cholamd_plan_program_hazards(const cholamd_plan *p, int follow_tail, int follow_tail_split, int follow_own, int split_min, int split_nb, int out[4])
+{
+  chol_sched_opts o;
+  follow_opts(&o, 0, follow_tail, follow_tail_split, follow_own, -1, split_min, split_nb);
+  int o6[6];
+  const int rc = program_hazards(p, &o, o6);
+  if (!rc) memcpy(out, o6, 4 * sizeof(int));
+  return rc;
+}
+int cholamd_plan_program_hazards_cols(const cholamd_plan *p, int follow_tail, int follow_tail_split, int follow_own, int follow_cols, int split_min, int split_nb, int out[6])
+{
+  chol_sched_opts o;
+  follow_opts(&o, 0, follow_tail, follow_tail_split, follow_own, follow_cols, split_min, split_nb);
+  return program_hazards(p, &o, out);
+}
 int cholamd_plan_program_counts(const cholamd_plan *p, int follow, int out[6])
 {
   chol_sched_opts o;
diff --git a/cholesky_amd/plan.py b/cholesky_amd/plan.py
--- a/cholesky_amd/plan.py
+++ b/cholesky_amd/plan.py
@@ -258,9 +258,9 @@
     def program_check(self, follow=True, workers=64):
         check(self.L.cholamd_plan_program_check(self.h, int(follow), int(workers)), "cholamd_plan_program_check")
 
-    def program_check_opts(self, follow_tail=-1, split_min=-1, split_nb=-1, workers=64, follow_tail_split=-1, follow_own=-1):
-        check(self.L.cholamd_plan_program_check_follow(self.h, follow_tail, follow_tail_split, follow_own, split_min, split_nb, int(workers)),
-              "cholamd_plan_program_check_follow")
+    def program_check_opts(self, follow_tail=-1, split_min=-1, split_nb=-1, workers=64, follow_tail_split=-1, follow_own=-1, follow_cols=-1):
+        check(self.L.cholamd_plan_program_check_cols(self.h, follow_tail, follow_tail_split, follow_own, follow_cols, split_min, split_nb, int(workers)),
+              "cholamd_plan_program_check_cols")
 
     def program_follow_own(self, follow_own=-1, follow_tail=-1, follow_tail_split=-1, split_min=-1, split_nb=-1):
         n = self.L.cholamd_plan_program_follow_own(self.h, follow_tail, follow_tail_split, follow_own, split_min, split_nb, 0, None)
@@ -269,6 +269,31 @@
         buf = np.zeros(5 * n + 5, dtype=np.int32)
         self.L.cholamd_plan_program_follow_own(self.h, follow_tail, follow_tail_split, follow_own, split_min, split_nb, buf.size, buf.ctypes.data)
         return [dict(zip(("job", "n_ext", "T", "own_at", "n_wait"), (int(v) for v in buf[5 * i:5 * i + 5]))) for i in range(n)]
+
+    def program_follow_cols(self, follow_cols=-1, follow_own=-1, follow_tail=-1, follow_tail_split=-1, split_min=-1, split_nb=-1):
+        args = (self.h, follow_tail, follow_tail_split, follow_own, follow_cols, split_min, split_nb)
+        n = self.L.cholamd_plan_program_follow_cols(*args, 0, None)
+        if n < 0:
+            check(int(n), "cholamd_plan_program_follow_cols")
+        buf = np.zeros(n + 1, dtype=np.int64)
+        self.L.cholamd_plan_program_follow_cols(*args, buf.size, buf.ctypes.data)
+        out, k = [], 1
+        for _ in range(int(buf[0])):
+            job, n_ext, T, own_at, a_at, ca, va, cb, vb, n_wait, ne, cols = (int(v) for v in buf[k:k + 12])
+            k += 12
+            items = [(int(buf[k + 3 * i]), bool(buf[k + 3 * i + 1]), int(buf[k + 3 * i + 2])) for i in range(n_ext)]
+            k += 3 * n_ext
+            early = [tuple(int(v) for v in buf[k + 3 * i:k + 3 * i + 3]) for i in range(ne)]
+            k += 3 * ne
+            out.append(dict(job=job, n_ext=n_ext, T=T, own_at=own_at, a_at=a_at, wait_a=(ca, va) if a_at >= 0 else None,
+                            wait_b=(cb, vb) if n_wait > 0 else None, n_wait=n_wait, cols=cols, items=items, early=early))
+        return out
+
+    def program_hazards_cols(self, follow_cols=-1, follow_own=-1, follow_tail=-1, follow_tail_split=-1, split_min=-1, split_nb=-1):
+        out = np.zeros(6, dtype=np.int32)
+        check(self.L.cholamd_plan_program_hazards_cols(self.h, follow_tail, follow_tail_split, follow_own, follow_cols, split_min, split_nb, out.ctypes.data),
+              "cholamd_plan_program_hazards_cols")
+        return int(out[0]), int(out[1]), (int(out[2]), int(out[3])), int(out[4]), int(out[5])
 
     def program_hazards(self, follow_own=-1, follow_tail=-1, follow_tail_split=-1, split_min=-1, split_nb=-1):
         out = np.zeros(4, dtype=np.int32)
diff --git a/include/cholamd.h b/include/cholamd.h
--- a/include/cholamd.h
+++ b/include/cholamd.h
@@ -116,11 +116,14 @@
 int cholamd_plan_program_check(const cholamd_plan *p, int follow, int workers);
 int cholamd_plan_program_check_opts(const cholamd_plan *p, int follow_tail, int split_min, int split_nb, int workers);
 int cholamd_plan_program_check_follow(const cholamd_plan *p, int follow_tail, int follow_tail_split, int follow_own, int split_min, int split_nb, int workers);
+int cholamd_plan_program_check_cols(const cholamd_plan *p, int follow_tail, int follow_tail_split, int follow_own, int follow_cols, int split_min, int split_nb, int workers);
 int cholamd_plan_program_counts(const cholamd_plan *p, int follow, int out[6]);
 int cholamd_follow_rounds(int n_ext, int tile_columns, int cap, int *rounds_out, int *own_at_out);
 int64_t cholamd_plan_program_followers(const cholamd_plan *p, int64_t cap, int *out);
 int64_t cholamd_plan_program_follow_own(const cholamd_plan *p, int follow_tail, int follow_tail_split, int follow_own, int split_min, int split_nb, int64_t cap, int *out);
+int64_t cholamd_plan_program_follow_cols(const cholamd_plan *p, int follow_tail, int follow_tail_split, int follow_own, int follow_cols, int split_min, int split_nb, int64_t cap, int64_t *out);
 int cholamd_plan_program_hazards(const cholamd_plan *p, int follow_tail, int follow_tail_split, int follow_own, int split_min, int split_nb, int out[4]);
+int cholamd_plan_program_hazards_cols(const cholamd_plan *p, int follow_tail, int follow_tail_split, int follow_own, int follow_cols, int split_min, int split_nb, int out[6]);
 int64_t cholamd_plan_program_jobs(const cholamd_plan *p, int follow, int64_t cap, int *out);
 int cholamd_plan_arena_to_dense(const cholamd_plan *p, const double *arena, double *dense);
 int cholamd_plan_write_matrix(const cholamd_plan *p, const double *arena, const char *file, int full_precision);
```
